# gmlc-dispatches/dispatches

Hardware: AMD Instinct MI355X
Metric: LP scenarios solved/sec, RTS-GMLC 24h multi-period dispatch, batch=4096 (higher is better)
Workload: dtype f64

## Files before the change

### dispatches_amd/csrc/dsp_capi.hip

```cpp
#include <hip/hip_runtime.h>

#include <cmath>
#include <cstdio>
#include <atomic>
#include <cstdlib>
#include <cstring>
#include <memory>
#include <new>
#include <vector>

#include "dsp_capi_internal.hpp"
#include "dsp_prepare.hpp"
#include "dsp_rtc.hpp"
#include "dsp_stream.hpp"

using namespace dsp;

struct Geometry { int wpb = 1, blocks_per_cu = 1; size_t lds = 0; };

struct dsp_handle {
  int device = 0;
  int n = 0, m = 0;
  int64_t nnz = 0;
  int cpl = 0, rpl = 0;
// ... 172 lines not shown
    Sc = build_slot_ell(AT, Lc, Lr, Ec.long_owner, pad_w);
    Sr = build_slot_ell(A, Lr, Lc, Er.long_owner, pad_w);
  }
  SlotELL Scu = build_slot_ell(ATu, Lc, Lr, Ec.long_owner, pad_w), Sru = build_slot_ell(Au, Lr, Lc, Er.long_owner, pad_w);
  const bool shared_slots = shared_slot_maps(cpl, rpl);
  SlotMap My = optimise_slots(Sc, P.m_pad, 4000, shared_slots), Mx = optimise_slots(Sr, P.n_pad, 4000, shared_slots);
  h->lds_conflicts[0] = My.cost_identity; h->lds_conflicts[1] = My.cost_final;
  h->lds_conflicts[2] = Mx.cost_identity; h->lds_conflicts[3] = Mx.cost_final;
  apply_slots(Sc, My.slot); apply_slots(Scu, My.slot);
  apply_slots(Sr, Mx.slot); apply_slots(Sru, Mx.slot);
  std::vector<int32_t> nat_x((size_t)P.n_pad, 0), nat_y((size_t)P.m_pad, 0);
  for (int j = 0; j < h->n; ++j) nat_x[j] = 8 * Mx.slot[Lc.pos[j]];
  for (int i = 0; i < h->m; ++i) nat_y[i] = 8 * My.slot[Lr.pos[i]];
  P.mr_wc_pack = Sc.pack; P.mr_wr_pack = Sr.pack; P.mr_tailc_entries = (int)Sc.tail_val.size(); P.mr_tailr_entries = (int)Sr.tail_val.size();
  if ((rc = fill_long(P.mr_long_c, Sc.long_owner_pos, Sc)) || (rc = fill_long(P.mr_long_r, Sr.long_owner_pos, Sr))) return rc;
  h->matreg = h->opt.no_matreg ? 0 : (rtc_ok ? 1 : matreg_available(cpl, rpl, Sc.pack, Sr.pack, has_long));
  h->matreg_qp = h->opt.no_matreg ? 0 : matreg_available(cpl, rpl, Sc.pack, Sr.pack, has_long, true);
  std::vector<Entry> pk;
  auto ent = [&](const std::vector<double> &val, const auto &idx, const Entry **field) {
    if (rc == DSP_OK) { pack_entries(val, idx, pk); rc = upload(h, pk, field); }
  };
  auto vec = [&](const auto &v, auto field) { if (rc == DSP_OK) rc = upload(h, v, field); };
  ent(Ec.val, Ec.idx, &P.ellc); ent(Er.val, Er.idx, &P.ellr); ent(Ec.tail_val, Ec.tail_idx, &P.tailc); ent(Er.tail_val, Er.tail_idx, &P.tailr);
  ent(Ecu.val, Ecu.idx, &P.ellc_unscaled); ent(Eru.val, Eru.idx, &P.ellr_unscaled);
  ent(Ecu.tail_val, Ecu.tail_idx, &P.tailc_unscaled); ent(Eru.tail_val, Eru.tail_idx, &P.tailr_unscaled);
  vec(h->dc, &P.col_scale); vec(h->dr, &P.row_scale);
  ent(Sc.val, Sc.off, &P.mr_ellc); ent(Sr.val, Sr.off, &P.mr_ellr); ent(Sc.tail_val, Sc.tail_off, &P.mr_tailc); ent(Sr.tail_val, Sr.tail_off, &P.mr_tailr);
  vec(Lc.at, &P.mr_colat); vec(Lr.at, &P.mr_rowat); vec(Mx.slot, &P.mr_slot_x); vec(My.slot, &P.mr_slot_y);
  ent(Scu.val, Scu.off, &P.mr_ellc_unscaled); ent(Sru.val, Sru.off, &P.mr_ellr_unscaled);
  ent(Scu.tail_val, Scu.tail_off, &P.mr_tailc_unscaled); ent(Sru.tail_val, Sru.tail_off, &P.mr_tailr_unscaled);
  vec(nat_x, &P.mr_nat_slot_x); vec(nat_y, &P.mr_nat_slot_y);
  return rc;
}

static int create_device_objects(dsp_handle *h, const HostCSR &A) {
  if (!h->opt.no_simplex && h->n + h->m <= 128 && h->m <= 64 && h->m >= 1) {
    h->sx_lds = simplex_lds_bytes(h->n, h->m, &h->sx_row_stride);
    if (h->sx_lds <= (size_t)h->lds_limit) {
      std::vector<double> dense((size_t)h->m * h->n, 0.0);
      for (int i = 0; i < A.m; ++i)
        for (int p = A.ptr[i]; p < A.ptr[i + 1]; ++p) dense[(size_t)i * h->n + A.idx[p]] = A.val[p];
      if (int rc = upload(h, dense, &h->A_dense)) return rc;
      h->simplex = 1;
    }
  }
  const size_t ring = sizeof(int) * kQueueRing * kQueueStride;
  if (hipMalloc((void **)&h->queue, ring) != hipSuccess || hipMemset(h->queue, 0, ring) != hipSuccess) return DSP_ERR_HIP;
  void *aw = nullptr;
  if (hipMalloc(&aw, sizeof(double) * (kAnchorWeights + 1)) != hipSuccess) return DSP_ERR_HIP;
  h->allocs.push_back(aw); h->anchor_w = (const double *)aw;
  hipLaunchKernelGGL(anchor_weight_kernel, dim3(1), dim3(256), 0, (hipStream_t)0, (double *)aw, kAnchorWeights + 1);
  if (hipGetLastError() != hipSuccess || hipStreamSynchronize((hipStream_t)0) != hipSuccess) return DSP_ERR_HIP;
  if (h->matreg && h->rtc_state[0] != 1) {
    SolveArgs first{}; first.P = h->P; first.matreg = 1; first.qp = 0;
    const size_t l = lds_bytes(h->P, 1, 0, h->cpl, h->rpl);
    if (l <= (size_t)h->lds_limit && light_followup_blocks(h->cpl, h->rpl, first, l) > 0) h->light_lds = l;
  }
  return DSP_OK;
}

static int resolve_options(const dsp_handle *h, const dsp_batch *batch, const dsp_options *opt, SolveArgs *a) {
  a->P = h->P; a->b = *batch; a->anchor_w = h->anchor_w;
  a->opt = opt ? *opt : h->opt;
  const dsp_options &o = a->opt;
  if (o.max_iter < 1 || o.check_every < 0 || o.kkt_every < 0 || !(o.kkt_gate >= 0) || o.stall_rescue < 0 || o.polish_patience < 0 || !(o.jump_rel >= 0) ||
      !(o.eps_rel > 0) || !(o.eps_obj >= 0) || !(o.eps_infeasible >= 0) || !(o.pid_kp >= 0) || !(o.restart_artificial >= 0) || !(o.step_scale > 0))
    return DSP_ERR_INVALID;
  a->eta = o.step_scale * h->eta_unit;
  a->qp = batch->row_compliance != nullptr;
  const bool fused64 = !h->streaming && o.precision == 0;
  if (o.restart_artificial == 0.0) a->opt.restart_artificial = fused64 ? (a->qp ? 0.3 : 0.2) : 0.36;
  if (o.pid_kp == 0.0) a->opt.pid_kp = fused64 ? 0.6 : 0.7;
  if (o.precision != 0 && o.precision != 1) return DSP_ERR_INVALID;
  const bool has_long = h->P.long_c.count > 0 || h->P.long_r.count > 0;
  if (o.precision && (h->streaming || has_long)) return DSP_ERR_INVALID;
  if (a->qp && !h->streaming && has_long) return DSP_ERR_INVALID;
  return DSP_OK;
}

static int finish_stats(dsp_handle *h, const dsp_batch *batch, dsp_stats *stats, bool timed, hipStream_t st) {
  if (!timed) return DSP_OK;
  const int B = batch->B;
  HIP_TRY(hipStreamSynchronize(st));
  HIP_TRY(hipEventElapsedTime(&stats->kernel_ms, h->ev0, h->ev1));
  std::vector<int32_t> hs(B), hi(B);
  HIP_TRY(hipMemcpy(hs.data(), batch->status, B * sizeof(int32_t), hipMemcpyDeviceToHost));
  if (batch->iters) HIP_TRY(hipMemcpy(hi.data(), batch->iters, B * sizeof(int32_t), hipMemcpyDeviceToHost));
  for (int i = 0; i < B; ++i) {
    stats->n_optimal += hs[i] == DSP_STATUS_OPTIMAL;
    if (batch->iters) { stats->total_iterations += hi[i]; stats->max_iterations = std::max(stats->max_iterations, hi[i]); }
  }
  return DSP_OK;
}

struct Followup { bool light = false; int wpb = 0; size_t lds = 0; };
static Followup followup_geometry(const dsp_handle *h, bool light) {
  Followup f{light};
  for (int wpb = 1; wpb <= 4 && !light; ++wpb) {
    const size_t l = lds_bytes(h->P, wpb, 0, h->cpl, h->rpl);
    if (l <= (size_t)h->lds_limit) { f.wpb = wpb; f.lds = l; }
  }
  if (light) { f.wpb = 1; f.lds = h->light_lds; }
  return f;
}
static hipError_t launch_followup(const dsp_handle *h, Followup f, const SolveArgs &first, const SolveArgs &c, int grid, hipStream_t st) {
  return f.light ? launch_solve_light(h->cpl, h->rpl, first, c, grid, f.lds, st)
                 : launch_solve(h->cpl, h->rpl, c, dim3(grid), dim3(64 * f.wpb), f.lds, st);
}

static int *claim_queue_slot(dsp_handle *h, hipStream_t st, int ints) {
  int *q = h->queue + (size_t)(h->queue_next.fetch_add(1u) % kQueueRing) * kQueueStride;
  hipLaunchKernelGGL(queue_reset_kernel, dim3(1), dim3(64), 0, st, q, ints);
  return q;
}

static int solve_streaming(dsp_handle *h, const dsp_batch *batch, const SolveArgs &a, dsp_stats *stats, bool timed, hipStream_t st) {
  if (timed) HIP_TRY(hipEventRecord(h->ev0, st));
  int periods = 0;
  HIP_TRY(stream_solve(&h->stream, *batch, a.opt, a.eta, st, &periods));
  if (timed) HIP_TRY(hipEventRecord(h->ev1, st));
  stats->streaming = 1; stats->quadratic = a.qp;
  stats->grid_blocks = (std::max(h->n, h->m) + 255) / 256; stats->block_threads = 256;
  stats->stream_bytes_per_iteration = (int64_t)stream_bytes_per_iteration(&h->stream);
  const StreamReport &rep = h->stream.report;
  stats->stream_form = rep.form;
  stats->stream_phases = rep.phases;
  stats->ipm_solved = rep.ipm_solved;
  return finish_stats(h, batch, stats, timed, st);
}

static int solve_f32(dsp_handle *h, const dsp_batch *batch, SolveArgs &a, dsp_stats *stats, bool timed, hipStream_t st) {
  a.queue = claim_queue_slot(h, st, 2);
  if (timed) HIP_TRY(hipEventRecord(h->ev0, st));
  int grid = 0, threads = 0; size_t lds = 0;
  HIP_TRY(launch_solve_f32(h->cpl, h->rpl, a, h->num_cus, (size_t)h->lds_limit, st, &grid, &threads, &lds));
  if (timed) HIP_TRY(hipEventRecord(h->ev1, st));
  stats->grid_blocks = grid; stats->block_threads = threads; stats->lds_bytes = (int)lds;
  stats->cols_per_lane = h->cpl; stats->rows_per_lane = h->rpl; stats->quadratic = a.qp; stats->precision = 1;
  return finish_stats(h, batch, stats, timed, st);
}

static int grow_simplex_warm(dsp_handle *h, int B) {
  const size_t N = (size_t)h->n + h->m;
  double *t = nullptr; int *bs = nullptr, *vl = nullptr; unsigned char *up = nullptr;
  HIP_TRY(hipMalloc((void **)&t, (size_t)B * h->m * N * sizeof(double))); h->sx_warm_allocs.push_back(t);
  HIP_TRY(hipMalloc((void **)&bs, (size_t)B * h->m * sizeof(int))); h->sx_warm_allocs.push_back(bs);
  HIP_TRY(hipMalloc((void **)&up, (size_t)B * N)); h->sx_warm_allocs.push_back(up);
  HIP_TRY(hipMalloc((void **)&vl, (size_t)B * sizeof(int))); h->sx_warm_allocs.push_back(vl);
  HIP_TRY(hipMemset(vl, 0, (size_t)B * sizeof(int)));
  h->sx_warm_T = t; h->sx_warm_basis = bs; h->sx_warm_upper = up; h->sx_warm_valid = vl; h->sx_warm_cap = B;
  return DSP_OK;
}

static int simplex_pass(dsp_handle *h, SolveArgs &a, hipStream_t st) {
  if (!h->simplex || a.qp) return DSP_OK;
  const int B = a.b.B;
  SimplexArgs sa{};
  sa.n = h->n; sa.m = h->m; sa.row_stride = h->sx_row_stride; sa.max_pivots = 20 * (h->n + h->m);
  sa.A_dense = h->A_dense; sa.col_scale = h->P.col_scale; sa.row_scale = h->P.row_scale; sa.b = a.b;
  sa.tol_p = 1e-10; sa.tol_d = 1e-12; sa.tol_piv = 1e-9; sa.unsolved = a.queue + 1;
  { static const char *tp = getenv("DSP_SX_TOLP"); if (tp) sa.tol_p = atof(tp); }
  if (a.opt.simplex_warm == 1 || a.opt.simplex_warm == 2) {
    if (B > h->sx_warm_cap)
      if (int rc = grow_simplex_warm(h, B)) return rc;
    sa.warm = a.opt.simplex_warm;
    sa.warm_T = h->sx_warm_T; sa.warm_basis = h->sx_warm_basis; sa.warm_upper = h->sx_warm_upper; sa.warm_valid = h->sx_warm_valid;
  }
  static const int sx_debug = getenv("DSP_SX_DEBUG") ? atoi(getenv("DSP_SX_DEBUG")) : 0;
  sa.debug_keep = sx_debug;
  const int per_cu = std::max<int>(1, std::min<int>(32, (int)((size_t)h->lds_limit / h->sx_lds)));
  HIP_TRY(launch_simplex(sa, std::min(B, h->num_cus * per_cu), h->sx_lds, st));
  a.skip_solved = 1;
  return DSP_OK;
}

static hipError_t first_pass(dsp_handle *h, SolveArgs &a, int grid, size_t lds, hipStream_t st) {
  if (!(h->rtc_state[a.qp] == 1 && a.matreg)) return launch_solve(h->cpl, h->rpl, a, dim3(grid), dim3(64 * a.waves_per_block), lds, st);
  size_t arg_size = sizeof(a);
  void *config[] = {HIP_LAUNCH_PARAM_BUFFER_POINTER, &a, HIP_LAUNCH_PARAM_BUFFER_SIZE, &arg_size, HIP_LAUNCH_PARAM_END};
  return hipModuleLaunchKernel(h->rtc[a.qp].fn, grid, 1, 1, 64 * a.waves_per_block, 1, 1, (unsigned)lds, st, nullptr, config);
}

static int certificate_pass(dsp_handle *h, const SolveArgs &a, Followup f, bool host_waits, hipStream_t st) {
  if (!a.matreg || !(a.opt.eps_infeasible > 0.0)) return DSP_OK;
  SolveArgs c = a;
  c.matreg = 0; c.skip_solved = 2; c.queue = a.queue + 3;
  c.b.x0 = a.b.x; c.b.y0 = a.b.y; c.waves_per_block = f.wpb;
  static const int cert_grid_env = getenv("DSP_CERT_GRID") ? atoi(getenv("DSP_CERT_GRID")) : 0;
  int nsus = -1;
  if (host_waits) {
    HIP_TRY(hipMemcpyAsync(&nsus, a.suspects, sizeof(int), hipMemcpyDeviceToHost, st));
    HIP_TRY(hipStreamSynchronize(st));
  }
  if (nsus == 0) return DSP_OK;
  const int want = nsus > 0 ? (nsus + f.wpb - 1) / f.wpb : (cert_grid_env > 0 ? cert_grid_env : 8);
  HIP_TRY(launch_followup(h, f, a, c, std::max(1, std::min(std::min((a.b.B + f.wpb - 1) / f.wpb, want), 2 * h->num_cus)), st));
  return DSP_OK;
}

static int recertify_passes(dsp_handle *h, const SolveArgs &a, Followup f, hipStream_t st) {
  if (!(a.opt.recertify_passes > 0 && a.b.flags)) return DSP_OK;
  static const struct { double pid_kp, restart_artificial; int check_every; } kRecertify[3] = {{0.45, 0.3, 0}, {0.8, 0.15, 0}, {0.3, 0.5, 12}};
  for (int v = 0; f.wpb && v < std::min(a.opt.recertify_passes, 3); ++v) {
    SolveArgs c = a;
    c.matreg = 0; c.skip_solved = 3; c.queue = a.queue + 5 + v;
    c.b.x0 = nullptr; c.b.y0 = nullptr; c.waves_per_block = f.wpb;
    c.opt.pid_kp = kRecertify[v].pid_kp; c.opt.restart_artificial = kRecertify[v].restart_artificial;
    if (kRecertify[v].check_every) c.opt.check_every = kRecertify[v].check_every;
    c.opt.polish_patience = std::max(c.opt.polish_patience, 1024);
    HIP_TRY(launch_followup(h, f, a, c, std::max(1, std::min((a.b.B + f.wpb - 1) / f.wpb, 64)), st));
  }
  return DSP_OK;
}

static int solve_fused(dsp_handle *h, const dsp_batch *batch, SolveArgs &a, dsp_stats *stats, bool timed, hipStream_t st) {
  const int B = batch->B, qp = a.qp;
  if (qp && h->rtc_state[1] == -1) {
    h->rtc_state[1] = rtc_get_kernel(h->device, h->cpl, h->rpl, false, h->P.mr_wc_pack, h->P.mr_wr_pack, true, &h->rtc[1], &h->rtc_why) ? 1 : 0;
    if (h->rtc_state[1] == 1) h->matreg_qp = 1;
  }
  Geometry geo;
  int rc = solve_geometry(h, a.opt.waves_per_block, B, &geo, qp);
  if (rc != DSP_OK) return rc;
  a.waves_per_block = geo.wpb; a.queue = claim_queue_slot(h, st, 8);
  a.queue_base = 0u; a.unsolved = a.queue + 1;
  a.suspects = a.queue + 2;
  a.matreg = qp ? h->matreg_qp : h->matreg;
#ifdef DSP_KKT_TRACE
  const char *trace_env = getenv("DSP_TRACE_SCENARIO");
  double *trace_dev = nullptr;
  if (trace_env) {
    HIP_TRY(hipMalloc((void **)&trace_dev, 4096 * 12 * sizeof(double)));
    HIP_TRY(hipMemsetAsync(trace_dev, 0, 4096 * 12 * sizeof(double), st));
    a.trace = trace_dev; a.trace_scenario = atoi(trace_env);
  }
#endif
  const int grid = std::min((B + geo.wpb - 1) / geo.wpb, h->num_cus * geo.blocks_per_cu);
  const Followup f = followup_geometry(h, a.matreg && !qp && h->rtc_state[0] != 1 && h->light_lds > 0);
  if (a.matreg && a.opt.eps_infeasible > 0.0 && !f.wpb) a.opt.eps_infeasible = 0.0;
  if (timed) HIP_TRY(hipEventRecord(h->ev0, st));
  if ((rc = simplex_pass(h, a, st)) != DSP_OK) return rc;
  HIP_TRY(first_pass(h, a, grid, geo.lds, st));
  if ((rc = certificate_pass(h, a, f, timed, st)) != DSP_OK || (rc = recertify_passes(h, a, f, st)) != DSP_OK) return rc;
  if (timed) HIP_TRY(hipEventRecord(h->ev1, st));
#ifdef DSP_KKT_TRACE
  if (trace_dev) {
    HIP_TRY(hipStreamSynchronize(st));
    std::vector<double> tr(4096 * 12);
    HIP_TRY(hipMemcpy(tr.data(), trace_dev, tr.size() * sizeof(double), hipMemcpyDeviceToHost));
    (void)hipFree(trace_dev);
    const char *path = getenv("DSP_TRACE_FILE");
    if (FILE *f = fopen(path ? path : "dsp_trace.bin", "wb")) { fwrite(tr.data(), sizeof(double), tr.size(), f); fclose(f); }
  }
#endif
  stats->grid_blocks = grid; stats->block_threads = 64 * a.waves_per_block; stats->lds_bytes = (int)geo.lds;
  stats->cols_per_lane = h->cpl; stats->rows_per_lane = h->rpl; stats->matreg = a.matreg; stats->simplex = h->simplex && !qp;
  stats->quadratic = qp; stats->rtc = (h->rtc_state[qp] == 1 && a.matreg) ? 1 : 0;
  stats->lds_conflicts_identity = h->lds_conflicts[0] + h->lds_conflicts[2];
  stats->lds_conflicts_chosen = a.matreg ? h->lds_conflicts[1] + h->lds_conflicts[3] : stats->lds_conflicts_identity;
  return finish_stats(h, batch, stats, timed, st);
}

extern "C" {

void dsp_default_options(dsp_options *o) {
  if (!o) return;
  std::memset(o, 0, sizeof(*o));
  o->eps_rel = 1e-9;
  o->eps_obj = 5e-7;
  o->max_iter = 200000;
  o->check_every = 0;
  o->kkt_every = 32;
  o->kkt_gate = 16.0;
  o->stall_rescue = 4000;
  o->no_simplex = 0;
  o->jump_rel = 3.0;
  o->restart_sufficient = 0.2;
  o->restart_necessary = 0.8;
  o->restart_artificial = 0.0;
  o->pid_kp = 0.0;
  o->max_dlog_weight = std::log(30.0);
  o->step_scale = 0.998;
  o->weight_guard = 4.0;
  o->jump_steady = 0.05;
  o->jump_tol = 3e-3;
  o->jump_min = 4.0;
  o->ray_jumps = 1;
  o->ruiz_iters = 10;
  o->waves_per_block = 0;
  o->precision = 0;
  o->polish_patience = 1024;
  o->no_rtc = 0;
  o->no_interior_point = 0;
  o->eps_infeasible = 1e-6;
  o->recertify_passes = 0;
  o->simplex_warm = 0;
  o->warm_patience = 0;
}

int dsp_version(void) { return DSP_VERSION; }
#ifndef DSP_SOURCE_HASH
#define DSP_SOURCE_HASH "unknown"
#endif
static const char kSourceHashTag[] = "dsp_source_hash=" DSP_SOURCE_HASH;
const char *dsp_source_hash(void) { return kSourceHashTag + 16; }
int dsp_last_hip_error(void) { return g_last_hip_error; }

const char *dsp_strerror(int code) {
  switch (code) {
    case DSP_OK: return "ok";
    case DSP_ERR_INVALID: return "invalid argument";
    case DSP_ERR_TOO_LARGE: return "LP too large (more than 4096 vectors longer than the ELL width, or dsp_spmv_step on a streaming handle)";
    case DSP_ERR_HIP: return "HIP runtime error (see dsp_last_hip_error)";
    case DSP_ERR_NO_DEVICE: return "no HIP device";
    case DSP_ERR_ALLOC: return "allocation failed";
    default: return "unknown error";
  }
}

int dsp_create(const dsp_lp_desc *d, int device, const dsp_options *opt, dsp_handle **out) {
  if (!out || !desc_ok(d)) return DSP_ERR_INVALID;
  static const int kCpl[] = {1, 2, 3, 4, 5, 7, 10};
  static const int kRpl[] = {1, 2, 3, 4, 6};
  int cpl = pick(kCpl, 7, (d->n + 63) / 64);
  int rpl = pick(kRpl, 5, std::max(1, (d->m + 63) / 64));
  const bool streaming = cpl < 0 || rpl < 0 || d->n > 65535 || d->m > 65535;
  if (streaming && d->m < 1) return DSP_ERR_INVALID;

  int ndev = 0;
  if (hipGetDeviceCount(&ndev) != hipSuccess || ndev <= 0) return DSP_ERR_NO_DEVICE;
  if (device < 0 || device >= ndev) return DSP_ERR_INVALID;
  HIP_TRY(hipSetDevice(device));

  struct Destroy { void operator()(dsp_handle *p) const { dsp_destroy(p); } };
  std::unique_ptr<dsp_handle, Destroy> owner(new (std::nothrow) dsp_handle());
  dsp_handle *h = owner.get();
  if (!h) return DSP_ERR_ALLOC;
  h->device = device; h->n = d->n; h->m = d->m; h->nnz = d->nnz; h->cpl = cpl; h->rpl = rpl;
  if (opt) h->opt = *opt; else dsp_default_options(&h->opt);
  hipDeviceProp_t prop;
  if (hipGetDeviceProperties(&prop, device) == hipSuccess) {
    h->num_cus = prop.multiProcessorCount;
    h->lds_limit = (int)prop.maxSharedMemoryPerMultiProcessor > 0 ? (int)prop.maxSharedMemoryPerMultiProcessor : 64 * 1024;
  }

  HostCSR A; A.m = d->m; A.n = d->n;
  A.ptr.assign(d->A_rowptr, d->A_rowptr + d->m + 1);
  A.idx.assign(d->A_colidx, d->A_colidx + d->nnz);
  A.val.assign(d->A_val, d->A_val + d->nnz);
  HostCSR Au = A;
  equilibrate(A, h->opt.ruiz_iters, h->dr, h->dc, std::max(0, h->opt.geo_iters), d->col_scale);
  HostCSR AT = transpose(A), ATu = transpose(Au);
  h->eta_unit = 1.0 / spectral_norm(A, AT, 500);
  int rc = streaming ? create_streaming(h, A, AT) : create_fused(h, A, AT, Au, ATu);
  if (rc == DSP_OK && !streaming) rc = create_device_objects(h, A);
  if (rc != DSP_OK) return rc;
  if (hipEventCreate(&h->ev0) != hipSuccess || hipEventCreate(&h->ev1) != hipSuccess) return DSP_ERR_HIP;
  *out = owner.release();
  return DSP_OK;
}

int dsp_solve(dsp_handle *h, const dsp_batch *batch, const dsp_options *opt, dsp_stats *stats, int sync_stats, void *hipStream) {
  if (!h || !batch || batch->B < 0) return DSP_ERR_INVALID;
  if (batch->B == 0) { if (stats) std::memset(stats, 0, sizeof(*stats)); return DSP_OK; }
  if (!batch->c || !batch->x || !batch->y || !batch->obj || !batch->status) return DSP_ERR_INVALID;
  hipStream_t st = (hipStream_t)hipStream;
  HIP_TRY(hipSetDevice(h->device));
  SolveArgs a{};
  if (int rc = resolve_options(h, batch, opt, &a)) return rc;
  dsp_stats lent;
  const bool timed = stats && sync_stats;
  stats = stats ? stats : &lent;
  std::memset(stats, 0, sizeof(*stats));
  if (h->streaming) return solve_streaming(h, batch, a, stats, timed, st);
  if (a.opt.precision == 1) return solve_f32(h, batch, a, stats, timed, st);
  return solve_fused(h, batch, a, stats, timed, st);
}

int dsp_spmv_step(dsp_handle *h, int32_t B, const double *X, const double *Y, double *AX, double *ATY, void *hipStream) {
  if (!h || B < 0 || !X || !Y || !AX || !ATY) return DSP_ERR_INVALID;
  if (B == 0) return DSP_OK;
  if (h->streaming) return DSP_ERR_TOO_LARGE;
  HIP_TRY(hipSetDevice(h->device));
  SpmvArgs a{};
  a.P = h->P; a.B = B; a.X = X; a.Y = Y; a.AX = AX; a.ATY = ATY;
  static const int wpb_env = getenv("DSP_SPMV_WPB") ? atoi(getenv("DSP_SPMV_WPB")) : 0;
  constexpr int kSpmvMaxWaves = 16;
  a.waves_per_block = wpb_env > 0 ? std::min(wpb_env, kSpmvMaxWaves) : kMaxWavesPerBlock;
  size_t lds = lds_bytes(h->P, a.waves_per_block);
  while (lds > (size_t)h->lds_limit && a.waves_per_block > 1) lds = lds_bytes(h->P, --a.waves_per_block);
  if (lds > (size_t)h->lds_limit) return DSP_ERR_TOO_LARGE;
  int blocks_per_cu = std::max<int>(1, std::min<int>((int)(h->lds_limit / lds), 32 / a.waves_per_block));
  int grid = std::min((B + a.waves_per_block - 1) / a.waves_per_block, h->num_cus * blocks_per_cu);
  const hipError_t se = launch_spmv(h->cpl, h->rpl, a, dim3(grid), dim3(64 * a.waves_per_block), lds, (hipStream_t)hipStream);
  if (se == hipErrorInvalidValue) return DSP_ERR_INVALID;
  HIP_TRY(se);
  return DSP_OK;
}

int dsp_rtc_compile_check(int cpl, int rpl, int has_long, unsigned wc_pack, unsigned wr_pack, int qp, char *msg, int msg_len) {
  std::vector<char> code;
  std::string name, why;
  const bool ok = rtc_build_code(cpl, rpl, has_long != 0, wc_pack, wr_pack, qp != 0, &code, &name, &why);
  if (msg && msg_len > 0) { std::snprintf(msg, (size_t)msg_len, "%s", ok ? name.c_str() : why.c_str()); }
  return ok ? (int)code.size() : 0;
}

const char *dsp_rtc_message(const dsp_handle *h) { return h ? h->rtc_why.c_str() : ""; }

int dsp_get_dims(const dsp_handle *h, int32_t *n, int32_t *m, int64_t *nnz) {
  if (!h) return DSP_ERR_INVALID;
  if (n) *n = h->n;
  if (m) *m = h->m;
// ... 27 lines not shown
```

### dispatches_amd/csrc/dsp_capi_internal.hpp

```cpp
#pragma once
#include "dsp_device.hpp"

namespace dsp { inline thread_local int g_last_hip_error = 0; }

#define HIP_TRY(expr)                                                                                            \
  do {                                                                                                           \
    if (hipError_t _e = (expr); _e != hipSuccess) { dsp::g_last_hip_error = (int)_e; return DSP_ERR_HIP; }       \
  } while (0)
```

### dispatches_amd/csrc/dsp_capi_loop.hip

```cpp
#include <cmath>
#include <vector>

#include "dsp_capi_internal.hpp"
#include "dsp_record_check.hpp"

using namespace dsp;

static bool market_col_ok(int32_t col, int32_t n) { return col >= 0 && col < n; }
static bool loop_cols_ok(const int32_t *cols, int count, int32_t n) {
  for (int i = 0; i < count; ++i)
    if (!market_col_ok(cols[i], n)) return false;
  return true;
}
static bool loop_terms_ok(const int32_t (*pt_cols)[2], int T, int32_t n) {
  for (int t = 0; t < T; ++t)
    for (int e = 0; e < 2; ++e)
      if (pt_cols[t][e] != -1 && !market_col_ok(pt_cols[t][e], n)) return false;
  return true;
}
static bool loop_wind_ok(const int32_t *wind_cols, int T, int32_t n, const void *cf_series) {
  return wind_cols[0] < 0 || (cf_series && loop_cols_ok(wind_cols, T, n));
}
static bool plant_sizes_ok(const double *wind_kw_plant, const double *c0_base_plant, int32_t wind_col0) {
  if (!wind_kw_plant != !c0_base_plant) return false;
  return !wind_kw_plant || wind_col0 >= 0;
}
static bool loop_tracker_cols_ok(const dsp_loop_model *tr, int T, const void *state, const void *cf_series) {
  if (tr->n_state < 0 || tr->n_state > 2 || (tr->n_state > 0 && !state)) return false;
  return loop_cols_ok(tr->state_init, tr->n_state, tr->n) && loop_cols_ok(tr->track_rows, T, tr->m) && loop_wind_ok(tr->wind_cols, T, tr->n, cf_series) &&
         plant_sizes_ok(tr->wind_kw_plant, tr->c0_base_plant, tr->wind_cols[0]);
}
static bool loop_tracker_ok(const dsp_loop_model *tr, int T, const void *state, const void *cf_series) {
  if (!tr || T < 1 || T > DSP_LOOP_MAX_T || tr->T != T || tr->n < 1 || tr->m < 1) return false;
  if (!tr->lb || !tr->ub || !tr->rlo || !tr->rhi || !tr->c0) return false;
  return loop_tracker_cols_ok(tr, T, state, cf_series);
}
static bool market_state_ok(const dsp_market_state *st) {
  if (!st || st->B < 0 || st->N < 1 || st->S < 1 || st->S > DSP_MARKET_MAX_S) return false;
  if (st->backcast ? (st->D < 1 || st->S > st->D || 24ll * st->D > st->N) : st->S != 1) return false;
  return st->start && st->hour && st->da_series && st->rt_series;
}
static bool loop_market_state_ok(const dsp_loop_market_state *st) {
  if (!st || st->B < 0 || st->N < 1 || st->S < 1 || st->S > DSP_MARKET_MAX_S || st->p_min_cents < 0 || st->p_min_cents > 2000000000ll) return false;
  if (st->backcast ? (st->D < 1 || st->S > st->D || 24ll * st->D > st->N) : st->S != 1) return false;
  if (st->rt_history_lag_days < 0 || (st->backcast && 24ll * ((long long)st->D + st->rt_history_lag_days) > st->N)) return false;
  if (st->self_schedule < 0 || st->self_schedule > 1) return false;
  if (st->curve_slots != 0 && (st->curve_slots < st->S + 1 || st->curve_slots > DSP_MARKET_MAX_S + 1)) return false;
  if (st->coupled < 0 || st->coupled > 1 || (st->coupled && st->self_schedule)) return false;
  return st->start && st->hour && st->da_series && st->rt_series;
}
static bool loop_market_model_ok(const dsp_loop_market_model *m) {
  return m && m->n >= 1 && m->T >= 1 && m->T <= DSP_MARKET_MAX_T && m->n_state >= 0 && m->n_state <= 2 &&
         (m->row_stride == 0 || m->row_stride >= m->n);
}
static bool loop_market_prepare_ok(const dsp_loop_market_state *st, const dsp_loop_market_model *m) {
  if (!m->c || !m->lb || !m->ub || !m->base_c || !m->c0) return false;
  if ((m->n_state > 0 && !st->state) || !loop_cols_ok(m->state_init, m->n_state, m->n)) return false;
  if (!loop_wind_ok(m->wind_cols, m->T, m->n, st->cf_series) || !plant_sizes_ok(m->wind_kw_plant, m->c0_base_plant, m->wind_cols[0])) return false;
  return loop_cols_ok(m->pda_cols, m->T, m->n) && loop_terms_ok(m->pt_cols, m->T, m->n);
}

static bool plant_p_min_ok(const dsp_loop_market_state *st, hipStream_t stream) {
  if (!st->p_min_cents_plant || st->B == 0) return true;
  hipStreamCaptureStatus capturing = hipStreamCaptureStatusNone;
  if (hipStreamIsCapturing(stream, &capturing) != hipSuccess) return false;
  if (capturing != hipStreamCaptureStatusNone) return true;
  std::vector<int64_t> host((size_t)st->B);
  if (hipMemcpyAsync(host.data(), st->p_min_cents_plant, host.size() * sizeof(int64_t), hipMemcpyDeviceToHost, stream) != hipSuccess) return false;
  if (hipStreamSynchronize(stream) != hipSuccess) return false;
  for (int64_t v : host)
    if (v < 0 || v > 2000000000ll) return false;
  return true;
}

extern "C" {

int dsp_wb_rolling_update(const dsp_wb_state *st, const dsp_wb_model *rt, const dsp_wb_model *tr, int32_t phase, int32_t k, void *hipStream) {
  if (!st || !rt || !tr || st->B < 0 || phase < 0 || phase > 2 || k < 0 || k > 23 || rt->T < 1 || rt->T > 8 || tr->T < 1 || tr->T > 8)
    return DSP_ERR_INVALID;
  if (st->B == 0) return DSP_OK;
  HIP_TRY(launch_wb_rolling(*st, *rt, *tr, (int)phase, (int)k, (hipStream_t)hipStream));
  return DSP_OK;
}

int dsp_loop_update(const dsp_loop_state *st, const dsp_loop_model *rt, const dsp_loop_model *tr, int32_t phase, int32_t k, void *hipStream) {
  if (!st || !rt || !tr || st->B < 0 || phase < 0 || phase > 2 || k < 0 || k > 23 || rt->T < 1 || rt->T > DSP_LOOP_MAX_T || tr->T < 1 ||
      tr->T > DSP_LOOP_MAX_T || rt->n_state < 0 || rt->n_state > 2 || tr->n_state != rt->n_state || !rt->c0 || !tr->c0)
    return DSP_ERR_INVALID;
  if (!plant_sizes_ok(rt->wind_kw_plant, rt->c0_base_plant, rt->wind_cols[0]) || !rt->wind_kw_plant != !tr->wind_kw_plant) return DSP_ERR_INVALID;
  if ((phase < 2 && tr->T > rt->T) || !loop_tracker_cols_ok(tr, tr->T, st->state, st->cf_series) || !loop_cols_ok(tr->state_real, tr->n_state, tr->n) ||
      !loop_terms_ok(tr->pt_cols, tr->T, tr->n))
    return DSP_ERR_INVALID;
  if (!loop_cols_ok(rt->pda_cols, rt->T, rt->n) || !loop_terms_ok(rt->pt_cols, rt->T, rt->n) || !loop_cols_ok(rt->state_init, rt->n_state, rt->n) ||
      !loop_wind_ok(rt->wind_cols, rt->T, rt->n, st->cf_series))
    return DSP_ERR_INVALID;
  if (st->B == 0) return DSP_OK;
  HIP_TRY(launch_loop_update(*st, *rt, *tr, (int)phase, (int)k, (hipStream_t)hipStream));
  return DSP_OK;
}

int dsp_loop_ledger(const dsp_loop_state *st, const dsp_loop_model *tr, const dsp_loop_ledger_desc *g, void *hipStream) {
  if (!st || !tr || !g || st->B < 0 || tr->n < 1 || !tr->x) return DSP_ERR_INVALID;
  if (g->n_forms < 1 || g->n_forms > DSP_LEDGER_MAX_FORMS || g->reserved != 0) return DSP_ERR_INVALID;
  if (!g->acc || !g->hour_value || !g->coef || !g->constant) return DSP_ERR_INVALID;
  if (g->coef_stride < 0 || (g->coef_stride != 0 && g->coef_stride < (int64_t)g->n_forms * DSP_LEDGER_MAX_TERMS)) return DSP_ERR_INVALID;
  if (g->const_stride < 0 || (g->const_stride != 0 && g->const_stride < g->n_forms)) return DSP_ERR_INVALID;
  for (int f = 0; f < g->n_forms; ++f) {
    if (g->n_terms[f] < 0 || g->n_terms[f] > DSP_LEDGER_MAX_TERMS || !loop_cols_ok(g->cols[f], g->n_terms[f], tr->n)) return DSP_ERR_INVALID;
    if (g->per_avail[f] == 0.0) continue;
    if (!std::isfinite(g->per_avail[f]) || tr->wind_cols[0] < 0 || !st->cf_series || !st->start || !st->hour || st->N < 1) return DSP_ERR_INVALID;
    if (!plant_sizes_ok(tr->wind_kw_plant, tr->c0_base_plant, tr->wind_cols[0])) return DSP_ERR_INVALID;
  }
  if (st->B == 0) return DSP_OK;
  HIP_TRY(launch_loop_ledger(*st, *tr, *g, (hipStream_t)hipStream));
  return DSP_OK;
}

int dsp_loop_record(const dsp_loop_record_desc *rec, int32_t B, void *hipStream) {
  if (!loop_record_ok(rec, B)) return DSP_ERR_INVALID;
  HIP_TRY(launch_loop_record(*rec, (hipStream_t)hipStream));
  return DSP_OK;
}

int dsp_bid_points(const dsp_bid_request *rq, void *hipStream) {
  if (!rq || rq->B < 0 || rq->T < 0 || rq->terms < 0 || rq->terms > 2 || rq->ldx < 1 || rq->ldp < rq->T) return DSP_ERR_INVALID;
  if (rq->B > DSP_BID_MAX_SCENARIOS || rq->T > DSP_BID_MAX_HOURS) return DSP_ERR_TOO_LARGE;
  if (rq->T == 0) return DSP_OK;
  if (!rq->out || (rq->B > 0 && (!rq->x || !rq->price))) return DSP_ERR_INVALID;
  for (int t = 0; t < rq->T; ++t)
    for (int e = 0; e < (rq->terms == 2 ? 2 : 1); ++e)
      if (rq->col[t][e] < 0 || rq->col[t][e] >= rq->ldx) return DSP_ERR_INVALID;
  HIP_TRY(launch_bid_points(*rq, (hipStream_t)hipStream));
  return DSP_OK;
}

int dsp_market_prepare(const dsp_market_state *st, const dsp_market_model *m, int32_t k, void *hipStream) {
  if (!market_state_ok(st) || !m || k < -1 || k > 23 || m->n < 1 || m->T < 1 || m->T > DSP_MARKET_MAX_T) return DSP_ERR_INVALID;
  if (!st->cf_series || !st->soc || !st->thr || !m->c || !m->lb || !m->ub || !m->base_c) return DSP_ERR_INVALID;
  if (k >= 0 && (!st->da_offer || !st->da_prices)) return DSP_ERR_INVALID;
  if (!market_col_ok(m->soc_init, m->n) || !market_col_ok(m->thr_init, m->n)) return DSP_ERR_INVALID;
  for (int t = 0; t < m->T; ++t)
    if (!market_col_ok(m->wind_cols[t], m->n) || !market_col_ok(m->pt_cols[t][0], m->n) || !market_col_ok(m->pt_cols[t][1], m->n) ||
        !market_col_ok(m->pda_cols[t], m->n))
      return DSP_ERR_INVALID;
  if (st->B == 0) return DSP_OK;
  HIP_TRY(launch_market_prepare(*st, *m, (int)k, (hipStream_t)hipStream));
  return DSP_OK;
}

int dsp_market_clear(const dsp_market_state *st, const dsp_market_model *m, const dsp_wb_model *tr, int32_t k, int32_t T,
                     double *dispatch, int32_t *curve, int32_t *count, void *hipStream) {
  if (!market_state_ok(st) || !m || k < -1 || k > 23 || m->n < 1 || m->T < 1 || m->T > DSP_MARKET_MAX_T || T < 1 || T > m->T) return DSP_ERR_INVALID;
  if (!m->x || !m->status || !dispatch || !curve || !count) return DSP_ERR_INVALID;
  if (k < 0 ? (T > 24 || !st->da_prices || tr) : T > 8) return DSP_ERR_INVALID;
  for (int t = 0; t < T; ++t)
    if (k < 0 ? !market_col_ok(m->pda_cols[t], m->n) : (!market_col_ok(m->pt_cols[t][0], m->n) || !market_col_ok(m->pt_cols[t][1], m->n)))
      return DSP_ERR_INVALID;
  if (tr) {
    if (tr->T != T || tr->n < 1 || tr->m < 1 || !tr->lb || !tr->ub || !tr->rlo || !tr->rhi || !st->cf_series || !st->soc || !st->thr) return DSP_ERR_INVALID;
    if (!market_col_ok(tr->soc_init, tr->n) || !market_col_ok(tr->thr_init, tr->n)) return DSP_ERR_INVALID;
    for (int t = 0; t < T; ++t)
      if (!market_col_ok(tr->wind_cols[t], tr->n) || !market_col_ok(tr->track_rows[t], tr->m)) return DSP_ERR_INVALID;
  }
  if (st->B == 0) return DSP_OK;
  HIP_TRY(launch_market_clear(*st, *m, tr, (int)k, (int)T, dispatch, curve, count, (hipStream_t)hipStream));
  return DSP_OK;
}

int dsp_loop_market_prepare(const dsp_loop_market_state *st, const dsp_loop_market_model *m, int32_t k, void *hipStream) {
  if (!loop_market_state_ok(st) || !loop_market_model_ok(m) || k < -1 || k > 23) return DSP_ERR_INVALID;
  if (m->row_stride != 0 && m->row_stride != m->n) return DSP_ERR_INVALID;
  if (k >= 0 && (!st->da_offer || !st->da_prices)) return DSP_ERR_INVALID;
  if (!loop_market_prepare_ok(st, m)) return DSP_ERR_INVALID;
  if (st->B == 0) return DSP_OK;
  HIP_TRY(launch_loop_market_prepare(*st, *m, (int)k, (hipStream_t)hipStream));
  return DSP_OK;
}

int dsp_loop_schedule_prepare(const dsp_loop_market_state *st, const dsp_loop_market_model *m, void *hipStream) {
  if (!loop_market_state_ok(st) || !loop_market_model_ok(m)) return DSP_ERR_INVALID;
  if ((long long)m->row_stride < (long long)st->S * m->n) return DSP_ERR_INVALID;
  if (!loop_market_prepare_ok(st, m) || m->wind_kw_plant || m->c0_base_plant) return DSP_ERR_INVALID;
  if (st->B == 0) return DSP_OK;
  HIP_TRY(launch_loop_schedule_prepare(*st, *m, (hipStream_t)hipStream));
  return DSP_OK;
}

int dsp_loop_monotone_prepare(const dsp_loop_market_state *st, const dsp_loop_market_model *m, double *rlo, double *rhi, int32_t m_rows,
                              int32_t first_coupling_row, void *hipStream) {
  if (!loop_market_state_ok(st) || !loop_market_model_ok(m) || !rlo || !rhi || st->S < 2 || first_coupling_row < 0) return DSP_ERR_INVALID;
  if ((long long)m->row_stride < (long long)st->S * m->n) return DSP_ERR_INVALID;
  if ((long long)first_coupling_row + (long long)(st->S * (st->S - 1) / 2) * m->T > (long long)m_rows) return DSP_ERR_INVALID;
  if (!loop_market_prepare_ok(st, m) || m->wind_kw_plant || m->c0_base_plant) return DSP_ERR_INVALID;
  if (st->B == 0) return DSP_OK;
  HIP_TRY(launch_loop_monotone_prepare(*st, *m, rlo, rhi, (int)m_rows, (int)first_coupling_row, (hipStream_t)hipStream));
  return DSP_OK;
}

int dsp_loop_market_clear(const dsp_loop_market_state *st, const dsp_loop_market_model *m, const dsp_loop_model *tr, int32_t k, int32_t T,
                          double *dispatch, int32_t *curve, int32_t *count, void *hipStream) {
  if (!loop_market_state_ok(st) || !loop_market_model_ok(m) || k < -1 || k > 23 || T < 1 || T > m->T) return DSP_ERR_INVALID;
  if (st->coupled && (long long)m->row_stride < (long long)st->S * m->n) return DSP_ERR_INVALID;
  if (!m->x || !m->status || !dispatch || !curve || !count) return DSP_ERR_INVALID;
  if (k < 0 ? (T > 24 || !st->da_prices || tr) : T > DSP_LOOP_MAX_T) return DSP_ERR_INVALID;
  if (!plant_sizes_ok(m->wind_kw_plant, m->c0_base_plant, m->wind_cols[0])) return DSP_ERR_INVALID;
  if (k < 0 ? !loop_cols_ok(m->pda_cols, T, m->n) : !loop_terms_ok(m->pt_cols, T, m->n)) return DSP_ERR_INVALID;
  if (tr && (!loop_tracker_ok(tr, T, st->state, st->cf_series) || tr->n_state != m->n_state || !tr->wind_kw_plant != !m->wind_kw_plant)) return DSP_ERR_INVALID;
  if (!plant_p_min_ok(st, (hipStream_t)hipStream)) return DSP_ERR_INVALID;
  if (st->B == 0) return DSP_OK;
  HIP_TRY(launch_loop_market_clear(*st, *m, tr, (int)k, (int)T, dispatch, curve, count, (hipStream_t)hipStream));
  return DSP_OK;
}

int dsp_loop_param_step(const dsp_loop_param_state *st, const dsp_loop_model *tr, int32_t phase, int32_t k, void *hipStream) {
  if (!st || !tr || st->B < 1 || st->N < 24 || tr->T < 1 || tr->T > DSP_LOOP_MAX_T) return DSP_ERR_INVALID;
  if (phase < 0 || phase > 2 || (phase == 0 ? k != -1 : (k < 0 || k > 23))) return DSP_ERR_INVALID;
  if (tr->wind_kw_plant || tr->c0_base_plant) return DSP_ERR_INVALID;
  if (!st->start || !st->hour || !st->da_series || !st->rt_series || !st->da_cf_series || !st->rt_cf_series || !st->bid_price ||
      !st->storage_mw)
    return DSP_ERR_INVALID;
  if (phase == 0) {
    if (!st->da_offer || !st->da_prices || !st->da_curve || !st->da_count) return DSP_ERR_INVALID;
  } else if (phase == 1) {
    if (!st->rt_dispatch || !st->rt_curve || !st->rt_count) return DSP_ERR_INVALID;
    if (!loop_tracker_ok(tr, tr->T, st->state, st->rt_cf_series)) return DSP_ERR_INVALID;
  } else {
    if (!st->h2_kg || !tr->x || tr->n < 1 || !market_col_ok(st->pem_col, tr->n)) return DSP_ERR_INVALID;
  }
  HIP_TRY(launch_loop_param_step(*st, *tr, (int)phase, (hipStream_t)hipStream));
  return DSP_OK;
}

int dsp_loop_project(const dsp_loop_project_state *st, const dsp_loop_model *pj, int32_t phase, int32_t j, void *hipStream) {
  if (!st || st->B < 1 || st->N < 1 || st->ruc_hour < 1 || st->ruc_hour > 23 || phase < 0 || phase > 2) return DSP_ERR_INVALID;
// ... 23 lines not shown
```

### dispatches_amd/csrc/dsp_device.hpp

```cpp
#pragma once
#ifdef __HIPCC_RTC__
#ifndef DSP_RTC_TYPES
#define DSP_RTC_TYPES
typedef signed char int8_t; typedef unsigned char uint8_t; typedef short int16_t; typedef unsigned short uint16_t;
typedef int int32_t; typedef unsigned int uint32_t; typedef long long int64_t; typedef unsigned long long uint64_t;
typedef unsigned long uintptr_t; typedef unsigned long size_t;
#ifndef INFINITY
#define INFINITY (__builtin_inff())
#endif
#ifndef NAN
#define NAN (__builtin_nanf(""))
#endif
#endif
#else
#include <hip/hip_runtime.h>

#include <cstdint>
#endif

#include "../../include/dsp_hip.h"
#include "dsp_shapes.hpp"

namespace dsp {

constexpr int kMaxLong = 32;

struct __attribute__((aligned(16))) Entry {
  double v;
  uint32_t off;
  uint32_t pad;
};

struct LongList {
  int count;
  int owner[kMaxLong];
  int start[kMaxLong];
  int len[kMaxLong];
};

struct DeviceProblem {
  int n, m;
  int n_pad, m_pad;
  int Wc, Wr;
  int ellc_entries, ellr_entries, tailc_entries, tailr_entries;
  const Entry *ellc, *ellr, *tailc, *tailr;
  const Entry *ellc_unscaled, *ellr_unscaled, *tailc_unscaled, *tailr_unscaled;
  const double *col_scale, *row_scale;
  LongList long_c, long_r;
  const Entry *mr_ellc, *mr_ellr, *mr_tailc, *mr_tailr;
  int mr_tailc_entries, mr_tailr_entries;
  const int *mr_colat, *mr_rowat;
  unsigned mr_wc_pack, mr_wr_pack;
  const int32_t *mr_slot_x, *mr_slot_y;
  LongList mr_long_c, mr_long_r;
  const Entry *mr_ellc_unscaled, *mr_ellr_unscaled, *mr_tailc_unscaled, *mr_tailr_unscaled;
  const int32_t *mr_nat_slot_x, *mr_nat_slot_y;
};

#define DSP_STATUS_UNSOLVED 99
#define DSP_STATUS_SUSPECT 98

struct SolveArgs {
  DeviceProblem P;
  dsp_batch b;
  int skip_solved;
  int waves_per_block;
  double eta;
  dsp_options opt;
  int *queue;
  unsigned queue_base;
  const int *unsolved;
  int matreg;
  int qp;
  double *trace;
  int trace_scenario;
  int *suspects;
  const double *anchor_w;
};

constexpr int kAnchorWeights = 4096;

#ifdef DSP_KKT_TRACE
#define DSP_SW_TRACE 1ull
#else
#define DSP_SW_TRACE 0ull
#endif
#ifdef DSP_PROF
#define DSP_SW_PROF 2ull
#else
#define DSP_SW_PROF 0ull
#endif
#ifdef DSP_CLOCKS
#define DSP_SW_CLOCKS 4ull
#else
#define DSP_SW_CLOCKS 0ull
#endif
#ifdef DSP_LEGACY_PULL
#define DSP_SW_PULL 8ull
#else
#define DSP_SW_PULL 0ull
#endif
#ifdef DSP_NO_JUMP
#define DSP_SW_NOJUMP 16ull
#else
#define DSP_SW_NOJUMP 0ull
#endif
constexpr unsigned long long kBuildSwitches = DSP_SW_TRACE | DSP_SW_PROF | DSP_SW_CLOCKS | DSP_SW_PULL | DSP_SW_NOJUMP;
constexpr unsigned long long kSolveArgsToken =
    ((unsigned long long)sizeof(SolveArgs) << 40) ^ ((unsigned long long)__builtin_offsetof(SolveArgs, opt) << 28) ^
    ((unsigned long long)__builtin_offsetof(SolveArgs, queue) << 16) ^ ((unsigned long long)sizeof(DeviceProblem) << 52) ^
    ((unsigned long long)DSP_VERSION << 8) ^ kBuildSwitches ^ ((unsigned long long)__builtin_offsetof(SolveArgs, anchor_w) << 4) ^
    ((unsigned long long)rare_lds_bytes(0) << 20);

struct SimplexArgs {
  int n, m;
  int row_stride;
  int max_pivots;
  const double *A_dense;
  const double *col_scale, *row_scale;
  dsp_batch b;
  double tol_p, tol_d, tol_piv;
  int *unsolved;
  int debug_keep;
  int warm;
  double *warm_T;
  int *warm_basis;
  unsigned char *warm_upper;
  int *warm_valid;
};

struct SpmvArgs {
  DeviceProblem P;
  int B;
  int waves_per_block;
  const double *X, *Y;
  double *AX, *ATY;
};

constexpr int kPadWidth = 4;
inline unsigned uniform_pack(int slots, int w) { unsigned p = 0; for (int q = 0; q < slots; ++q) p |= (unsigned)w << (4 * q); return p; }

#ifndef __HIPCC_RTC__
hipError_t launch_solve(int cpl, int rpl, const SolveArgs &a, dim3 grid, dim3 block, size_t lds, hipStream_t st);
int matreg_available(int cpl, int rpl, unsigned wc_pack, unsigned wr_pack, bool lng, bool qp = false);
hipError_t occupancy_solve(int cpl, int rpl, const SolveArgs &a, int block_threads, size_t lds, int *blocks_per_cu);
int light_followup_blocks(int cpl, int rpl, const SolveArgs &first, size_t lds);
hipError_t launch_solve_light(int cpl, int rpl, const SolveArgs &first, const SolveArgs &a, int grid, size_t lds, hipStream_t st);
size_t simplex_lds_bytes(int n, int m, int *row_stride);
hipError_t launch_simplex(const SimplexArgs &a, int grid, size_t lds, hipStream_t st);
hipError_t launch_solve_f32(int cpl, int rpl, const SolveArgs &a, int num_cus, size_t lds_limit, hipStream_t st, int *grid,
                            int *threads, size_t *lds);
hipError_t launch_wb_rolling(const dsp_wb_state &st, const dsp_wb_model &rt, const dsp_wb_model &tr, int phase, int k, hipStream_t stream);
hipError_t launch_loop_update(const dsp_loop_state &st, const dsp_loop_model &rt, const dsp_loop_model &tr, int phase, int k, hipStream_t stream);
hipError_t launch_loop_ledger(const dsp_loop_state &st, const dsp_loop_model &tr, const dsp_loop_ledger_desc &ledger, hipStream_t stream);
hipError_t launch_loop_record(const dsp_loop_record_desc &rec, hipStream_t stream);
hipError_t launch_bid_points(const dsp_bid_request &rq, hipStream_t st);
hipError_t launch_market_prepare(const dsp_market_state &st, const dsp_market_model &m, int k, hipStream_t stream);
hipError_t launch_market_clear(const dsp_market_state &st, const dsp_market_model &m, const dsp_wb_model *tr, int k, int T, double *dispatch,
                               int32_t *curve, int32_t *count, hipStream_t stream);
hipError_t launch_loop_market_prepare(const dsp_loop_market_state &st, const dsp_loop_market_model &m, int k, hipStream_t stream);
hipError_t launch_loop_schedule_prepare(const dsp_loop_market_state &st, const dsp_loop_market_model &m, hipStream_t stream);
hipError_t launch_loop_monotone_prepare(const dsp_loop_market_state &st, const dsp_loop_market_model &m, double *rlo, double *rhi, int m_rows,
                                        int first, hipStream_t stream);
hipError_t launch_loop_market_clear(const dsp_loop_market_state &st, const dsp_loop_market_model &m, const dsp_loop_model *tr, int k, int T,
                                    double *dispatch, int32_t *curve, int32_t *count, hipStream_t stream);
hipError_t launch_loop_param_step(const dsp_loop_param_state &st, const dsp_loop_model &tr, int phase, hipStream_t stream);
hipError_t launch_loop_project(const dsp_loop_project_state &st, const dsp_loop_model &pj, int phase, int j, hipStream_t stream);
hipError_t launch_spmv(int cpl, int rpl, const SpmvArgs &a, dim3 grid, dim3 block, size_t lds, hipStream_t st);

#endif

}
```

### dispatches_amd/csrc/dsp_loop.hip

```cpp
#include <hip/hip_runtime.h>

#include "dsp_device.hpp"
#include "dsp_loop_device.hpp"

using namespace dsp;

template <class M, class S>
__device__ __forceinline__ void loop_check(const S &s, const M &m, int b) {
  if (m.status && s.bad && m.status[b] != 0) *s.bad = 1;
  if (m.flags && s.uncertified && (m.flags[b] & DSP_FLAG_OBJ_WAIVED)) atomicAdd(reinterpret_cast<unsigned long long *>(s.uncertified), 1ull);
}

__global__ void __launch_bounds__(256) wb_rolling_kernel(dsp_wb_state s, dsp_wb_model rt, dsp_wb_model tr, int phase, int k) {
  const int b = blockIdx.x * blockDim.x + threadIdx.x;
  if (b >= s.B) return;
  const long long h = *s.hour, st0 = s.start[b];
  auto win = [&](const double *series, int t) { return series[(st0 + h + t) % s.N]; };
  if (phase == 0) {
    const dsp_wb_model &m = rt;
    const int known = min(m.T, 24 - k);
    double *c = m.c + (size_t)b * m.n, *lb = m.lb + (size_t)b * m.n, *ub = m.ub + (size_t)b * m.n;
    double avail_sum = 0.0;
    for (int t = 0; t < m.T; ++t) {
      const double rtp = win(s.rt_series, t);
      const double dap = t < known ? s.da_prices[(size_t)b * 24 + k + t] : win(s.da_series, t);
      const double r3 = loop_opaque(__dmul_rn(1e-3, rtp));
      c[m.pt_cols[t][0]] = __dsub_rn(m.base_c[m.pt_cols[t][0]], r3);
      c[m.pt_cols[t][1]] = __dsub_rn(m.base_c[m.pt_cols[t][1]], r3);
      c[m.pda_cols[t]] = __dsub_rn(m.base_c[m.pda_cols[t]], loop_opaque(__dsub_rn(dap, rtp)));
      const double avail = __dmul_rn(m.wind_kw, win(s.cf_series, t));
      ub[m.wind_cols[t]] = avail;
      avail_sum = t ? __dadd_rn(avail_sum, avail) : avail;
      const double fix = t < known ? s.da_offer[(size_t)b * 24 + k + t] : 0.0;
      lb[m.pda_cols[t]] = fix;
      ub[m.pda_cols[t]] = t < known ? fix : INFINITY;
    }
    if (m.c0) m.c0[b] = __dadd_rn(m.c0_base, loop_opaque(__dmul_rn(m.waste_per_kw, avail_sum)));
    lb[m.soc_init] = s.soc[b]; ub[m.soc_init] = s.soc[b];
    lb[m.thr_init] = s.thr[b]; ub[m.thr_init] = s.thr[b];
  } else if (phase == 1) {
    loop_check(s, rt, b);
    const double *xr = rt.x + (size_t)b * rt.n;
    double *lb = tr.lb + (size_t)b * tr.n, *ub = tr.ub + (size_t)b * tr.n;
    double *rlo = tr.rlo + (size_t)b * tr.m, *rhi = tr.rhi + (size_t)b * tr.m;
    double avail_sum = 0.0;
    for (int t = 0; t < tr.T; ++t) {
      const double offer = __dmul_rn(1e-3, loop_opaque(__dadd_rn(xr[rt.pt_cols[t][0]], xr[rt.pt_cols[t][1]])));
      rlo[tr.track_rows[t]] = offer;
      rhi[tr.track_rows[t]] = offer;
      const double avail = __dmul_rn(tr.wind_kw, win(s.cf_series, t));
      ub[tr.wind_cols[t]] = avail;
      avail_sum = t ? __dadd_rn(avail_sum, avail) : avail;
    }
    if (tr.c0) tr.c0[b] = __dadd_rn(tr.c0_base, loop_opaque(__dmul_rn(tr.waste_per_kw, avail_sum)));
    lb[tr.soc_init] = s.soc[b]; ub[tr.soc_init] = s.soc[b];
    lb[tr.thr_init] = s.thr[b]; ub[tr.thr_init] = s.thr[b];
  } else {
    loop_check(s, tr, b);
    const double *x = tr.x + (size_t)b * tr.n;
    const double delivered = loop_opaque(__dmul_rn(1e-3, loop_opaque(__dadd_rn(x[tr.pt_cols[0][0]], x[tr.pt_cols[0][1]]))));
    const double rt0 = win(s.rt_series, 0);
    s.delivered[b] = delivered;
    s.soc[b] = __ddiv_rn(rint(loop_opaque(__dmul_rn(x[tr.soc0], 100.0))), 100.0);
    s.thr[b] = __ddiv_rn(rint(loop_opaque(__dmul_rn(x[tr.thr0], 100.0))), 100.0);
    const double dao = s.da_offer[(size_t)b * 24 + k], dap = s.da_prices[(size_t)b * 24 + k];
    const double t1 = loop_opaque(__dmul_rn(delivered, rt0)), t2 = loop_opaque(__dmul_rn(dao, loop_opaque(__dsub_rn(dap, rt0))));
    s.revenue[b] = __dadd_rn(s.revenue[b], loop_opaque(__dadd_rn(t1, t2)));
    s.energy_mwh[b] = __dadd_rn(s.energy_mwh[b], delivered);
  }
}

__global__ void wb_clock_kernel(long long *hour) { *hour += 1; }

__device__ __forceinline__ double loop_power(const dsp_loop_model &m, const double *x, int t) {
  double p = m.pt_const[t];
  if (m.pt_cols[t][0] >= 0) p = fma(m.pt_coef[t][0], x[m.pt_cols[t][0]], p);
  if (m.pt_cols[t][1] >= 0) p = fma(m.pt_coef[t][1], x[m.pt_cols[t][1]], p);
  return p;
}
__device__ __forceinline__ void loop_state_and_wind(const dsp_loop_state &s, const dsp_loop_model &m, int b, long long h, long long st0, double c0) {
  double *lb = m.lb + (size_t)b * m.n, *ub = m.ub + (size_t)b * m.n;
  for (int j = 0; j < m.n_state; ++j) {
    const double v = s.state[(size_t)b * m.n_state + j];
    lb[m.state_init[j]] = v; ub[m.state_init[j]] = v;
  }
  if (m.wind_cols[0] >= 0) {
    const double kw = m.wind_kw_plant ? m.wind_kw_plant[b] : m.wind_kw;
    double sum = 0.0;
    for (int t = 0; t < m.T; ++t) {
      const double avail = kw * s.cf_series[(st0 + h + t) % s.N];
      ub[m.wind_cols[t]] = avail;
      sum += avail;
    }
    c0 = fma(m.waste_per_kw, sum, c0);
  }
  m.c0[b] = c0;
}
__global__ void __launch_bounds__(256) loop_update_kernel(dsp_loop_state s, dsp_loop_model rt, dsp_loop_model tr, int phase, int k) {
  const int b = blockIdx.x * blockDim.x + threadIdx.x;
  if (b >= s.B) return;
  const long long h = *s.hour, st0 = s.start[b];
  auto win = [&](const double *series, int t) { return series[(st0 + h + t) % s.N]; };
  if (phase == 0) {
    const dsp_loop_model &m = rt;
    const int known = min(m.T, 24 - k);
    double *c = m.c + (size_t)b * m.n, *lb = m.lb + (size_t)b * m.n, *ub = m.ub + (size_t)b * m.n;
    double c0 = m.c0_base_plant ? m.c0_base_plant[b] : m.c0_base;
    for (int t = 0; t < m.T; ++t) {
      const double rtp = win(s.rt_series, t);
      const double dap = t < known ? s.da_prices[(size_t)b * 24 + k + t] : win(s.da_series, t);
      for (int e = 0; e < 2; ++e)
        if (m.pt_cols[t][e] >= 0) c[m.pt_cols[t][e]] = fma(-rtp, m.pt_coef[t][e], m.base_c[m.pt_cols[t][e]]);
      c[m.pda_cols[t]] = m.base_c[m.pda_cols[t]] - (dap - rtp);
      c0 = fma(-rtp, m.pt_const[t], c0);
      const double fix = t < known ? s.da_offer[(size_t)b * 24 + k + t] : 0.0;
      lb[m.pda_cols[t]] = fix;
      ub[m.pda_cols[t]] = t < known ? fix : INFINITY;
    }
    loop_state_and_wind(s, m, b, h, st0, c0);
  } else if (phase == 1) {
    loop_check(s, rt, b);
    const double *xr = rt.x + (size_t)b * rt.n;
    double *rlo = tr.rlo + (size_t)b * tr.m, *rhi = tr.rhi + (size_t)b * tr.m;
    for (int t = 0; t < tr.T; ++t) {
      const double rhs = loop_power(rt, xr, t) - tr.pt_const[t];
      rlo[tr.track_rows[t]] = rhs;
      rhi[tr.track_rows[t]] = rhs;
    }
    loop_state_and_wind(s, tr, b, h, st0, tr.c0_base_plant ? tr.c0_base_plant[b] : tr.c0_base);
  } else {
    loop_check(s, tr, b);
    const double *x = tr.x + (size_t)b * tr.n;
    const double delivered = loop_power(tr, x, 0);
    const double rt0 = win(s.rt_series, 0);
    s.delivered[b] = delivered;
    for (int j = 0; j < tr.n_state; ++j)
      s.state[(size_t)b * tr.n_state + j] = rint(x[tr.state_real[j]] * s.state_scale[j]) / s.state_scale[j];
    const double dao = s.da_offer[(size_t)b * 24 + k], dap = s.da_prices[(size_t)b * 24 + k];
    s.revenue[b] += delivered * rt0 + dao * (dap - rt0);
    s.energy_mwh[b] += delivered;
  }
}

__global__ void __launch_bounds__(256) loop_ledger_kernel(dsp_loop_state s, const double *x, int n, double wind_kw, const double *wind_kw_plant,
                                                          dsp_loop_ledger_desc g) {
  const int b = blockIdx.x * blockDim.x + threadIdx.x, f = blockIdx.y;
  if (b >= s.B) return;
  const double per_avail = g.per_avail[f];
  double avail0 = 0.0;
  if (per_avail != 0.0) {
    const double kw = wind_kw_plant ? wind_kw_plant[b] : wind_kw;
    avail0 = loop_opaque(__dmul_rn(kw, s.cf_series[(s.start[b] + *s.hour) % s.N]));
  }
  const double *coef = g.coef + (size_t)b * g.coef_stride + f * DSP_LEDGER_MAX_TERMS;
  const double v = loop_ledger_form(x + (size_t)b * n, g.cols[f], coef, g.n_terms[f], g.constant[(size_t)b * g.const_stride + f], per_avail, avail0);
  const size_t at = (size_t)f * s.B + b;
  g.hour_value[at] = v;
  g.acc[at] = __dadd_rn(g.acc[at], loop_opaque(v));
}

__global__ void __launch_bounds__(256) loop_record_kernel(dsp_loop_record_desc d) {
  const dsp_loop_record_segment &g = d.segments[blockIdx.y];
  const int e = blockIdx.x * blockDim.x + threadIdx.x;
  if (e >= d.n_plants * g.width) return;
  const int q = e / g.width, j = e - q * g.width;
  const long long t = *d.clock + d.offset;
  const long long r = (t < 0 || t / d.divisor >= d.rows) ? d.rows : t / d.divisor;
  const size_t from = (size_t)d.plants[q] * (size_t)g.plant_stride + (size_t)j * (size_t)g.elem_stride;
  const size_t to = ((size_t)r * d.n_plants + q) * g.width + j;
  if (g.elem_bytes == 8)
    ((unsigned long long *)g.dst)[to] = ((const unsigned long long *)g.src)[from];
  else
    ((unsigned int *)g.dst)[to] = ((const unsigned int *)g.src)[from];
}

namespace dsp {

hipError_t launch_loop_record(const dsp_loop_record_desc &rec, hipStream_t stream) {
  int widest = 0;
  for (int g = 0; g < rec.n_segments; ++g) widest = rec.segments[g].width > widest ? rec.segments[g].width : widest;
  const long long lanes = (long long)rec.n_plants * widest;
  hipLaunchKernelGGL(loop_record_kernel, dim3((unsigned)((lanes + 255) / 256), rec.n_segments), dim3(256), 0, stream, rec);
  return hipGetLastError();
}

hipError_t launch_loop_ledger(const dsp_loop_state &st, const dsp_loop_model &tr, const dsp_loop_ledger_desc &ledger, hipStream_t stream) {
  hipLaunchKernelGGL(loop_ledger_kernel, dim3((st.B + 255) / 256, ledger.n_forms), dim3(256), 0, stream, st, tr.x, (int)tr.n, tr.wind_kw,
                     tr.wind_kw_plant, ledger);
  return hipGetLastError();
}

template <class K, class S, class M>
static hipError_t launch_hand_off(K kernel, const S &st, const M &rt, const M &tr, int phase, int k, hipStream_t stream) {
  hipLaunchKernelGGL(kernel, dim3((st.B + 255) / 256), dim3(256), 0, stream, st, rt, tr, phase, k);
  if (phase == 2) hipLaunchKernelGGL(wb_clock_kernel, dim3(1), dim3(1), 0, stream, (long long *)st.hour);
  return hipGetLastError();
}
hipError_t launch_wb_rolling(const dsp_wb_state &st, const dsp_wb_model &rt, const dsp_wb_model &tr, int phase, int k, hipStream_t stream) {
  return launch_hand_off(wb_rolling_kernel, st, rt, tr, phase, k, stream);
}
hipError_t launch_loop_update(const dsp_loop_state &st, const dsp_loop_model &rt, const dsp_loop_model &tr, int phase, int k, hipStream_t stream) {
  return launch_hand_off(loop_update_kernel, st, rt, tr, phase, k, stream);
}

}
```

### dispatches_amd/csrc/dsp_loop_device.hpp

```cpp
#pragma once
#include <hip/hip_runtime.h>

#include <cstdint>

#include "../../include/dsp_hip.h"
#include "dsp_bid_cents.hpp"

namespace dsp {

__device__ __forceinline__ double loop_opaque(double v) { asm volatile("" : "+v"(v)); return v; }

template <class State>
__device__ __forceinline__ long long loop_scenario_index(const State &s, long long st0, long long h, int i, int hod, int t) {
  if (!s.backcast) return (st0 + h + t) % s.N;
  const long long D = s.D, d = h / 24;
  const long long pos = (24 * (D - 1 - i) + hod + t) % (24 * D);
  long long v = (st0 + 24 * (d - D) + pos) % s.N;
  return v < 0 ? v + s.N : v;
}

__device__ __forceinline__ double loop_wind_window(double *ub, const int32_t *wind_cols, int T, double kw, const double *cf_series,
                                                   long long first, long long N) {
  double avail_sum = 0.0;
  for (int q = 0; q < T; ++q) {
    const double avail = loop_opaque(__dmul_rn(kw, cf_series[(first + q) % N]));
    ub[wind_cols[q]] = avail;
    avail_sum = q ? __dadd_rn(avail_sum, avail) : avail;
  }
  return avail_sum;
}

__device__ __forceinline__ double loop_c0(double base, double per_kw, double avail_sum) {
  return __dadd_rn(base, loop_opaque(__dmul_rn(per_kw, avail_sum)));
}

__device__ __forceinline__ void loop_tracker_plant(const dsp_loop_model &tr, int b, const double *cf_series, long long first, long long N,
                                                   const double *state) {
  double *lb = tr.lb + (size_t)b * tr.n, *ub = tr.ub + (size_t)b * tr.n;
  for (int j = 0; j < tr.n_state; ++j) {
    const double v = state[j];
    lb[tr.state_init[j]] = v; ub[tr.state_init[j]] = v;
  }
  double c0 = tr.c0_base_plant ? tr.c0_base_plant[b] : tr.c0_base;
  if (tr.wind_cols[0] >= 0) {
    const double kw = tr.wind_kw_plant ? tr.wind_kw_plant[b] : tr.wind_kw;
    c0 = loop_c0(c0, tr.waste_per_kw, loop_wind_window(ub, tr.wind_cols, tr.T, kw, cf_series, first, N));
  }
  tr.c0[b] = c0;
}

__device__ __forceinline__ double loop_ledger_form(const double *x, const int32_t *cols, const double *coef, int E, double constant,
                                                   double per_avail, double avail0) {
  double v = constant;
  for (int e = 0; e < E; ++e) v = fma(coef[e], x[cols[e]], v);
  if (per_avail != 0.0) v = fma(per_avail, avail0, v);
  return v;
}

__device__ __forceinline__ void loop_emit_point(int32_t *out, int &pos, long long &run, long long &cleared, long long U, long long M,
                                                bool price_taker, double lmp) {
  run = pos == 0 ? M : max(run, M);
  out[2 * pos] = (int32_t)U;
  out[2 * pos + 1] = (int32_t)run;
  if (pos == 0 || !price_taker || __ddiv_rn((double)run, 100.0) <= lmp) cleared = U;
  ++pos;
}

__device__ __forceinline__ double loop_curve_close(int32_t *out, int pos, int slots, long long cleared) {
  for (int q = pos; q < slots; ++q) { out[2 * q] = 0; out[2 * q + 1] = 0; }
  return __ddiv_rn((double)cleared, 100.0);
}

template <int SP>
__device__ __forceinline__ double loop_curve_and_clear(const long long (&keys)[SP], int S, long long pmin, bool price_taker, double lmp,
                                                       int32_t *out, int32_t *count) {
  const bool has_min = keys[0] != kBidDrop && bid_key_power(keys[0]) == pmin;
  long long lowest = 0x7fffffffffffffffll;
  int n = 0;
#pragma unroll
  for (int i = 0; i < SP; ++i) {
    const bool first = keys[i] != kBidDrop && (i == 0 || bid_key_power(keys[i]) != bid_key_power(keys[i ? i - 1 : 0]));
    if (first) { lowest = min(lowest, bid_key_price(keys[i])); ++n; }
  }
  int pos = 0;
  long long run = 0, cleared = 0;
  if (!has_min) loop_emit_point(out, pos, run, cleared, pmin, n == 0 ? 0 : lowest, price_taker, lmp);
#pragma unroll
  for (int i = 0; i < SP; ++i) {
    const bool first = keys[i] != kBidDrop && (i == 0 || bid_key_power(keys[i]) != bid_key_power(keys[i ? i - 1 : 0]));
    if (first) loop_emit_point(out, pos, run, cleared, bid_key_power(keys[i]), bid_key_price(keys[i]), price_taker, lmp);
  }
  *count = pos;
  return loop_curve_close(out, pos, S + 1, cleared);
}

}
```

### dispatches_amd/csrc/dsp_simplex.hip

```cpp
#include <hip/hip_runtime.h>

#include <cmath>
#include <cstdint>
#include <cstdlib>

#include "dsp_device.hpp"
#include "dsp_wave.hpp"

namespace dsp {

namespace {

constexpr double kBig = 1e300;

__device__ __forceinline__ double lds_d(const double *base, int idx) { return base[idx]; }

__device__ __forceinline__ int first_lane(unsigned long long mask) { return __ffsll((long long)mask) - 1; }

template <int CQ>
__global__ void __launch_bounds__(64, CQ == 1 ? 4 : 3) simplex_kernel(SimplexArgs a) {
  extern __shared__ __attribute__((aligned(16))) char smem[];
  const dsp_batch &b = a.b;
  const int lane = threadIdx.x;
  const int n = a.n, m = a.m, N = n + m;
  const int RS = a.row_stride;
  double *T = reinterpret_cast<double *>(smem);
  const int mp = (m + 1) & ~1, Np = (N + 1) & ~1;
  double *alpha_s = T + (size_t)m * RS;
  double *cB_s = alpha_s + mp;
  double *xval = cB_s + mp;
  double *scal = xval + Np;
  int *iscal = reinterpret_cast<int *>(scal + 8);

  for (int s = blockIdx.x; s < b.B; s += gridDim.x) {
    bool use_warm = a.warm == 1 && a.warm_valid[s] != 0;
    int pivots_before = 0;
  restart:
    double lo[CQ], hi[CQ], cost[CQ], val[CQ];
    bool basic[CQ], upper[CQ], fixedv[CQ], live[CQ];
    double cabs = 0.0;
    bool bad = false;
#pragma unroll
    for (int q = 0; q < CQ; ++q) {
      const int j = lane + 64 * q;
      live[q] = j < N;
      lo[q] = 0.0; hi[q] = 0.0; cost[q] = 0.0;
      if (j < n) {
        const double d = a.col_scale[j];
        const double cu = b.c[(size_t)s * b.c_stride + j];
        const double lu = b.var_lb ? b.var_lb[(size_t)s * b.var_lb_stride + j] : -INFINITY;
        const double uu = b.var_ub ? b.var_ub[(size_t)s * b.var_ub_stride + j] : INFINITY;
        cost[q] = cu * d; lo[q] = lu / d; hi[q] = uu / d;
        if (!(lu <= uu) || !(cu == cu)) bad = true;
      } else if (j < N) {
        const int i = j - n;
        const double d = a.row_scale[i];
        const double l = b.row_lb ? b.row_lb[(size_t)s * b.row_lb_stride + i] : -INFINITY;
        const double u = b.row_ub ? b.row_ub[(size_t)s * b.row_ub_stride + i] : INFINITY;
        lo[q] = l * d; hi[q] = u * d;
        if (!(l <= u)) bad = true;
      }
      cabs = fmax(cabs, fabs(cost[q]));
      fixedv[q] = lo[q] == hi[q];
      basic[q] = live[q] && j >= n;
      const bool lo_f = is_finite(lo[q]), hi_f = is_finite(hi[q]);
      double v = 0.0;
      if (lo_f && (!hi_f || fabs(lo[q]) <= fabs(hi[q]))) v = lo[q];
      else if (hi_f) v = hi[q];
      val[q] = v;
      upper[q] = hi_f && v == hi[q] && !(v == lo[q]);
    }
    if (__ballot(bad) != 0ull) {
#pragma unroll
      for (int q = 0; q < CQ; ++q) { const int j = lane + 64 * q; if (j < n) b.x[(size_t)s * n + j] = NAN; }
      if (lane < m) b.y[(size_t)s * m + lane] = NAN;
      bool nanc = false;
#pragma unroll
      for (int q = 0; q < CQ; ++q) nanc |= !(cost[q] == cost[q]);
      const bool any_nan = __ballot(nanc) != 0ull;
      if (lane == 0) {
        b.obj[s] = NAN;
        b.status[s] = any_nan ? DSP_STATUS_NUMERICAL : DSP_STATUS_PRIMAL_INFEASIBLE;
        if (b.iters) b.iters[s] = 0;
        if (b.jumps) b.jumps[s] = 0;
        if (b.flags) b.flags[s] = 0;
      }
      continue;
    }
    const double ctol = a.tol_d * (1.0 + wave_max(cabs));
    int bvar = (lane < m) ? n + lane : -1;
    double beta = 0.0, blo = -INFINITY, bhi = INFINITY;
    if (use_warm) {
      const double *Ts = a.warm_T + (size_t)s * m * N;
      if (lane < m) bvar = a.warm_basis[(size_t)s * m + lane];
      for (int i0 = 0; i0 < m; i0 += 4) {
        double tv[4][CQ];
#pragma unroll
        for (int u = 0; u < 4; ++u) {
          const int i = min(i0 + u, m - 1);
#pragma unroll
          for (int q = 0; q < CQ; ++q) { const int j = lane + 64 * q; tv[u][q] = (j < N) ? Ts[(size_t)i * N + j] : 0.0; }
        }
#pragma unroll
        for (int u = 0; u < 4; ++u) {
          if (i0 + u < m) {
#pragma unroll
            for (int q = 0; q < CQ; ++q) { const int j = lane + 64 * q; if (j < N) T[(i0 + u) * RS + j] = tv[u][q]; }
          }
        }
      }
#pragma unroll
      for (int q = 0; q < CQ; ++q) { const int j = lane + 64 * q; if (j < N) xval[j] = lo[q]; }
      wave_lds_fence();
      if (lane < m) blo = xval[bvar];
      wave_lds_fence();
#pragma unroll
      for (int q = 0; q < CQ; ++q) { const int j = lane + 64 * q; if (j < N) xval[j] = hi[q]; }
      wave_lds_fence();
      if (lane < m) bhi = xval[bvar];
      wave_lds_fence();
#pragma unroll
      for (int q = 0; q < CQ; ++q) { const int j = lane + 64 * q; if (j < N) xval[j] = 0.0; }
      wave_lds_fence();
      if (lane < m) xval[bvar] = 1.0;
      wave_lds_fence();
#pragma unroll
      for (int q = 0; q < CQ; ++q) {
        const int j = lane + 64 * q;
        basic[q] = live[q] && xval[j] != 0.0;
        const bool lo_f = is_finite(lo[q]), hi_f = is_finite(hi[q]);
        bool up = live[q] && a.warm_upper[(size_t)s * N + j] != 0 && hi_f && !fixedv[q];
        if (!lo_f && hi_f) up = true;
        val[q] = up ? hi[q] : (lo_f ? lo[q] : 0.0);
        upper[q] = up;
      }
      wave_lds_fence();
#pragma unroll
      for (int q = 0; q < CQ; ++q) { const int j = lane + 64 * q; if (j < N) xval[j] = basic[q] ? 0.0 : val[q]; }
      wave_lds_fence();
      if (lane < m) {
#pragma unroll 8
        for (int j = 0; j < N; ++j) beta = fma(-T[lane * RS + j], xval[j], beta);
      }
    } else {
      for (int i0 = 0; i0 < m; i0 += 4) {
        double tv[4][CQ];
#pragma unroll
        for (int u = 0; u < 4; ++u) {
          const int i = min(i0 + u, m - 1);
#pragma unroll
          for (int q = 0; q < CQ; ++q) { const int j = lane + 64 * q; tv[u][q] = (j < n) ? -a.A_dense[(size_t)i * n + j] : ((j - n == i) ? 1.0 : 0.0); }
        }
#pragma unroll
        for (int u = 0; u < 4; ++u) {
          if (i0 + u < m) {
#pragma unroll
            for (int q = 0; q < CQ; ++q) { const int j = lane + 64 * q; if (j < N) T[(i0 + u) * RS + j] = tv[u][q]; }
          }
        }
      }
#pragma unroll
      for (int q = 0; q < CQ; ++q) { const int j = lane + 64 * q; if (j < N) xval[j] = val[q]; }
      wave_lds_fence();
      if (lane < m) {
#pragma unroll 8
        for (int j = 0; j < n; ++j) beta = fma(-T[lane * RS + j], xval[j], beta);
        const double d = a.row_scale[lane];
        const double l = b.row_lb ? b.row_lb[(size_t)s * b.row_lb_stride + lane] : -INFINITY;
        const double u = b.row_ub ? b.row_ub[(size_t)s * b.row_ub_stride + lane] : INFINITY;
        blo = l * d; bhi = u * d;
      }
    }
    const int it_limit = use_warm ? min(a.max_pivots, 6 * N) : a.max_pivots;
    int status = -1, pivots = pivots_before;
    bool p1_priced_out = false;
    bool phase1 = false;

    int refines = 0;
    double res_c = 0.0, mag_c = 0.0;
    bool res_valid = false;
    bool tight = false;
  pivot:
    for (int it = 0;; ++it) {
      const double ptol = (tight ? 1e-3 : 1.0) * a.tol_p * (1.0 + fmax(fabs(finite_or_zero(blo)), fabs(finite_or_zero(bhi))));
      const bool below = lane < m && beta < blo - ptol;
      const bool above = lane < m && beta > bhi + ptol;
      phase1 = __ballot(below || above) != 0ull;
// ... 549 lines not shown
      wave_lds_fence();
      if (lane < m) xval[n + lane] = res;
      wave_lds_fence();
      double rj[CQ];
#pragma unroll
      for (int q = 0; q < CQ; ++q) { const int j = lane + 64 * q; rj[q] = (j >= n && j < N) ? xval[j] : 0.0; }
#pragma unroll
      for (int i0 = 0; i0 < MR; i0 += 4) {
        double part[4];
#pragma unroll
        for (int u = 0; u < 4; ++u) {
          double t = 0.0;
#pragma unroll
          for (int q = 0; q < CQ; ++q) t = fma(T[i0 + u][q], rj[q], t);
          part[u] = t;
        }
        wave_sums<4>(part);
#pragma unroll
        for (int u = 0; u < 4; ++u) if (lane == i0 + u && lane < m) beta += part[u];
      }
      wave_lds_fence();
      bool out = false;
      if (lane < m) {
        const double tt = 1e-3 * a.tol_p * (1.0 + fmax(fabs(finite_or_zero(blo)), fabs(finite_or_zero(bhi))));
        out = beta < blo - tt || beta > bhi + tt;
      }
      if (__ballot(out) != 0ull) { tight = true; status = -1; goto pivot; }
    }

#pragma unroll
    for (int q = 0; q < CQ; ++q) { const int j = lane + 64 * q; if (j < N) xval[j] = val[q]; }
    wave_lds_fence();
    if (lane < m) xval[bvar] = beta;
    wave_lds_fence();
    double xs[CQ];
    double po = 0.0;
    bool okv = true, okb = true, okr = true;
    double viol = 0.0;
#pragma unroll
    for (int q = 0; q < CQ; ++q) {
      const int j = lane + 64 * q;
      xs[q] = (j < N) ? xval[j] : 0.0;
      if (j < N) {
        const double scl = 1.0 + fmax(fabs(xs[q]), fmax(fabs(finite_or_zero(lo[q])), fabs(finite_or_zero(hi[q]))));
        const double tol = 1e-9 * scl;
        if (xs[q] < lo[q] - tol || xs[q] > hi[q] + tol || !(xs[q] == xs[q])) { okv = false; okb = false; }
        viol = fmax(viol, fmax(lo[q] - xs[q], xs[q] - hi[q]) / scl);
      }
      if (j < n) po = fma(cost[q], xs[q], po);
    }
    po = wave_sum(po);
    {
      double res = 0.0, mag = 0.0;
      for (int i0 = 0; i0 < m; i0 += 2) {
        double part[4] = {0.0, 0.0, 0.0, 0.0};
#pragma unroll
        for (int u = 0; u < 2; ++u) {
          const int i = i0 + u;
          if (i < m) {
#pragma unroll
            for (int q = 0; q < CQ; ++q) {
              const int j = lane + 64 * q;
              if (j < n) { const double t = a.A_dense[(size_t)i * n + j] * xs[q]; part[2 * u] += t; part[2 * u + 1] += fabs(t); }
            }
          }
        }
        wave_sums<4>(part);
#pragma unroll
        for (int u = 0; u < 2; ++u)
          if (lane == i0 + u) { res = part[2 * u] - xval[n + lane]; mag = part[2 * u + 1] + fabs(xval[n + lane]); }
      }
      const double gmag = wave_max(mag);
      if (lane < m && !(fabs(res) <= 1e-9 * (1.0 + gmag))) { okv = false; okr = false; }
    }
    const bool certified = __ballot(!okv) == 0ull;
    const unsigned long long bad_bounds = __ballot(!okb), bad_any = __ballot(!okv);
    int reason = status == -1 ? 1 : 0;
    if (status == DSP_STATUS_OPTIMAL && !certified) { status = -1; reason = 2; }
    const bool clearly_infeasible = status == DSP_STATUS_PRIMAL_INFEASIBLE && p1_priced_out && __ballot(!okr) == 0ull && wave_max(viol) > 1e-6;
    if (clearly_infeasible) {
#pragma unroll
      for (int q = 0; q < CQ; ++q) { const int j = lane + 64 * q; if (j < n) b.x[(size_t)s * n + j] = NAN; }
      if (lane < m) b.y[(size_t)s * m + lane] = NAN;
      if (lane == 0) {
        b.obj[s] = NAN;
        b.status[s] = DSP_STATUS_PRIMAL_INFEASIBLE;
        if (b.iters) b.iters[s] = pivots;
        if (b.jumps) b.jumps[s] = 0;
        if (b.flags) b.flags[s] = 0;
      }
      wave_lds_fence();
      continue;
    }
    if (status == DSP_STATUS_PRIMAL_INFEASIBLE || status == DSP_STATUS_DUAL_INFEASIBLE) { status = -1; reason = 3; }
    if (status == -1) {
      if (lane == 0) {
        if (a.debug_keep) {
          b.status[s] = 50 + reason;
          if (b.iters) b.iters[s] = pivots;
          if (b.jumps) b.jumps[s] = bad_bounds ? 1000 + first_lane(bad_bounds) : (bad_any ? 2000 + first_lane(bad_any) : 0);
          b.obj[s] = po;
          if (b.flags) b.flags[s] = 0;
        } else {
          b.status[s] = DSP_STATUS_UNSOLVED;
          atomicAdd(a.unsolved, 1);
        }
      }
      wave_lds_fence();
      continue;
    }
    double dsl[CQ];
#pragma unroll
    for (int q = 0; q < CQ; ++q) dsl[q] = cost[q];
    const double cb2 = (lane < m) ? cbas : 0.0;
#pragma unroll
    for (int i = 0; i < MR; ++i) {
      const double cb = readlane_f64(cb2, i);
#pragma unroll
      for (int q = 0; q < CQ; ++q) dsl[q] = fma(-cb, T[i][q], dsl[q]);
    }
#pragma unroll
    for (int q = 0; q < CQ; ++q) {
      const int j = lane + 64 * q;
      if (j < n) b.x[(size_t)s * n + j] = xs[q] * a.col_scale[j];
      else if (j < N) b.y[(size_t)s * m + (j - n)] = dsl[q] * a.row_scale[j - n];
    }
    if (lane == 0) {
      b.obj[s] = po;
      b.status[s] = status;
      if (b.iters) b.iters[s] = pivots;
      if (b.jumps) b.jumps[s] = 0;
      if (b.flags) b.flags[s] = 0;
    }
    wave_lds_fence();
  }
}

}

size_t simplex_lds_bytes(int n, int m, int *row_stride) {
  const int N = n + m;
  int rs = N | 1;
  if (row_stride) *row_stride = rs;
  const int mp = (m + 1) & ~1, Np = (N + 1) & ~1;
  return ((size_t)m * rs + mp + mp + Np + 8 + 8) * sizeof(double);
}

hipError_t launch_simplex(const SimplexArgs &a, int grid, size_t lds, hipStream_t st) {
  const int cq = (a.n + a.m + 63) / 64;
  if (cq > 2) return hipErrorInvalidValue;
  SimplexArgs args = a;
  void *params[] = {&args};
  static const int force_lds = getenv("DSP_SX_LDS") ? atoi(getenv("DSP_SX_LDS")) : 0;
  if (!force_lds && !a.warm && a.m <= 24 && cq <= 1 && a.b.B <= 2048) {
    const void *fr = reinterpret_cast<const void *>(&simplex_reg_kernel<1, 24>);
    return hipLaunchKernel(fr, dim3(a.b.B < grid ? a.b.B : grid), dim3(64), params, 0, st);
  }
  const void *fn = cq <= 1 ? reinterpret_cast<const void *>(&simplex_kernel<1>)
                           : reinterpret_cast<const void *>(&simplex_kernel<2>);
  hipError_t e = hipFuncSetAttribute(fn, hipFuncAttributeMaxDynamicSharedMemorySize, (int)lds);
  if (e != hipSuccess) return e;
  return hipLaunchKernel(fn, dim3(grid), dim3(64), params, lds, st);
}

}
```

### dispatches_amd/hip_solver.py

```python
from __future__ import annotations

import ctypes as C
import os
from typing import Optional

import numpy as np

_HERE = os.path.dirname(os.path.abspath(__file__))
_LIB_PATH = os.path.join(_HERE, os.environ.get("DSP_LIB", "libdsp_hip.so"))
_lib = None


class DspOptions(C.Structure):
    _fields_ = [("eps_rel", C.c_double), ("eps_obj", C.c_double), ("max_iter", C.c_int32), ("check_every", C.c_int32),
                ("restart_sufficient", C.c_double), ("restart_necessary", C.c_double),
                ("restart_artificial", C.c_double), ("pid_kp", C.c_double), ("max_dlog_weight", C.c_double),
                ("step_scale", C.c_double), ("weight_guard", C.c_double), ("jump_steady", C.c_double), ("jump_tol", C.c_double),
                ("jump_min", C.c_double), ("ray_jumps", C.c_int32), ("ruiz_iters", C.c_int32),
                ("waves_per_block", C.c_int32), ("kkt_every", C.c_int32), ("no_matreg", C.c_int32), ("geo_iters", C.c_int32),
                ("kkt_gate", C.c_double), ("stall_rescue", C.c_int32), ("no_simplex", C.c_int32),
                ("jump_rel", C.c_double), ("precision", C.c_int32), ("polish_patience", C.c_int32), ("no_rtc", C.c_int32), ("no_interior_point", C.c_int32),
                ("eps_infeasible", C.c_double), ("recertify_passes", C.c_int32), ("simplex_warm", C.c_int32), ("warm_patience", C.c_int32)]


class DspBatch(C.Structure):
    _fields_ = [("B", C.c_int32), ("reserved", C.c_int32),
                ("c", C.c_void_p), ("c_stride", C.c_int64),
                ("var_lb", C.c_void_p), ("var_lb_stride", C.c_int64),
                ("var_ub", C.c_void_p), ("var_ub_stride", C.c_int64),
                ("row_lb", C.c_void_p), ("row_lb_stride", C.c_int64),
                ("row_ub", C.c_void_p), ("row_ub_stride", C.c_int64),
                ("obj_offset", C.c_void_p), ("obj_offset_stride", C.c_int64),
                ("row_compliance", C.c_void_p), ("row_compliance_stride", C.c_int64),
                ("x0", C.c_void_p), ("y0", C.c_void_p), ("primal_weight", C.c_void_p),
                ("x", C.c_void_p), ("y", C.c_void_p), ("obj", C.c_void_p),
                ("status", C.c_void_p), ("iters", C.c_void_p), ("jumps", C.c_void_p), ("flags", C.c_void_p)]


class DspStats(C.Structure):
    _fields_ = [("total_iterations", C.c_int64), ("max_iterations", C.c_int32), ("n_optimal", C.c_int32),
                ("grid_blocks", C.c_int32), ("block_threads", C.c_int32), ("lds_bytes", C.c_int32),
                ("cols_per_lane", C.c_int32), ("rows_per_lane", C.c_int32), ("kernel_ms", C.c_float),
                ("matreg", C.c_int32), ("lds_conflicts_identity", C.c_int32), ("lds_conflicts_chosen", C.c_int32),
                ("simplex", C.c_int32), ("streaming", C.c_int32), ("stream_bytes_per_iteration", C.c_int64),
                ("quadratic", C.c_int32), ("precision", C.c_int32), ("rtc", C.c_int32), ("stream_form", C.c_int32), ("stream_phases", C.c_int32),
                ("ipm_solved", C.c_int32), ("reserved1", C.c_int32)]


class DspLpDesc(C.Structure):
    _fields_ = [("n", C.c_int32), ("m", C.c_int32), ("nnz", C.c_int64),
                ("A_rowptr", C.POINTER(C.c_int32)), ("A_colidx", C.POINTER(C.c_int32)),
                ("A_val", C.POINTER(C.c_double)), ("col_scale", C.POINTER(C.c_double))]


class DspWbModel(C.Structure):
    _fields_ = [("c", C.c_void_p), ("lb", C.c_void_p), ("ub", C.c_void_p), ("rlo", C.c_void_p), ("rhi", C.c_void_p),
                ("base_c", C.c_void_p), ("x", C.c_void_p),
                ("n", C.c_int32), ("m", C.c_int32), ("T", C.c_int32),
                ("soc_init", C.c_int32), ("thr_init", C.c_int32), ("soc0", C.c_int32), ("thr0", C.c_int32),
                ("wind_cols", C.c_int32 * 8), ("pt_cols", (C.c_int32 * 2) * 8), ("pda_cols", C.c_int32 * 8),
                ("track_rows", C.c_int32 * 8), ("wind_kw", C.c_double),
                ("c0", C.c_void_p), ("c0_base", C.c_double), ("waste_per_kw", C.c_double),
                ("status", C.c_void_p), ("flags", C.c_void_p)]


class DspWbState(C.Structure):
    _fields_ = [("B", C.c_int32), ("N", C.c_int32), ("start", C.c_void_p), ("hour", C.c_void_p),
                ("da_series", C.c_void_p), ("rt_series", C.c_void_p), ("cf_series", C.c_void_p),
                ("soc", C.c_void_p), ("thr", C.c_void_p), ("da_offer", C.c_void_p), ("da_prices", C.c_void_p),
                ("delivered", C.c_void_p), ("revenue", C.c_void_p), ("energy_mwh", C.c_void_p),
                ("bad", C.c_void_p), ("uncertified", C.c_void_p)]


class DspLoopModel(C.Structure):
    _fields_ = [("c", C.c_void_p), ("lb", C.c_void_p), ("ub", C.c_void_p), ("rlo", C.c_void_p), ("rhi", C.c_void_p),
                ("base_c", C.c_void_p), ("x", C.c_void_p), ("c0", C.c_void_p),
                ("n", C.c_int32), ("m", C.c_int32), ("T", C.c_int32), ("n_state", C.c_int32),
                ("pt_cols", (C.c_int32 * 2) * 16), ("pt_coef", (C.c_double * 2) * 16), ("pt_const", C.c_double * 16),
                ("pda_cols", C.c_int32 * 16), ("track_rows", C.c_int32 * 16), ("wind_cols", C.c_int32 * 16),
                ("state_init", C.c_int32 * 2), ("state_real", C.c_int32 * 2),
                ("wind_kw", C.c_double), ("c0_base", C.c_double), ("waste_per_kw", C.c_double),
                ("status", C.c_void_p), ("flags", C.c_void_p), ("wind_kw_plant", C.c_void_p), ("c0_base_plant", C.c_void_p)]


class DspLoopState(C.Structure):
    _fields_ = [("B", C.c_int32), ("N", C.c_int32), ("start", C.c_void_p), ("hour", C.c_void_p),
                ("da_series", C.c_void_p), ("rt_series", C.c_void_p), ("cf_series", C.c_void_p),
                ("state", C.c_void_p), ("state_scale", C.c_double * 2), ("da_offer", C.c_void_p), ("da_prices", C.c_void_p),
                ("delivered", C.c_void_p), ("revenue", C.c_void_p), ("energy_mwh", C.c_void_p),
                ("bad", C.c_void_p), ("uncertified", C.c_void_p)]


EXPORTED_SYMBOLS = ("dsp_default_options", "dsp_create", "dsp_solve", "dsp_spmv_step", "dsp_get_dims",
                    "dsp_get_scaling", "dsp_destroy", "dsp_strerror", "dsp_last_hip_error", "dsp_version",
                    "dsp_rtc_compile_check", "dsp_rtc_message", "dsp_wb_rolling_update", "dsp_loop_update", "dsp_bid_points", "dsp_source_hash",
                    "dsp_market_prepare", "dsp_market_clear", "dsp_loop_market_prepare", "dsp_loop_market_clear", "dsp_loop_param_step", "dsp_loop_project",
                    "dsp_loop_schedule_prepare", "dsp_loop_monotone_prepare", "dsp_loop_ledger", "dsp_loop_record")


ABI_VERSION = 21


BID_MAX_HOURS, BID_MAX_SCENARIOS = 64, 16384


class DspBidRequest(C.Structure):
    _fields_ = [("B", C.c_int32), ("T", C.c_int32), ("ldx", C.c_int32), ("ldp", C.c_int32), ("terms", C.c_int32), ("reserved", C.c_int32),
                ("x", C.c_void_p), ("price", C.c_void_p), ("ok", C.c_void_p), ("out", C.c_void_p), ("p_min", C.c_double),
                ("col", (C.c_int32 * 2) * BID_MAX_HOURS), ("val", (C.c_double * 2) * BID_MAX_HOURS), ("constant", C.c_double * BID_MAX_HOURS)]


MARKET_MAX_T, MARKET_MAX_S = 48, 16


class DspMarketModel(C.Structure):
    _fields_ = [("c", C.c_void_p), ("lb", C.c_void_p), ("ub", C.c_void_p), ("base_c", C.c_void_p), ("x", C.c_void_p), ("c0", C.c_void_p),
                ("status", C.c_void_p), ("flags", C.c_void_p),
                ("n", C.c_int32), ("T", C.c_int32), ("soc_init", C.c_int32), ("thr_init", C.c_int32),
                ("wind_cols", C.c_int32 * MARKET_MAX_T), ("pt_cols", (C.c_int32 * 2) * MARKET_MAX_T), ("pda_cols", C.c_int32 * MARKET_MAX_T),
                ("wind_kw", C.c_double), ("c0_base", C.c_double), ("waste_per_kw", C.c_double)]


class DspMarketState(C.Structure):
    _fields_ = [("B", C.c_int32), ("S", C.c_int32), ("D", C.c_int32), ("N", C.c_int32), ("backcast", C.c_int32), ("price_taker", C.c_int32),
                ("start", C.c_void_p), ("hour", C.c_void_p),
                ("da_series", C.c_void_p), ("rt_series", C.c_void_p), ("cf_series", C.c_void_p),
                ("soc", C.c_void_p), ("thr", C.c_void_p), ("da_offer", C.c_void_p), ("da_prices", C.c_void_p),
                ("bad", C.c_void_p), ("uncertified", C.c_void_p)]


class DspLoopMarketModel(C.Structure):
    _fields_ = [("c", C.c_void_p), ("lb", C.c_void_p), ("ub", C.c_void_p), ("base_c", C.c_void_p), ("x", C.c_void_p), ("c0", C.c_void_p),
                ("status", C.c_void_p), ("flags", C.c_void_p),
                ("n", C.c_int32), ("T", C.c_int32), ("n_state", C.c_int32), ("row_stride", C.c_int32),
                ("pt_cols", (C.c_int32 * 2) * MARKET_MAX_T), ("pt_coef", (C.c_double * 2) * MARKET_MAX_T), ("pt_const", C.c_double * MARKET_MAX_T),
                ("pda_cols", C.c_int32 * MARKET_MAX_T), ("wind_cols", C.c_int32 * MARKET_MAX_T), ("state_init", C.c_int32 * 2),
                ("wind_kw", C.c_double), ("c0_base", C.c_double), ("waste_per_kw", C.c_double),
                ("wind_kw_plant", C.c_void_p), ("c0_base_plant", C.c_void_p)]


class DspLoopMarketState(C.Structure):
    _fields_ = [("B", C.c_int32), ("S", C.c_int32), ("D", C.c_int32), ("N", C.c_int32), ("backcast", C.c_int32), ("price_taker", C.c_int32),
                ("start", C.c_void_p), ("hour", C.c_void_p),
                ("da_series", C.c_void_p), ("rt_series", C.c_void_p), ("cf_series", C.c_void_p),
                ("state", C.c_void_p), ("da_offer", C.c_void_p), ("da_prices", C.c_void_p),
                ("bad", C.c_void_p), ("uncertified", C.c_void_p), ("p_min_cents", C.c_int64),
                ("rt_history_lag_days", C.c_int32), ("self_schedule", C.c_int32), ("curve_slots", C.c_int32), ("coupled", C.c_int32),
                ("p_min_cents_plant", C.c_void_p)]


class DspLoopParamState(C.Structure):
    _fields_ = [("B", C.c_int32), ("N", C.c_int32), ("price_taker", C.c_int32), ("battery", C.c_int32),
                ("start", C.c_void_p), ("hour", C.c_void_p),
                ("da_series", C.c_void_p), ("rt_series", C.c_void_p), ("da_cf_series", C.c_void_p), ("rt_cf_series", C.c_void_p),
                ("state", C.c_void_p), ("bid_price", C.c_void_p), ("storage_mw", C.c_void_p), ("wind_mw", C.c_double),
                ("da_offer", C.c_void_p), ("da_prices", C.c_void_p), ("da_curve", C.c_void_p), ("da_count", C.c_void_p),
                ("rt_dispatch", C.c_void_p), ("rt_curve", C.c_void_p), ("rt_count", C.c_void_p),
                ("h2_kg", C.c_void_p), ("h2_mul", C.c_double), ("h2_div", C.c_double), ("pem_col", C.c_int32), ("reserved", C.c_int32)]


class DspLoopProjectState(C.Structure):
    _fields_ = [("B", C.c_int32), ("N", C.c_int32), ("ruc_hour", C.c_int32), ("slots", C.c_int32),
                ("start", C.c_void_p), ("hour", C.c_void_p), ("cf_series", C.c_void_p), ("state", C.c_void_p),
                ("state_scale", C.c_double * 2), ("obj", C.c_void_p),
                ("proj_state", C.c_void_p), ("proj_real", C.c_void_p), ("proj_obj", C.c_void_p),
                ("bad", C.c_void_p), ("uncertified", C.c_void_p),
                ("da_offer", C.c_void_p), ("da_prices", C.c_void_p), ("pend_offer", C.c_void_p), ("pend_prices", C.c_void_p),
                ("da_curve", C.c_void_p), ("da_count", C.c_void_p), ("pend_curve", C.c_void_p), ("pend_count", C.c_void_p)]


LEDGER_MAX_FORMS, LEDGER_MAX_TERMS = 8, 8


class DspLoopLedgerDesc(C.Structure):
    _fields_ = [("n_forms", C.c_int32), ("reserved", C.c_int32), ("n_terms", C.c_int32 * LEDGER_MAX_FORMS),
                ("cols", (C.c_int32 * LEDGER_MAX_TERMS) * LEDGER_MAX_FORMS), ("per_avail", C.c_double * LEDGER_MAX_FORMS),
                ("coef", C.c_void_p), ("constant", C.c_void_p), ("coef_stride", C.c_int64), ("const_stride", C.c_int64),
                ("acc", C.c_void_p), ("hour_value", C.c_void_p)]


RECORD_MAX_PLANTS, RECORD_MAX_SEGMENTS, RECORD_MAX_WIDTH = 64, 16, 1 << 20


class DspLoopRecordSegment(C.Structure):
    _fields_ = [("src", C.c_void_p), ("dst", C.c_void_p), ("plant_stride", C.c_int64), ("elem_stride", C.c_int64),
                ("width", C.c_int32), ("elem_bytes", C.c_int32)]


class DspLoopRecordDesc(C.Structure):
    _fields_ = [("n_plants", C.c_int32), ("n_segments", C.c_int32), ("plants", C.c_int32 * RECORD_MAX_PLANTS), ("clock", C.c_void_p),
                ("divisor", C.c_int32), ("offset", C.c_int32), ("rows", C.c_int32), ("reserved", C.c_int32),
                ("segments", DspLoopRecordSegment * RECORD_MAX_SEGMENTS)]


def source_hash(root: Optional[str] = None) -> Optional[str]:
    import glob
    import hashlib
    root = root or os.path.dirname(_HERE)
    csrc = os.path.join(root, "dispatches_amd", "csrc")
    files = sorted(glob.glob(os.path.join(csrc, "*.hip")) + glob.glob(os.path.join(csrc, "*.hpp")), key=os.path.basename)
    hdr = os.path.join(root, "include", "dsp_hip.h")
    if not files or not os.path.exists(hdr):
        return None
    h = hashlib.sha256()
    for f in files + [hdr]:
        h.update(os.path.basename(f).encode())
        with open(f, "rb") as fh:
            h.update(fh.read())
    return h.hexdigest()[:16]


def load_library(path: Optional[str] = None):
    global _lib
    if _lib is not None and path is None:
        return _lib
    path = path or _LIB_PATH
    if not os.path.exists(path):
        raise RuntimeError(f"{path} not found: build the HIP extension first (python -c 'import __graft_entry__ as g; g.build()')")
    try:
        import torch
    except Exception:
        pass
    lib = C.CDLL(path)
    lib.dsp_version.restype = C.c_int
    if not hasattr(lib, "dsp_source_hash"):
        raise RuntimeError(f"{path} predates ABI 9 (no dsp_source_hash): rebuild (python -c 'import __graft_entry__ as g; g.build(force=True)')")
    lib.dsp_source_hash.restype = C.c_char_p
    if lib.dsp_version() != ABI_VERSION:
        raise RuntimeError(f"{path} has ABI version {lib.dsp_version()}, this binding mirrors include/dsp_hip.h version "
                           f"{ABI_VERSION}: rebuild (python -c 'import __graft_entry__ as g; g.build(force=True)')")
    want, have = source_hash(), lib.dsp_source_hash().decode()
    if want is not None and have != want and "DSP_LIB" not in os.environ and os.environ.get("DSP_ALLOW_STALE_LIB") != "1":
        raise RuntimeError(f"{path} was built from other sources (library {have}, tree {want}): rebuild "
                           f"(python -c 'import __graft_entry__ as g; g.build()')")
    missing = [name for name in EXPORTED_SYMBOLS if not hasattr(lib, name)]
    if missing:
        raise RuntimeError(f"{path} lacks {missing}: rebuild (python -c 'import __graft_entry__ as g; g.build(force=True)')")
    vp, i32, i64, dp = C.c_void_p, C.c_int32, C.c_int64, C.c_void_p
    lib.dsp_default_options.argtypes = [C.POINTER(DspOptions)]
    lib.dsp_default_options.restype = None
    lib.dsp_create.argtypes = [C.POINTER(DspLpDesc), C.c_int, C.POINTER(DspOptions), C.POINTER(vp)]
    lib.dsp_create.restype = C.c_int
    lib.dsp_solve.argtypes = [vp, C.POINTER(DspBatch), C.POINTER(DspOptions), C.POINTER(DspStats), C.c_int, vp]
    lib.dsp_solve.restype = C.c_int
    lib.dsp_spmv_step.argtypes = [vp, i32, dp, dp, dp, dp, vp]
    lib.dsp_spmv_step.restype = C.c_int
    lib.dsp_get_dims.argtypes = [vp, C.POINTER(i32), C.POINTER(i32), C.POINTER(i64)]
    lib.dsp_get_dims.restype = C.c_int
    lib.dsp_get_scaling.argtypes = [vp, dp, dp, C.POINTER(C.c_double)]
    lib.dsp_get_scaling.restype = C.c_int
    lib.dsp_destroy.argtypes = [vp]
    lib.dsp_destroy.restype = C.c_int
    lib.dsp_strerror.argtypes = [C.c_int]
    lib.dsp_strerror.restype = C.c_char_p
    lib.dsp_rtc_compile_check.argtypes = [C.c_int, C.c_int, C.c_int, C.c_uint, C.c_uint, C.c_int, C.c_char_p, C.c_int]
    lib.dsp_rtc_compile_check.restype = C.c_int
    lib.dsp_rtc_message.argtypes = [vp]
    lib.dsp_rtc_message.restype = C.c_char_p
    lib.dsp_wb_rolling_update.argtypes = [C.POINTER(DspWbState), C.POINTER(DspWbModel), C.POINTER(DspWbModel), i32, i32, vp]
    lib.dsp_wb_rolling_update.restype = C.c_int
    lib.dsp_loop_update.argtypes = [C.POINTER(DspLoopState), C.POINTER(DspLoopModel), C.POINTER(DspLoopModel), i32, i32, vp]
    lib.dsp_loop_update.restype = C.c_int
    lib.dsp_bid_points.argtypes = [C.POINTER(DspBidRequest), vp]
    lib.dsp_bid_points.restype = C.c_int
    lib.dsp_market_prepare.argtypes = [C.POINTER(DspMarketState), C.POINTER(DspMarketModel), i32, vp]
    lib.dsp_market_prepare.restype = C.c_int
    lib.dsp_market_clear.argtypes = [C.POINTER(DspMarketState), C.POINTER(DspMarketModel), C.POINTER(DspWbModel), i32, i32, vp, vp, vp, vp]
    lib.dsp_market_clear.restype = C.c_int
    lib.dsp_loop_market_prepare.argtypes = [C.POINTER(DspLoopMarketState), C.POINTER(DspLoopMarketModel), i32, vp]
    lib.dsp_loop_market_prepare.restype = C.c_int
    lib.dsp_loop_market_clear.argtypes = [C.POINTER(DspLoopMarketState), C.POINTER(DspLoopMarketModel), C.POINTER(DspLoopModel), i32, i32, vp, vp, vp, vp]
    lib.dsp_loop_market_clear.restype = C.c_int
    lib.dsp_loop_schedule_prepare.argtypes = [C.POINTER(DspLoopMarketState), C.POINTER(DspLoopMarketModel), vp]
    lib.dsp_loop_schedule_prepare.restype = C.c_int
    lib.dsp_loop_monotone_prepare.argtypes = [C.POINTER(DspLoopMarketState), C.POINTER(DspLoopMarketModel), vp, vp, i32, i32, vp]
    lib.dsp_loop_monotone_prepare.restype = C.c_int
    lib.dsp_loop_param_step.argtypes = [C.POINTER(DspLoopParamState), C.POINTER(DspLoopModel), i32, i32, vp]
    lib.dsp_loop_param_step.restype = C.c_int
    lib.dsp_loop_project.argtypes = [C.POINTER(DspLoopProjectState), C.POINTER(DspLoopModel), i32, i32, vp]
    lib.dsp_loop_project.restype = C.c_int
    lib.dsp_loop_ledger.argtypes = [C.POINTER(DspLoopState), C.POINTER(DspLoopModel), C.POINTER(DspLoopLedgerDesc), vp]
    lib.dsp_loop_ledger.restype = C.c_int
    lib.dsp_loop_record.argtypes = [C.POINTER(DspLoopRecordDesc), i32, vp]
    lib.dsp_loop_record.restype = C.c_int
    lib.dsp_last_hip_error.restype = C.c_int
    if path == _LIB_PATH:
        _lib = lib
    return lib


class DspError(RuntimeError):
    pass


def _check(lib, rc, what):
    if rc != 0:
        raise DspError(f"{what} failed: {lib.dsp_strerror(rc).decode()} (code {rc}, hip error {lib.dsp_last_hip_error()})")


def default_options(**overrides) -> DspOptions:
    lib = load_library()
    o = DspOptions()
    lib.dsp_default_options(C.byref(o))
    env = {}
    for item in filter(None, os.environ.get("DSP_OPTIONS", "").split(",")):
        k, _, v = item.partition("=")
        env[k.strip()] = type(getattr(o, k.strip(), 0.0))(float(v))
    for k, v in {**env, **overrides}.items():
        if not hasattr(o, k):
            raise TypeError(f"unknown solver option {k!r}")
        setattr(o, k, v)
    return o


class DeviceLP:

    def __init__(self, lp, device: int = 0, options: Optional[DspOptions] = None):
        import torch

        if not torch.cuda.is_available():
            raise DspError("no MI355X visible: the dispatch solver has no CPU path")
        self.lib = load_library()
        self.lp = lp
        self.device = device
        self._rowptr = np.ascontiguousarray(lp.indptr, np.int32)
        self._colidx = np.ascontiguousarray(lp.indices, np.int32)
        self._val = np.ascontiguousarray(lp.data, np.float64)
        cs = getattr(lp, "col_scale", None)
        self._col_scale = None if cs is None else np.ascontiguousarray(cs, np.float64)
        desc = DspLpDesc(lp.n, lp.m, int(self._rowptr[-1]),
                         self._rowptr.ctypes.data_as(C.POINTER(C.c_int32)),
                         self._colidx.ctypes.data_as(C.POINTER(C.c_int32)),
                         self._val.ctypes.data_as(C.POINTER(C.c_double)),
                         None if self._col_scale is None else self._col_scale.ctypes.data_as(C.POINTER(C.c_double)))
        h = C.c_void_p()
        torch.cuda.set_device(device)
        _check(self.lib, self.lib.dsp_create(C.byref(desc), device, C.byref(options) if options else None, C.byref(h)),
               "dsp_create")
        self.handle = h
        self.options = options
        self.last_stats: Optional[DspStats] = None

    def close(self):
        if getattr(self, "handle", None):
            self.lib.dsp_destroy(self.handle)
            self.handle = None

    def __del__(self):
        try:
            self.close()
        except Exception:
            pass

    def scaling(self):
        dr = np.zeros(self.lp.m)
        dc = np.zeros(self.lp.n)
        eta = C.c_double()
        _check(self.lib, self.lib.dsp_get_scaling(self.handle, dr.ctypes.data, dc.ctypes.data, C.byref(eta)), "dsp_get_scaling")
        return dr, dc, eta.value

    @staticmethod
    def _ptr_stride(t, width):
        if t is None:
            return None, 0
        assert t.is_cuda and t.dtype.is_floating_point and t.element_size() == 8 and t.is_contiguous()
        if t.dim() == 1:
            assert t.shape[0] == width
            return t.data_ptr(), 0
        assert t.shape[1] == width
        return t.data_ptr(), width

    def solve(self, B, c, lb=None, ub=None, rlo=None, rhi=None, x0=None, y0=None, options=None, out=None,
              sync_stats=True, obj_offset=None, primal_weight=None, row_compliance=None):
        import torch

        n, m = self.lp.n, self.lp.m
        dev = torch.device("cuda", self.device)
        if out is None:
            out = dict(x=torch.empty((B, n), dtype=torch.float64, device=dev),
                       y=torch.empty((B, max(m, 1)), dtype=torch.float64, device=dev),
                       obj=torch.empty(B, dtype=torch.float64, device=dev),
                       status=torch.empty(B, dtype=torch.int32, device=dev),
                       iters=torch.empty(B, dtype=torch.int32, device=dev),
                       jumps=torch.empty(B, dtype=torch.int32, device=dev),
                       flags=torch.zeros(B, dtype=torch.int32, device=dev))
        bt = DspBatch()
        bt.B = B
        bt.c, bt.c_stride = self._ptr_stride(c, n)
        bt.var_lb, bt.var_lb_stride = self._ptr_stride(lb, n)
        bt.var_ub, bt.var_ub_stride = self._ptr_stride(ub, n)
        bt.row_lb, bt.row_lb_stride = self._ptr_stride(rlo, m)
        bt.row_ub, bt.row_ub_stride = self._ptr_stride(rhi, m)
        if obj_offset is not None:
            assert obj_offset.is_cuda and obj_offset.element_size() == 8 and obj_offset.numel() in (1, B)
            bt.obj_offset, bt.obj_offset_stride = obj_offset.data_ptr(), (1 if obj_offset.numel() == B and B > 1 else 0)
        if row_compliance is not None:
            bt.row_compliance, bt.row_compliance_stride = self._ptr_stride(row_compliance, m)
        bt.x0 = x0.data_ptr() if x0 is not None else None
        bt.y0 = y0.data_ptr() if y0 is not None else None
        if primal_weight is not None:
            assert primal_weight.is_cuda and primal_weight.element_size() == 8 and primal_weight.numel() == B
            bt.primal_weight = primal_weight.data_ptr()
        bt.x, bt.y, bt.obj = out["x"].data_ptr(), out["y"].data_ptr(), out["obj"].data_ptr()
        bt.status, bt.iters = out["status"].data_ptr(), out["iters"].data_ptr()
        bt.jumps = out["jumps"].data_ptr() if "jumps" in out else None
        bt.flags = out["flags"].data_ptr() if "flags" in out else None
        stats = DspStats()
        stream = torch.cuda.current_stream(dev).cuda_stream
        rc = self.lib.dsp_solve(self.handle, C.byref(bt), C.byref(options) if options is not None else None,
                                C.byref(stats), 1 if sync_stats else 0, C.c_void_p(stream))
        _check(self.lib, rc, "dsp_solve")
        self.last_stats = stats
        out["stats"] = stats
        return out

    def spmv_step(self, X, Y, AX=None, ATY=None):
        import torch

        B = X.shape[0]
        AX = torch.empty((B, self.lp.m), dtype=torch.float64, device=X.device) if AX is None else AX
        ATY = torch.empty((B, self.lp.n), dtype=torch.float64, device=X.device) if ATY is None else ATY
        stream = torch.cuda.current_stream(X.device).cuda_stream
        _check(self.lib, self.lib.dsp_spmv_step(self.handle, B, X.data_ptr(), Y.data_ptr(), AX.data_ptr(),
                                                ATY.data_ptr(), C.c_void_p(stream)), "dsp_spmv_step")
        return AX, ATY


def period_shift_maps(lp, shift: int):
    import re

    cache = lp.__dict__.setdefault("_shift_maps", {})
    if shift not in cache:
        def build(names):
            pat = re.compile(r"^(.*)\[(\d+)\]$")
            where = {}
            parsed = []
            for k, nm in enumerate(names):
                mt = pat.match(nm)
                parsed.append((mt.group(1), int(mt.group(2))) if mt else None)
                if mt:
                    where[(mt.group(1), int(mt.group(2)))] = k
            return np.array([where.get((p[0], p[1] + shift), k) if p else k for k, p in enumerate(parsed)], np.int64)
        cache[shift] = (build(lp.col_names), build(lp.row_names))
    return cache[shift]


FLAG_OBJ_WAIVED = 1
STATUS_PRIMAL_INFEASIBLE, STATUS_DUAL_INFEASIBLE = 2, 3
STATUS_UNCERTIFIED = 5


def uncertified(status, flags):
    status = np.asarray(status)
    if flags is None:
        return np.zeros(status.shape, bool)
    return (status == 0) & ((np.asarray(flags) & FLAG_OBJ_WAIVED) != 0)


class DeviceSolution:

    def __init__(self, out, m, device, price_windows=()):
        self.x, self.y, self.m, self.device = out["x"], out["y"], m, device
        self.price_windows = price_windows

    def fetch(self):
        import torch
        hx = torch.empty(self.x.shape, dtype=self.x.dtype, pin_memory=True)
        hy = torch.empty(self.y.shape, dtype=self.y.dtype, pin_memory=True)
        hx.copy_(self.x, non_blocking=True)
        hy.copy_(self.y, non_blocking=True)
        torch.cuda.current_stream(self.device).synchronize()
        return hx.numpy(), hy.numpy()[:, :self.m]

    def columns(self, cols):
        import torch
        idx = torch.as_tensor(np.ascontiguousarray(cols, np.int64), device=self.x.device)
        return self.x.index_select(1, idx).cpu().numpy()

    def rows(self, lo, hi):
        return self.x[lo:hi].cpu().numpy()

    def device_prices(self, prices):
        import torch
        for host, dev in self.price_windows:
            if host is prices:
                return dev
        return torch.as_tensor(np.ascontiguousarray(prices, np.float64), device=self.x.device)

    def bid_points(self, cols, vals, const, terms, prices, p_min, ok=None):
        import torch
        B, T = self.x.shape[0], len(const)
        if B > BID_MAX_SCENARIOS or T > BID_MAX_HOURS or B < 1 or T < 1:
            return None
        lib = load_library()
        dev = self.x.device
        pd = prices if isinstance(prices, torch.Tensor) else self.device_prices(prices)
        okd = None if ok is None else torch.as_tensor(np.ascontiguousarray(ok, np.uint8), device=dev)
        out = torch.empty((T, B + 1), dtype=torch.int64, device=dev)
        rq = DspBidRequest()
        rq.B, rq.T, rq.ldx, rq.ldp, rq.terms = B, T, self.x.stride(0), pd.stride(0), int(terms)
        rq.x, rq.price, rq.ok, rq.out, rq.p_min = self.x.data_ptr(), pd.data_ptr(), (okd.data_ptr() if okd is not None else None), out.data_ptr(), float(p_min)
        C.memmove(rq.col, np.ascontiguousarray(cols, np.int32).ctypes.data, 8 * T)
        C.memmove(rq.val, np.ascontiguousarray(vals, np.float64).ctypes.data, 16 * T)
        C.memmove(rq.constant, np.ascontiguousarray(const, np.float64).ctypes.data, 8 * T)
        stream = torch.cuda.current_stream(dev)
        _check(lib, lib.dsp_bid_points(C.byref(rq), C.c_void_p(stream.cuda_stream)), "dsp_bid_points")
        host = torch.empty((T, B + 1), dtype=torch.int64, pin_memory=True)
        host.copy_(out, non_blocking=True)
        stream.synchronize()
        keys = host.numpy()
        halves = keys[:, 1:].view(np.int32)
        return keys[:, 0].astype(np.int64), halves[:, 1::2], halves[:, 0::2]


class HipPdlpSolver:

    supports_warm_start = True

    RECERTIFY_VARIANTS = (dict(pid_kp=0.45, restart_artificial=0.3), dict(pid_kp=0.8, restart_artificial=0.15),
                          dict(pid_kp=0.3, restart_artificial=0.5, check_every=12))

    def __init__(self, device: int = 0, recertify: int = 3, lazy_solution: bool = True, **options):
        self.device = device
        self.lazy_solution = bool(lazy_solution)
        self.recertify = max(0, min(int(recertify), len(self.RECERTIFY_VARIANTS)))
        self._option_overrides = options
        self.options = None
        self.last_stats = None
        self.last_recertified = 0

    def available(self, exception_flag=False):
        try:
            import torch
            load_library()
            ok = torch.cuda.is_available()
        except Exception:
            ok = False
        if not ok and exception_flag:
            raise DspError("HIP dispatch solver unavailable (library not built or no GPU)")
        return ok

    def _device_lp(self, model) -> DeviceLP:
        if self.options is None:
            self.options = default_options(**self._option_overrides)
        h = model.solve_handle
        if h is None or h.lp is not model.lp:
            hints = dict(getattr(model, "solver_hints", None) or {})
            hints.update(self._option_overrides)
            h = DeviceLP(model.lp, self.device, default_options(**hints))
            model.solve_handle = h
        return h

    def _recertify(self, dlp, inputs, out, host, idx):
        import torch

        dev = torch.device("cuda", self.device)
        certified = 0
        todo = np.asarray(idx)
        for variant in self.RECERTIFY_VARIANTS[:self.recertify]:
            if not len(todo):
                break
            opts = DspOptions.from_buffer_copy(dlp.options)
            for k, v in variant.items():
                setattr(opts, k, v)
# ... 106 lines not shown
```

### dispatches_amd/rolling.py

```python
from __future__ import annotations

import numpy as np

from . import scenarios
from ._device_loop import _DeviceLoop, _NoSolver, attach_solver


class _DeviceModel:

    def __init__(self, model, B, dev, device_index, hints=None, lp_backend=None, waste_cost_per_kw=None, cf_template_sum=0.0):
        import torch
        self.lp = model.lp
        self.c0 = None
        if waste_cost_per_kw is not None:
            self.c0 = torch.zeros(B, dtype=torch.float64, device=dev)
            base = float(model.base_c0) if hasattr(model, "base_c0") else float(np.asarray(model.c0).ravel()[0])
            self._c0_base = base - float(waste_cost_per_kw) * float(model.block.windBattery["wind_kw"]) * float(cf_template_sum)
            self._waste_per_kw = float(waste_cost_per_kw)
        self.T = len(model.HOUR)
        t = lambda a, dt=torch.float64: torch.as_tensor(np.ascontiguousarray(a), dtype=dt, device=dev)
        lb, ub, rlo, rhi = model.block.current_bounds()
        self.c = t(model.base_c if hasattr(model, "base_c") else model.c[0]).repeat(B, 1)
        self.base_c = self.c[0].clone()
        self.lb, self.ub = t(lb).repeat(B, 1), t(ub).repeat(B, 1)
        self.rlo, self.rhi = t(rlo).repeat(B, 1), t(rhi).repeat(B, 1)
        fam = model.block.windBattery
        per = fam["periods"]
        idx = lambda cols: torch.as_tensor(np.asarray(cols, np.int64), device=dev)
        self.wind_cols = idx([p["wind"].index for p in per])
        self.soc_init, self.thr_init = fam["soc_init"].index, fam["thr_init"].index
        self.soc0, self.thr0 = per[0]["state_of_charge"].index, getattr(per[0]["energy_throughput"], "index", None)
        self.wind_kw = float(fam["wind_kw"])
        self.pt_cols = idx([[p["grid_elec"].index, p["elec_out"].index] for p in per])
        attach_solver(self, B, dev, device_index, hints, lp_backend)

    def wb_struct(self, needs_state=True):
        from .hip_solver import DspWbModel
        w = DspWbModel()
        w.c, w.lb, w.ub, w.rlo, w.rhi = (t.data_ptr() for t in (self.c, self.lb, self.ub, self.rlo, self.rhi))
        w.base_c, w.x = self.base_c.data_ptr(), self.out["x"].data_ptr()
        w.n, w.m, w.T = self.lp.n, self.lp.m, self.T
        if self.thr0 is None and needs_state:
            raise ValueError("this model holds period 0's throughput as an expression (two-level accumulator): it cannot hand the "
                             "realised state to the fused rolling-update kernel")
        w.soc_init, w.thr_init, w.soc0, w.thr0 = self.soc_init, self.thr_init, self.soc0, (self.thr_init if self.thr0 is None else self.thr0)
        wc, pt = self.wind_cols.cpu().tolist(), self.pt_cols.cpu().tolist()
        pda = self.pda_cols.cpu().tolist() if hasattr(self, "pda_cols") else []
        trk = self.track_rows.cpu().tolist() if hasattr(self, "track_rows") else []
        for t in range(8):
            w.wind_cols[t] = wc[t] if t < len(wc) else -1
            w.pt_cols[t][0], w.pt_cols[t][1] = (pt[t] if t < len(pt) else (-1, -1))
            w.pda_cols[t] = pda[t] if t < len(pda) else -1
            w.track_rows[t] = trk[t] if t < len(trk) else -1
        w.wind_kw = self.wind_kw
        if self.c0 is not None:
            w.c0, w.c0_base, w.waste_per_kw = self.c0.data_ptr(), self._c0_base, self._waste_per_kw
        w.status, w.flags = self.out["status"].data_ptr(), self.out["flags"].data_ptr()
        return w

    def market_struct(self):
        from .hip_solver import DspMarketModel
        w = DspMarketModel()
        w.c, w.lb, w.ub, w.base_c, w.x = (t.data_ptr() for t in (self.c, self.lb, self.ub, self.base_c, self.out["x"]))
        w.c0 = self.c0.data_ptr()
        w.status, w.flags = self.out["status"].data_ptr(), self.out["flags"].data_ptr()
        w.n, w.T, w.soc_init, w.thr_init = self.lp.n, self.T, self.soc_init, self.thr_init
        wc, pt, pda = self.wind_cols.cpu().tolist(), self.pt_cols.cpu().tolist(), self.pda_cols.cpu().tolist()
        for t in range(self.T):
            w.wind_cols[t], w.pda_cols[t] = wc[t], pda[t]
            w.pt_cols[t][0], w.pt_cols[t][1] = pt[t]
        w.wind_kw, w.c0_base, w.waste_per_kw = self.wind_kw, self._c0_base, self._waste_per_kw
        return w

    def power_output(self, x):
        return 1e-3 * x[:, self.pt_cols].sum(dim=2)

    def solve(self, B, x0=None, y0=None, primal_weight=None, hour=None):
        opts = self.opts if (hour is None or self.opts is None) else (self.opts_first if hour == 0 else self.opts_warm)
        self.out = self.dlp.solve(B, self.c, self.lb, self.ub, self.rlo if self.lp.m else None,
                                  self.rhi if self.lp.m else None, x0=x0, y0=y0, primal_weight=primal_weight,
                                  options=opts, out=self.out, sync_stats=False, obj_offset=self.c0)
        return self.out


class BatchedWindBatteryDoubleLoop(_DeviceLoop):
    def __init__(self, n_scenarios, device=0, first_scenario=0, series="rts_gmlc_309.npz", stride=17,
                 day_ahead_horizon=48, real_time_horizon=4, tracking_horizon=4, wind_mw=200.0, batt_mw=25.0,
                 price_cap=500.0, warm_start=True, lp_backend=None, use_graphs=True, use_fused=True, record=None, simplex_warm=True, warm_patience=10000,
                 n_price_scenarios=1, forecaster="perfect", max_historical_days=10, market="stub"):
        import torch
        from .workflow import Tracker
        self.B = B = int(n_scenarios)
        self.S = S = int(n_price_scenarios)
        self.D = D = int(max_historical_days)
        self._check_market_arguments(forecaster, market, S, D)
        self.forecaster, self.market = forecaster, market
        self.stochastic = forecaster != "perfect" or market != "stub"
        rows = B * S
        self.dev = dev = torch.device("cuda", device) if lp_backend is None else torch.device("cpu")
        s = scenarios.load_series(series)
        self.N = N = len(s["rt_lmp"])
        if self.stochastic and (24 * D > N or tracking_horizon > real_time_horizon):
            raise ValueError("the stochastic mode needs max_historical_days whole days inside the series and tracking_horizon <= real_time_horizon")
        t = lambda a: torch.as_tensor(np.ascontiguousarray(a, np.float64), device=dev)
        self.da_series = t(np.clip(s["da_lmp"], 0.0, price_cap))
        self.rt_series = t(np.clip(s["rt_lmp"], 0.0, price_cap))
        self.cf_series = t(s["rt_cf"])
        ids = first_scenario + np.arange(B)
        self.start = torch.as_tensor((stride * ids) % N, dtype=torch.int64, device=dev)
        self.T_da, self.T_rt, self.T_tr = day_ahead_horizon, real_time_horizon, tracking_horizon
        bidder, da_model = scenarios.wind_battery_batch(1, day_ahead_horizon, _NoSolver(), series=series, stride=stride,
                                                        wind_mw=wind_mw, batt_mw=batt_mw, price_cap=price_cap)
        rt_model = bidder.real_time_model
        if real_time_horizon != 4:
            raise NotImplementedError("real_time_horizon is 4 in every reference driver")
        tracker = Tracker(tracking_model_object=bidder.bidding_model_object.__class__(
            model_data=bidder.bidding_model_object.model_data, wind_capacity_factors=list(s["rt_cf"][:tracking_horizon]),
            wind_pmax_mw=wind_mw, battery_pmax_mw=batt_mw, battery_energy_capacity_mwh=4 * batt_mw),
            tracking_horizon=tracking_horizon, n_tracking_hour=1, solver=_NoSolver())
        tracker._pass_market_dispatch([0.0] * tracking_horizon)
        tr_model = tracker.model
        self.penalty = float(bidder.real_time_underbid_penalty)
        self.da = _DeviceModel(da_model, rows, dev, device, hints=getattr(da_model, "solver_hints", None), lp_backend=lp_backend,
                               waste_cost_per_kw=bidder.bidding_model_object.wind_waste_penalty * 1e-3,
                               cf_template_sum=float(np.sum(s["rt_cf"][:day_ahead_horizon])))
        waste = bidder.bidding_model_object.wind_waste_penalty * 1e-3
        self.rt = _DeviceModel(rt_model, rows, dev, device, hints=getattr(rt_model, "solver_hints", None), lp_backend=lp_backend,
                               waste_cost_per_kw=waste, cf_template_sum=float(np.sum(s["rt_cf"][:real_time_horizon])))
        self.tr = _DeviceModel(tr_model, B, dev, device, hints=getattr(tr_model, "solver_hints", None), lp_backend=lp_backend,
                               waste_cost_per_kw=waste, cf_template_sum=float(np.sum(s["rt_cf"][:tracking_horizon])))
        if self.tr.thr0 is None:
            raise ValueError("the tracking model must carry period 0's throughput as a column: the loop reads the realised state from it")
        idx = lambda cols: torch.as_tensor(np.asarray(cols, np.int64), device=dev)
        self.da.pda_cols, self.rt.pda_cols = idx(da_model.pda_cols), idx(rt_model.pda_cols)
        self.da.u_cols, self.rt.u_cols = (idx([v.index for v in mm.real_time_underbid_power]) for mm in (da_model, rt_model))
        self.rt_periods, self.tr_periods = rt_model.block.windBattery["periods"], tr_model.block.windBattery["periods"]
        self.da_periods = da_model.block.windBattery["periods"]
        from .hip_solver import period_shift_maps
        self.weight_only = warm_start == "weight"
        self.warm_start = bool(warm_start) and not self.weight_only and day_ahead_horizon > 24
        cmap, rmap = period_shift_maps(da_model.lp, 24)
        self.da_cmap, self.da_rmap = idx(cmap), idx(rmap)
        if self.warm_start:
            if lp_backend is None and self.da.opts is not None:
                import os
                self.da.opts.warm_patience = int(os.environ.get("DSP_WARM_PATIENCE", warm_patience))
            self.da_x0 = torch.zeros((rows, da_model.lp.n), dtype=torch.float64, device=dev)
            self.da_y0 = torch.zeros((rows, max(da_model.lp.m, 1)), dtype=torch.float64, device=dev)
        self.tr.track_rows = idx([tr_model.block.kept_row_index(r) for r in tr_model.tracking_rows])
        self.tr.c[:] = t(tr_model.c[0])
        z = lambda: torch.zeros(B, dtype=torch.float64, device=dev)
        self.soc, self.thr = z(), z()
        self.revenue, self.energy_mwh, self.da_energy_mwh = z(), z(), z()
        self.bad = torch.zeros((), dtype=torch.bool, device=dev)
        self.uncertified = torch.zeros((), dtype=torch.int64, device=dev)
        self.hour = 0
        self.hour_t = torch.zeros((), dtype=torch.int64, device=dev)
        self._clk = self.hour_t
        self.da_offer = torch.zeros((B, 24), dtype=torch.float64, device=dev)
        self.da_prices = torch.zeros((B, 24), dtype=torch.float64, device=dev)
        self.da_pw = torch.zeros(rows, dtype=torch.float64, device=dev)
        self.delivered = z()
        self._hundred = torch.full((), 100.0, dtype=torch.float64, device=dev)
        self.solves = 0
        self.use_graphs = bool(use_graphs) and lp_backend is None
        self.simplex_warm = bool(simplex_warm) and lp_backend is None
        self.use_fused = bool(use_fused) and lp_backend is None and real_time_horizon <= 8 and tracking_horizon <= 8
        if self.stochastic:
            from .hip_solver import MARKET_MAX_T
            self.use_fused = self.use_fused and day_ahead_horizon <= MARKET_MAX_T
            i32 = lambda *shape: torch.zeros(shape, dtype=torch.int32, device=dev)
            self.da_curve, self.da_count = i32(B, 24, S + 1, 2), i32(B, 24)
            self.rt_curve, self.rt_count = i32(B, tracking_horizon, S + 1, 2), i32(B, tracking_horizon)
            self.rt_dispatch = torch.zeros((B, tracking_horizon), dtype=torch.float64, device=dev)
            self.offered_mwh = z()
        if self.use_fused:
            from .hip_solver import DspWbState, load_library
            self._lib = load_library()
            st = DspWbState()
            st.B, st.N = B, N
            st.start, st.hour = self.start.data_ptr(), self.hour_t.data_ptr()
            st.da_series, st.rt_series, st.cf_series = self.da_series.data_ptr(), self.rt_series.data_ptr(), self.cf_series.data_ptr()
            st.soc, st.thr = self.soc.data_ptr(), self.thr.data_ptr()
            st.da_offer, st.da_prices = self.da_offer.data_ptr(), self.da_prices.data_ptr()
            st.delivered, st.revenue, st.energy_mwh = self.delivered.data_ptr(), self.revenue.data_ptr(), self.energy_mwh.data_ptr()
            st.bad, st.uncertified = self.bad.data_ptr(), self.uncertified.data_ptr()
            self._wb_state, self._wb_rt, self._wb_tr = st, self.rt.wb_struct(needs_state=False), self.tr.wb_struct()
            if self.stochastic:
                from .hip_solver import DspMarketState
                mk = DspMarketState()
                mk.B, mk.S, mk.D, mk.N = B, S, D, N
                mk.backcast, mk.price_taker = int(forecaster == "backcast"), int(market == "price_taker")
                for name in ("start", "hour", "da_series", "rt_series", "cf_series", "soc", "thr", "da_offer", "da_prices", "bad", "uncertified"):
                    setattr(mk, name, getattr(st, name))
                self._mk_state, self._mk_da, self._mk_rt = mk, self.da.market_struct(), self.rt.market_struct()
        self._graphs = {}
        self._rec = None
        if record is not None:
            plants, days = record
            R, H = len(plants), 24 * int(days)
            buf = lambda *shape: torch.zeros(shape, dtype=torch.float64, device=dev)
            sc = (S,) if self.stochastic else ()
            self._rec = dict(plants=idx(plants), days=int(days),
                             state=buf(H + 1, R, 2), rt_x=buf(H + 1, R, *sc, self.rt.lp.n), tr_x=buf(H + 1, R, self.tr.lp.n),
                             rt_obj=buf(H + 1, R, *sc), tr_obj=buf(H + 1, R),
                             da_state=buf(int(days) + 1, R, 2), da_x=buf(int(days) + 1, R, *sc, self.da.lp.n), da_obj=buf(int(days) + 1, R, *sc))
            if self.stochastic:
                ibuf = lambda *shape: torch.zeros(shape, dtype=torch.int32, device=dev)
                Dn, Ttr = int(days) + 1, tracking_horizon
                self._rec.update(da_curve=ibuf(Dn, R, 24, S + 1, 2), da_count=ibuf(Dn, R, 24), da_dispatch=buf(Dn, R, 24),
                                 rt_curve=ibuf(H + 1, R, Ttr, S + 1, 2), rt_count=ibuf(H + 1, R, Ttr), rt_dispatch=buf(H + 1, R, Ttr))
            self._day_t = torch.zeros((), dtype=torch.int64, device=dev)
            self._limit_h = torch.full((), H, dtype=torch.int64, device=dev)
            self._limit_d = torch.full((), int(days), dtype=torch.int64, device=dev)

    def _record(self, what, value, daily=False):
        import torch
        r = self._rec
        at = torch.minimum(torch.div(self.hour_t, 24, rounding_mode="floor"), self._limit_d) if daily else torch.minimum(self.hour_t, self._limit_h)
        r[what].index_copy_(0, at.view(1), value.index_select(0, r["plants"]).unsqueeze(0))

    def recorded(self):
        r = self._rec
        H, D = min(self.hour, 24 * r["days"]), min(self.hour // 24, r["days"])
        out = {k: r[k][:H].cpu().numpy() for k in ("state", "rt_x", "tr_x", "rt_obj", "tr_obj")}
        out.update({k: r[k][:D].cpu().numpy() for k in ("da_state", "da_x", "da_obj")})
        if self.stochastic:
            out.update({k: r[k][:H].cpu().numpy() for k in ("rt_curve", "rt_count", "rt_dispatch")})
            out.update({k: r[k][:D].cpu().numpy() for k in ("da_curve", "da_count", "da_dispatch")})
        out["plants"] = r["plants"].cpu().numpy()
        return out

    def reset(self):
        for t in (self.soc, self.thr, self.revenue, self.energy_mwh, self.da_energy_mwh, self.da_pw, self.delivered, self.hour_t, self.uncertified,
                  self.da_offer, self.da_prices):
            t.zero_()
        self.bad.zero_()
        if self.stochastic:
            self.offered_mwh.zero_()
        if self.warm_start:
            self.da_x0.zero_(), self.da_y0.zero_()
        self.hour = self.solves = 0

    def _set_prices(self, m, da, rt):
        m.c[:] = m.base_c
        m.c[:, m.pt_cols[:, 0]] -= 1e-3 * rt
        m.c[:, m.pt_cols[:, 1]] -= 1e-3 * rt
        m.c[:, m.pda_cols] -= da - rt

    def _set_state(self, m):
        m.lb[:, m.soc_init] = self.soc
        m.ub[:, m.soc_init] = self.soc
        m.lb[:, m.thr_init] = self.thr
        m.ub[:, m.thr_init] = self.thr
        avail = m.wind_kw * self._window(self.cf_series, m.T)
        m.ub[:, m.wind_cols] = avail
        if m.c0 is not None:
            total = avail[:, 0]
            for t in range(1, m.T):
                total = total + avail[:, t]
            m.c0.copy_(m._c0_base + m._waste_per_kw * total)

    def _day_ahead_step(self):
        import torch
        m = self.da
        da, rt = self._window(self.da_series, m.T), self._window(self.rt_series, m.T)
        self._set_prices(m, da, rt)
        self._set_state(m)
        self._free_day_ahead_power(m)
        if self.warm_start:
            out = m.solve(self.B, x0=self.da_x0, y0=self.da_y0, primal_weight=self.da_pw)
            torch.index_select(out["x"], 1, self.da_cmap, out=self.da_x0)
            torch.index_select(out["y"], 1, self.da_rmap, out=self.da_y0)
        else:
            if not self.weight_only:
                self.da_pw.zero_()
            out = m.solve(self.B, primal_weight=self.da_pw)
        self._check(out)
        if self._rec is not None:
            self._record("da_state", torch.stack([self.soc, self.thr], 1), daily=True)
            self._record("da_x", out["x"], daily=True)
            self._record("da_obj", out["obj"], daily=True)
        self.da_offer.copy_(out["x"][:, m.pda_cols][:, :24])
        self.da_prices.copy_(da[:, :24])
        self.da_energy_mwh += self.da_offer.sum(1)

    def _set_state_rows(self, m):
        soc, thr = self._rows(self.soc), self._rows(self.thr)
        m.lb[:, m.soc_init] = soc
        m.ub[:, m.soc_init] = soc
        m.lb[:, m.thr_init] = thr
        m.ub[:, m.thr_init] = thr
        avail = m.wind_kw * self._window(self.cf_series, m.T)
        m.ub[:, m.wind_cols] = self._rows(avail)
        total = avail[:, 0]
        for t in range(1, m.T):
            total = total + avail[:, t]
        m.c0.copy_(self._rows(m._c0_base + m._waste_per_kw * total))

    def _market(self, fn, *args):
        import ctypes as C
        self._call(fn, C.byref(self._mk_state), *args)

    def _day_ahead_step_stochastic(self):
        import ctypes as C
        import torch
        m, B, S = self.da, self.B, self.S
        if self.use_fused:
            self._market(self._lib.dsp_market_prepare, C.byref(self._mk_da), -1)
        else:
            da, rt = self._forecast(self.da_series, m.T, 0).expand(B, S, m.T), self._forecast(self.rt_series, m.T, 0).expand(B, S, m.T)
            self._set_prices(m, da.reshape(B * S, m.T), rt.reshape(B * S, m.T))
            self._set_state_rows(m)
            self._free_day_ahead_power(m)
        if self.warm_start:
            out = m.solve(B * S, x0=self.da_x0, y0=self.da_y0, primal_weight=self.da_pw)
            torch.index_select(out["x"], 1, self.da_cmap, out=self.da_x0)
            torch.index_select(out["y"], 1, self.da_rmap, out=self.da_y0)
        else:
            if not self.weight_only:
                self.da_pw.zero_()
            out = m.solve(B * S, primal_weight=self.da_pw)
        if self.use_fused:
            self._market(self._lib.dsp_market_clear, C.byref(self._mk_da), None, -1, 24, C.c_void_p(self.da_offer.data_ptr()),
                         C.c_void_p(self.da_curve.data_ptr()), C.c_void_p(self.da_count.data_ptr()))
        else:
            self._check(out)
            power = out["x"][:, m.pda_cols[:24]].reshape(B, S, 24)
            U, M, count = self._curves(power, self._forecast(self.da_series, 24, 0), out["status"])
            realised = self._window(self.da_series, 24)
            self.da_offer.copy_(self._clear(U, M, count, realised))
            self.da_prices.copy_(realised)
            self._store_curves(self.da_curve, self.da_count, U, M, count)
        if self._rec is not None:
            self._record("da_state", torch.stack([self.soc, self.thr], 1), daily=True)
            self._record("da_x", out["x"].reshape(B, S, -1), daily=True)
            self._record("da_obj", out["obj"].reshape(B, S), daily=True)
            for key, v in (("da_curve", self.da_curve), ("da_count", self.da_count), ("da_dispatch", self.da_offer)):
                self._record(key, v, daily=True)
        self._account_day_ahead()

    def _hour_step_stochastic(self, k):
        import ctypes as C
        import torch
        m, tr, B, S = self.rt, self.tr, self.B, self.S
        hour = k if self.simplex_warm else None
        if self._rec is not None:
            self._record("state", torch.stack([self.soc, self.thr], 1))
        if self.use_fused:
            self._market(self._lib.dsp_market_prepare, C.byref(self._mk_rt), k)
            m.solve(B * S, hour=hour)
            self._market(self._lib.dsp_market_clear, C.byref(self._mk_rt), C.byref(self._wb_tr), k, tr.T, C.c_void_p(self.rt_dispatch.data_ptr()),
                         C.c_void_p(self.rt_curve.data_ptr()), C.c_void_p(self.rt_count.data_ptr()))
            tr.solve(B, hour=hour)
        else:
            rt_f = self._forecast(self.rt_series, m.T, k).expand(B, S, m.T)
            da_f = self._forecast(self.da_series, m.T, k).expand(B, S, m.T).clone()
            known = min(m.T, 24 - k)
            da_f[:, :, :known] = self.da_prices[:, None, k:k + known]
            self._set_prices(m, da_f.reshape(B * S, m.T), rt_f.reshape(B * S, m.T))
            self._set_state_rows(m)
            self._free_day_ahead_power(m, k, S)
            out = m.solve(B * S, hour=hour)
            self._check(out)
            power = m.power_output(out["x"])[:, :tr.T].reshape(B, S, tr.T)
            U, M, count = self._curves(power, rt_f[:, :, :tr.T], out["status"])
            lmp = torch.cat([self._window(self.rt_series, 1), rt_f[:, 0, 1:tr.T]], dim=1)
            self.rt_dispatch.copy_(self._clear(U, M, count, lmp))
            self._store_curves(self.rt_curve, self.rt_count, U, M, count)
            self._set_state(tr)
            tr.rlo[:, tr.track_rows] = self.rt_dispatch
            tr.rhi[:, tr.track_rows] = self.rt_dispatch
            out = tr.solve(B, hour=hour)
            self._check(out)
        if self._rec is not None:
            self._record("rt_x", m.out["x"].reshape(B, S, -1))
            self._record("rt_obj", m.out["obj"].reshape(B, S))
            self._record("tr_x", tr.out["x"])
            self._record("tr_obj", tr.out["obj"])
            for key, v in (("rt_curve", self.rt_curve), ("rt_count", self.rt_count), ("rt_dispatch", self.rt_dispatch)):
                self._record(key, v)
        if self.use_fused:
            self._fused(2, k)
            return
        x = tr.out["x"]
        rt0 = self._window(self.rt_series, 1)[:, 0]
        self.delivered.copy_(tr.power_output(x)[:, 0])
        self.soc.copy_(torch.round(x[:, tr.soc0] * 100.0) / self._hundred)
        self.thr.copy_(torch.round(x[:, tr.thr0] * 100.0) / self._hundred)
        self.revenue += self.delivered * rt0 + self.da_offer[:, k] * (self.da_prices[:, k] - rt0)
        self.energy_mwh += self.delivered
        self.hour_t += 1

    def _fused(self, phase, k):
        import ctypes as C
        self._call(self._lib.dsp_wb_rolling_update, C.byref(self._wb_state), C.byref(self._wb_rt), C.byref(self._wb_tr), phase, k)

    def _hour_step(self, k):
        import torch
        if self.use_fused:
            if self._rec is not None:
                self._record("state", torch.stack([self.soc, self.thr], 1))
            self._fused(0, k)
            self.rt.solve(self.B, hour=k if self.simplex_warm else None)
            self._fused(1, k)
            self.tr.solve(self.B, hour=k if self.simplex_warm else None)
            if self._rec is not None:
                for key, m in (("rt", self.rt), ("tr", self.tr)):
                    self._record(key + "_x", m.out["x"])
                    self._record(key + "_obj", m.out["obj"])
            self._fused(2, k)
            return
        m = self.rt
        if self._rec is not None:
            self._record("state", torch.stack([self.soc, self.thr], 1))
        rt = self._window(self.rt_series, m.T)
        da = self._window(self.da_series, m.T).clone()
        known = min(m.T, 24 - k)
        da[:, :known] = self.da_prices[:, k:k + known]
        self._set_prices(m, da, rt)
        self._set_state(m)
        self._free_day_ahead_power(m, k)
        hour = k if self.simplex_warm else None
        out = m.solve(self.B, hour=hour)
        self._check(out)
        offer = m.power_output(out["x"])
        tr = self.tr
        self._set_state(tr)
        tr.rlo[:, tr.track_rows] = offer[:, :tr.T]
        tr.rhi[:, tr.track_rows] = offer[:, :tr.T]
        out = tr.solve(self.B, hour=hour)
        self._check(out)
        if self._rec is not None:
            for key, mm in (("rt", self.rt), ("tr", self.tr)):
                self._record(key + "_x", mm.out["x"])
                self._record(key + "_obj", mm.out["obj"])
        x = out["x"]
        self.delivered.copy_(tr.power_output(x)[:, 0])
        self.soc.copy_(torch.round(x[:, tr.soc0] * 100.0) / self._hundred)
        self.thr.copy_(torch.round(x[:, tr.thr0] * 100.0) / self._hundred)
        self.revenue += self.delivered * rt[:, 0] + self.da_offer[:, k] * (self.da_prices[:, k] - rt[:, 0])
        self.energy_mwh += self.delivered
        self.hour_t += 1

    def day_ahead(self):
        self.day_start = self.hour
        self._run("da", self._day_ahead_step_stochastic if self.stochastic else self._day_ahead_step)
        self.solves += self.B * self.S
        return self.da_offer.clone()

    def hour_step(self):
        k = self.hour - self.day_start
        self._run(k, (lambda: self._hour_step_stochastic(k)) if self.stochastic else (lambda: self._hour_step(k)))
        self.solves += self.B * self.S + self.B
        self.hour += 1
        return self.delivered.clone()

    def results(self):
        res = dict(obj=self.revenue, energy_mwh=self.energy_mwh, soc=self.soc, throughput=self.thr)
        if self.stochastic:
            res.update(da_energy_mwh=self.da_energy_mwh, offered_mwh=self.offered_mwh)
        return res, not bool(self.bad.item())


class PipelinedDoubleLoops:

    def __init__(self, n_scenarios, device=0, first_scenario=0, groups=0, record=None, **kw):
        import torch
        from .distributed import shard_bounds
        n = int(n_scenarios)
        G = int(groups) if groups and groups > 0 else (2 if n >= 1024 else 1)
        self.groups = G = max(1, min(G, max(n, 1)))
        self.dev = torch.device("cuda", device)
        cuts = [shard_bounds(n, G, g) for g in range(G)]
        rec = lambda b0, b1: None if record is None else ([p - b0 for p in record[0] if b0 <= p < b1], record[1])
        self.record_order = None if record is None else [p for b0, b1 in cuts for p in record[0] if b0 <= p < b1]
        self.loops = [BatchedWindBatteryDoubleLoop(b1 - b0, device=device, first_scenario=first_scenario + b0, record=rec(b0, b1), **kw) for b0, b1 in cuts]
        self.streams = [torch.cuda.Stream(device=self.dev) for _ in range(G)] if G > 1 else [None]

    def run_day(self):
        import torch
        if self.groups == 1:
            return self.loops[0].run_day()
        cur = torch.cuda.current_stream(self.dev)
        for loop, s in zip(self.loops, self.streams):
            s.wait_stream(cur)
            with torch.cuda.stream(s):
                loop.run_day()
        for s in self.streams:
            cur.wait_stream(s)

    def run_days(self, n, per_day=None):
        import torch
        if self.groups == 1:
            for _ in range(n):
                self.loops[0].run_day()
                if per_day is not None:
                    per_day(0, self.loops[0])
            return
        cur = torch.cuda.current_stream(self.dev)
        for s in self.streams:
            s.wait_stream(cur)
        for _ in range(n):
            for g, (loop, s) in enumerate(zip(self.loops, self.streams)):
                with torch.cuda.stream(s):
                    loop.run_day()
                    if per_day is not None:
                        per_day(g, loop)
        for s in self.streams:
            cur.wait_stream(s)

    def reset(self):
        for l in self.loops:
            l.reset()

    def recorded(self):
        parts = [l.recorded() for l in self.loops if l._rec is not None and len(l._rec["plants"])]
        out = {k: np.concatenate([p[k] for p in parts], axis=1) for k in parts[0] if k != "plants"}
        out["plants"] = np.asarray(self.record_order)
        return out

    @property
    def hour(self):
        return self.loops[0].hour

    @property
    def revenue(self):
        import torch
        return self.loops[0].revenue if self.groups == 1 else torch.cat([l.revenue for l in self.loops])

    @property
    def uncertified(self):
        return sum(l.uncertified for l in self.loops)

    @property
    def warm_start(self):
        return self.loops[0].warm_start

    def day_ahead_iterations(self):
        import torch
        return torch.cat([l.da.out["iters"] for l in self.loops])

    def results(self):
        import torch
        parts = [l.results() for l in self.loops]
        keys = parts[0][0].keys()
        return {k: torch.cat([p[0][k] for p in parts]) for k in keys}, all(p[1] for p in parts)
```

### include/dsp_hip.h

```cpp
#ifndef DSP_HIP_H
#define DSP_HIP_H

#ifndef __HIPCC_RTC__
#include <stdint.h>
#endif

#ifdef __cplusplus
extern "C" {
#endif

#define DSP_VERSION 21

#define DSP_OK                 0
#define DSP_ERR_INVALID       -1
#define DSP_ERR_TOO_LARGE     -2
#define DSP_ERR_HIP           -3
#define DSP_ERR_NO_DEVICE     -4
#define DSP_ERR_ALLOC         -5

#define DSP_STATUS_OPTIMAL            0
#define DSP_STATUS_ITERATION_LIMIT    1
#define DSP_STATUS_PRIMAL_INFEASIBLE  2
#define DSP_STATUS_DUAL_INFEASIBLE    3
#define DSP_STATUS_NUMERICAL          4

#define DSP_FLAG_OBJ_WAIVED   1
#define DSP_FLAG_STALL_RESCUE 2
#define DSP_FLAG_POLISH       4

typedef struct dsp_handle dsp_handle;

typedef struct dsp_lp_desc {
  int32_t n;
  int32_t m;
  int64_t nnz;
  const int32_t *A_rowptr;
  const int32_t *A_colidx;
  const double  *A_val;
  const double  *col_scale;
} dsp_lp_desc;

typedef struct dsp_options {
  double  eps_rel;
  double  eps_obj;
  int32_t max_iter;
  int32_t check_every;
  double  restart_sufficient;
  double  restart_necessary;
  double  restart_artificial;
  double  pid_kp;
  double  max_dlog_weight;
  double  step_scale;
  double  weight_guard;
  double  jump_steady;
  double  jump_tol;
  double  jump_min;
  int32_t ray_jumps;
  int32_t ruiz_iters;
  int32_t waves_per_block;
  int32_t kkt_every;
  int32_t no_matreg;
  int32_t geo_iters;
  double  kkt_gate;
  int32_t stall_rescue;
  int32_t no_simplex;
  double  jump_rel;
  int32_t precision;
  int32_t polish_patience;
  int32_t no_rtc;
  int32_t no_interior_point;
  double  eps_infeasible;
  int32_t recertify_passes;
  int32_t simplex_warm;
  int32_t warm_patience;
} dsp_options;

typedef struct dsp_batch {
  int32_t B;
  int32_t reserved;
  const double *c;          int64_t c_stride;
  const double *var_lb;     int64_t var_lb_stride;
  const double *var_ub;     int64_t var_ub_stride;
  const double *row_lb;     int64_t row_lb_stride;
  const double *row_ub;     int64_t row_ub_stride;
  const double *obj_offset; int64_t obj_offset_stride;
  const double *row_compliance; int64_t row_compliance_stride;
  const double *x0;
  const double *y0;
  double  *primal_weight;
  double  *x;
  double  *y;
  double  *obj;
  int32_t *status;
  int32_t *iters;
  int32_t *jumps;
  int32_t *flags;
} dsp_batch;

typedef struct dsp_stats {
  int64_t total_iterations;
  int32_t max_iterations;
  int32_t n_optimal;
  int32_t grid_blocks;
  int32_t block_threads;
  int32_t lds_bytes;
  int32_t cols_per_lane;
  int32_t rows_per_lane;
  float   kernel_ms;
  int32_t matreg;
  int32_t lds_conflicts_identity;
  int32_t lds_conflicts_chosen;
  int32_t simplex;
  int32_t streaming;
  int64_t stream_bytes_per_iteration;
  int32_t quadratic;
  int32_t precision;
  int32_t rtc;
  int32_t stream_form;
  int32_t stream_phases;
  int32_t ipm_solved;
  int32_t reserved1;
} dsp_stats;

#define DSP_STREAM_FORM_NONE       0
#define DSP_STREAM_FORM_TWO_LAUNCH 1
#define DSP_STREAM_FORM_TILE       2
#define DSP_STREAM_FORM_LANE       3
#define DSP_STREAM_FORM_BLOCK      4
#define DSP_STREAM_FORM_IPM        5

void dsp_default_options(dsp_options *opt);

int dsp_create(const dsp_lp_desc *desc, int device, const dsp_options *opt, dsp_handle **out);

int dsp_solve(dsp_handle *h, const dsp_batch *batch, const dsp_options *opt, dsp_stats *stats, int sync_stats,
              void *hipStream);

int dsp_spmv_step(dsp_handle *h, int32_t B, const double *X, const double *Y, double *AX, double *ATY,
                  void *hipStream);

typedef struct dsp_wb_model {
  double *c, *lb, *ub, *rlo, *rhi;
  const double *base_c;
  const double *x;
  int32_t n, m, T;
  int32_t soc_init, thr_init;
  int32_t soc0, thr0;
  int32_t wind_cols[8];
  int32_t pt_cols[8][2];
  int32_t pda_cols[8];
  int32_t track_rows[8];
  double wind_kw;
  double *c0;
  double c0_base, waste_per_kw;
  const int32_t *status, *flags;
} dsp_wb_model;

typedef struct dsp_wb_state {
  int32_t B, N;
  const int64_t *start;
  int64_t *hour;
  const double *da_series, *rt_series, *cf_series;
  double *soc, *thr;
  const double *da_offer, *da_prices;
  double *delivered, *revenue, *energy_mwh;
  uint8_t *bad;
  int64_t *uncertified;
} dsp_wb_state;

int dsp_wb_rolling_update(const dsp_wb_state *st, const dsp_wb_model *rt, const dsp_wb_model *tr, int32_t phase, int32_t k,
                          void *hipStream);

#define DSP_LOOP_MAX_T 16
typedef struct dsp_loop_model {
  double *c, *lb, *ub, *rlo, *rhi;
  const double *base_c;
  const double *x;
  double *c0;
  int32_t n, m, T, n_state;
  int32_t pt_cols[16][2];
  double  pt_coef[16][2];
  double  pt_const[16];
  int32_t pda_cols[16];
  int32_t track_rows[16];
  int32_t wind_cols[16];
  int32_t state_init[2], state_real[2];
  double  wind_kw, c0_base, waste_per_kw;
  const int32_t *status, *flags;
  const double *wind_kw_plant, *c0_base_plant;
} dsp_loop_model;

typedef struct dsp_loop_state {
  int32_t B, N;
  const int64_t *start;
  int64_t *hour;
  const double *da_series, *rt_series, *cf_series;
  double *state;
  double state_scale[2];
  const double *da_offer, *da_prices;
  double *delivered, *revenue, *energy_mwh;
  uint8_t *bad;
  int64_t *uncertified;
} dsp_loop_state;

int dsp_loop_update(const dsp_loop_state *st, const dsp_loop_model *rt, const dsp_loop_model *tr, int32_t phase, int32_t k, void *hipStream);

#define DSP_LEDGER_MAX_FORMS 8
#define DSP_LEDGER_MAX_TERMS 8
typedef struct dsp_loop_ledger_desc {
  int32_t n_forms, reserved;
  int32_t n_terms[8];
  int32_t cols[8][8];
  double  per_avail[8];
  const double *coef;
  const double *constant;
  int64_t coef_stride, const_stride;
  double *acc;
  double *hour_value;
} dsp_loop_ledger_desc;

int dsp_loop_ledger(const dsp_loop_state *st, const dsp_loop_model *tr, const dsp_loop_ledger_desc *ledger, void *hipStream);

#define DSP_RECORD_MAX_PLANTS 64
#define DSP_RECORD_MAX_SEGMENTS 16
#define DSP_RECORD_MAX_WIDTH 1048576
typedef struct dsp_loop_record_segment {
  const void *src;
  void *dst;
  int64_t plant_stride, elem_stride;
  int32_t width, elem_bytes;
} dsp_loop_record_segment;
typedef struct dsp_loop_record_desc {
  int32_t n_plants, n_segments;
  int32_t plants[64];
  const int64_t *clock;
  int32_t divisor, offset;
  int32_t rows, reserved;
  dsp_loop_record_segment segments[16];
} dsp_loop_record_desc;

int dsp_loop_record(const dsp_loop_record_desc *rec, int32_t B, void *hipStream);

#define DSP_BID_MAX_HOURS 64
#define DSP_BID_MAX_SCENARIOS 16384
typedef struct dsp_bid_request {
  int32_t B, T;
  int32_t ldx, ldp;
  int32_t terms;
  int32_t reserved;
  const double *x;
  const double *price;
  const uint8_t *ok;
  int64_t *out;
  double p_min;
  int32_t col[DSP_BID_MAX_HOURS][2];
  double val[DSP_BID_MAX_HOURS][2];
  double constant[DSP_BID_MAX_HOURS];
} dsp_bid_request;
int dsp_bid_points(const dsp_bid_request *rq, void *hipStream);

#define DSP_MARKET_MAX_T 48
#define DSP_MARKET_MAX_S 16
typedef struct dsp_market_model {
  double *c, *lb, *ub;
  const double *base_c;
  const double *x;
  double *c0;
  const int32_t *status, *flags;
  int32_t n, T;
  int32_t soc_init, thr_init;
  int32_t wind_cols[DSP_MARKET_MAX_T];
  int32_t pt_cols[DSP_MARKET_MAX_T][2];
  int32_t pda_cols[DSP_MARKET_MAX_T];
  double wind_kw, c0_base, waste_per_kw;
} dsp_market_model;

typedef struct dsp_market_state {
  int32_t B, S, D, N;
  int32_t backcast, price_taker;
  const int64_t *start;
  const int64_t *hour;
  const double *da_series, *rt_series, *cf_series;
  const double *soc, *thr;
  const double *da_offer;
  double *da_prices;
  uint8_t *bad;
  int64_t *uncertified;
} dsp_market_state;

int dsp_market_prepare(const dsp_market_state *st, const dsp_market_model *m, int32_t k, void *hipStream);

int dsp_market_clear(const dsp_market_state *st, const dsp_market_model *m, const dsp_wb_model *tr, int32_t k, int32_t T,
                     double *dispatch, int32_t *curve, int32_t *count, void *hipStream);

typedef struct dsp_loop_market_model {
  double *c, *lb, *ub;
  const double *base_c;
  const double *x;
  double *c0;
  const int32_t *status, *flags;
  int32_t n, T, n_state;
  int32_t row_stride;
  int32_t pt_cols[DSP_MARKET_MAX_T][2];
  double  pt_coef[DSP_MARKET_MAX_T][2];
  double  pt_const[DSP_MARKET_MAX_T];
  int32_t pda_cols[DSP_MARKET_MAX_T];
  int32_t wind_cols[DSP_MARKET_MAX_T];
  int32_t state_init[2];
  double wind_kw, c0_base, waste_per_kw;
  const double *wind_kw_plant, *c0_base_plant;
} dsp_loop_market_model;

typedef struct dsp_loop_market_state {
  int32_t B, S, D, N;
  int32_t backcast, price_taker;
  const int64_t *start;
  const int64_t *hour;
  const double *da_series, *rt_series, *cf_series;
  const double *state;
  const double *da_offer;
  double *da_prices;
  uint8_t *bad;
  int64_t *uncertified;
  int64_t p_min_cents;
  int32_t rt_history_lag_days;
// ... 75 lines not shown
```

Before: 4.670 million.

## Fold wind-battery rolling hand-off phases into simplex solve kernels

Moves the per-hour rolling update (phase0 price/bound writes, phase1 tracking-row setup, and the previous hour's settlement) out of separate kernel launches and into the warm simplex kernel through a WbHandOff argument. Settlement of an hour can be deferred and folded into the next hour's real-time solve, with the clock advanced in bulk by a lag counter. The aim is to remove small launches and serialization points between solves in the multi-period loop. In exchange it adds a second code path with deferred state, extra validation, and a larger simplex argument struct.

```diff
diff --git a/dispatches_amd/csrc/dsp_capi.hip b/dispatches_amd/csrc/dsp_capi.hip
--- a/dispatches_amd/csrc/dsp_capi.hip
+++ b/dispatches_amd/csrc/dsp_capi.hip
@@ -348,8 +348,8 @@
   return DSP_OK;
 }
 
-static int simplex_pass(dsp_handle *h, SolveArgs &a, hipStream_t st) {
-  if (!h->simplex || a.qp) return DSP_OK;
+static int simplex_pass(dsp_handle *h, SolveArgs &a, hipStream_t st, const WbHandOff *wb) {
+  if (!h->simplex || a.qp) return wb ? DSP_ERR_INVALID : DSP_OK;
   const int B = a.b.B;
   SimplexArgs sa{};
   sa.n = h->n; sa.m = h->m; sa.row_stride = h->sx_row_stride; sa.max_pivots = 20 * (h->n + h->m);
@@ -362,6 +362,7 @@
     sa.warm = a.opt.simplex_warm;
     sa.warm_T = h->sx_warm_T; sa.warm_basis = h->sx_warm_basis; sa.warm_upper = h->sx_warm_upper; sa.warm_valid = h->sx_warm_valid;
   }
+  if (wb) sa.wb = *wb;
   static const int sx_debug = getenv("DSP_SX_DEBUG") ? atoi(getenv("DSP_SX_DEBUG")) : 0;
   sa.debug_keep = sx_debug;
   const int per_cu = std::max<int>(1, std::min<int>(32, (int)((size_t)h->lds_limit / h->sx_lds)));
@@ -409,7 +410,7 @@
   return DSP_OK;
 }
 
-static int solve_fused(dsp_handle *h, const dsp_batch *batch, SolveArgs &a, dsp_stats *stats, bool timed, hipStream_t st) {
+static int solve_fused(dsp_handle *h, const dsp_batch *batch, SolveArgs &a, dsp_stats *stats, bool timed, hipStream_t st, const WbHandOff *wb = nullptr) {
   const int B = batch->B, qp = a.qp;
   if (qp && h->rtc_state[1] == -1) {
     h->rtc_state[1] = rtc_get_kernel(h->device, h->cpl, h->rpl, false, h->P.mr_wc_pack, h->P.mr_wr_pack, true, &h->rtc[1], &h->rtc_why) ? 1 : 0;
@@ -435,7 +436,7 @@
   const Followup f = followup_geometry(h, a.matreg && !qp && h->rtc_state[0] != 1 && h->light_lds > 0);
   if (a.matreg && a.opt.eps_infeasible > 0.0 && !f.wpb) a.opt.eps_infeasible = 0.0;
   if (timed) HIP_TRY(hipEventRecord(h->ev0, st));
-  if ((rc = simplex_pass(h, a, st)) != DSP_OK) return rc;
+  if ((rc = simplex_pass(h, a, st, wb)) != DSP_OK) return rc;
   HIP_TRY(first_pass(h, a, grid, geo.lds, st));
   if ((rc = certificate_pass(h, a, f, timed, st)) != DSP_OK || (rc = recertify_passes(h, a, f, st)) != DSP_OK) return rc;
   if (timed) HIP_TRY(hipEventRecord(h->ev1, st));
@@ -455,6 +456,20 @@
   stats->lds_conflicts_identity = h->lds_conflicts[0] + h->lds_conflicts[2];
   stats->lds_conflicts_chosen = a.matreg ? h->lds_conflicts[1] + h->lds_conflicts[3] : stats->lds_conflicts_identity;
   return finish_stats(h, batch, stats, timed, st);
+}
+
+int dsp::solve_with_hand_off(dsp_handle *h, const dsp_batch *batch, const dsp_options *opt, const WbHandOff &wb, hipStream_t st) {
+  if (!h || h->streaming || !h->simplex) return DSP_ERR_INVALID;
+  const dsp_wb_model &own = (wb.phases & DSP_WB_HAND_PHASE1) ? wb.tr : wb.rt;
+  if (own.n != h->n || own.m != h->m) return DSP_ERR_INVALID;
+  HIP_TRY(hipSetDevice(h->device));
+  SolveArgs a{};
+  if (int rc = resolve_options(h, batch, opt, &a)) return rc;
+  const int warm = (a.opt.simplex_warm == 1 || a.opt.simplex_warm == 2) ? a.opt.simplex_warm : 0;
+  if (a.qp || a.opt.precision != 0 || simplex_in_registers(warm, h->n, h->m, batch->B)) return DSP_ERR_INVALID;
+  dsp_stats stats;
+  std::memset(&stats, 0, sizeof(stats));
+  return solve_fused(h, batch, a, &stats, false, st, &wb);
 }
 
 extern "C" {
diff --git a/dispatches_amd/csrc/dsp_capi_internal.hpp b/dispatches_amd/csrc/dsp_capi_internal.hpp
--- a/dispatches_amd/csrc/dsp_capi_internal.hpp
+++ b/dispatches_amd/csrc/dsp_capi_internal.hpp
@@ -1,7 +1,10 @@
 #pragma once
 #include "dsp_device.hpp"
 
-namespace dsp { inline thread_local int g_last_hip_error = 0; }
+namespace dsp {
+inline thread_local int g_last_hip_error = 0;
+int solve_with_hand_off(dsp_handle *h, const dsp_batch *batch, const dsp_options *opt, const WbHandOff &wb, hipStream_t st);
+}
 
 #define HIP_TRY(expr)                                                                                            \
   do {                                                                                                           \
diff --git a/dispatches_amd/csrc/dsp_capi_loop.hip b/dispatches_amd/csrc/dsp_capi_loop.hip
--- a/dispatches_amd/csrc/dsp_capi_loop.hip
+++ b/dispatches_amd/csrc/dsp_capi_loop.hip
@@ -79,7 +79,57 @@
   if (!st || !rt || !tr || st->B < 0 || phase < 0 || phase > 2 || k < 0 || k > 23 || rt->T < 1 || rt->T > 8 || tr->T < 1 || tr->T > 8)
     return DSP_ERR_INVALID;
   if (st->B == 0) return DSP_OK;
-  HIP_TRY(launch_wb_rolling(*st, *rt, *tr, (int)phase, (int)k, (hipStream_t)hipStream));
+  HIP_TRY(launch_wb_rolling(*st, *rt, *tr, (int)phase, (int)k, 0, phase == 2 ? 1 : 0, (hipStream_t)hipStream));
+  return DSP_OK;
+}
+
+static bool wb_state_ok(const dsp_wb_state *st, bool phase2) {
+  if (!st || st->B < 0 || st->N < 1 || !st->start || !st->hour || !st->da_series || !st->rt_series || !st->cf_series) return false;
+  if (!st->soc || !st->thr || !st->da_offer || !st->da_prices) return false;
+  return !phase2 || (st->delivered && st->revenue && st->energy_mwh);
+}
+static bool wb_model_written_ok(const dsp_wb_model *m, bool rows) {
+  if (!m || m->n < 1 || m->m < 0 || m->T < 1 || m->T > 8 || !m->c || !m->lb || !m->ub || (rows && (!m->rlo || !m->rhi))) return false;
+  return loop_cols_ok(m->wind_cols, m->T, m->n) && market_col_ok(m->soc_init, m->n) && market_col_ok(m->thr_init, m->n);
+}
+static bool wb_power_cols_ok(const dsp_wb_model *m, int T) {
+  for (int t = 0; t < T; ++t)
+    if (!market_col_ok(m->pt_cols[t][0], m->n) || !market_col_ok(m->pt_cols[t][1], m->n)) return false;
+  return true;
+}
+static bool wb_settle_ok(const dsp_wb_state *st, const dsp_wb_model *tr, int k, int off) {
+  if (!wb_state_ok(st, true) || !tr || tr->n < 1 || !tr->x || tr->T < 1 || k < 0 || k > 23 || off < 0) return false;
+  return wb_power_cols_ok(tr, 1) && market_col_ok(tr->soc0, tr->n) && market_col_ok(tr->thr0, tr->n);
+}
+static bool wb_batch_is_model(const dsp_batch *b, const dsp_wb_model *m, bool rows) {
+  if (b->c != m->c || b->var_lb != m->lb || b->var_ub != m->ub || b->c_stride != m->n || b->var_lb_stride != m->n || b->var_ub_stride != m->n) return false;
+  return !rows || (b->row_lb == m->rlo && b->row_ub == m->rhi && b->row_lb_stride == m->m && b->row_ub_stride == m->m);
+}
+
+int dsp_wb_hour_solve(dsp_handle *h, const dsp_batch *batch, const dsp_options *opt, const dsp_wb_state *st, const dsp_wb_model *rt,
+                      const dsp_wb_model *tr, int32_t phases, int32_t k, int32_t off, void *hipStream) {
+  const bool p0 = phases == DSP_WB_HAND_PHASE0 || phases == (DSP_WB_HAND_PHASE0 | DSP_WB_HAND_PHASE2_PREV);
+  const bool p1 = phases == DSP_WB_HAND_PHASE1, p2 = p0 && (phases & DSP_WB_HAND_PHASE2_PREV);
+  if (!h || !batch || !st || !rt || !tr || !(p0 || p1) || k < 0 || k > 23 || off < 0) return DSP_ERR_INVALID;
+  if (batch->B != st->B || !batch->c || !batch->x || !batch->y || !batch->obj || !batch->status || !wb_state_ok(st, p2)) return DSP_ERR_INVALID;
+  if (p0) {
+    if (!wb_model_written_ok(rt, false) || !rt->base_c || !loop_cols_ok(rt->pda_cols, rt->T, rt->n) || !wb_power_cols_ok(rt, rt->T)) return DSP_ERR_INVALID;
+    if (!wb_batch_is_model(batch, rt, false)) return DSP_ERR_INVALID;
+    if (p2 && (k < 1 || off < 1 || !wb_settle_ok(st, tr, k - 1, off - 1))) return DSP_ERR_INVALID;
+  } else {
+    if (!wb_model_written_ok(tr, true) || tr->m < 1 || !loop_cols_ok(tr->track_rows, tr->T, tr->m) || !wb_batch_is_model(batch, tr, true)) return DSP_ERR_INVALID;
+    if (rt->n < 1 || !rt->x || rt->T < tr->T || rt->T > 8 || !wb_power_cols_ok(rt, tr->T)) return DSP_ERR_INVALID;
+  }
+  if (st->B == 0) return DSP_OK;
+  WbHandOff wb{*st, *rt, *tr, (int)k, (int)off, (int)phases};
+  return solve_with_hand_off(h, batch, opt, wb, (hipStream_t)hipStream);
+}
+
+int dsp_wb_hour_settle(const dsp_wb_state *st, const dsp_wb_model *rt, const dsp_wb_model *tr, int32_t k, int32_t off, int32_t advance,
+                       void *hipStream) {
+  if (!rt || advance < 0 || !wb_settle_ok(st, tr, k, off)) return DSP_ERR_INVALID;
+  if (st->B == 0) return DSP_OK;
+  HIP_TRY(launch_wb_rolling(*st, *rt, *tr, 2, (int)k, (int)off, (int)advance, (hipStream_t)hipStream));
   return DSP_OK;
 }
 
diff --git a/dispatches_amd/csrc/dsp_device.hpp b/dispatches_amd/csrc/dsp_device.hpp
--- a/dispatches_amd/csrc/dsp_device.hpp
+++ b/dispatches_amd/csrc/dsp_device.hpp
@@ -112,6 +112,14 @@
     ((unsigned long long)DSP_VERSION << 8) ^ kBuildSwitches ^ ((unsigned long long)__builtin_offsetof(SolveArgs, anchor_w) << 4) ^
     ((unsigned long long)rare_lds_bytes(0) << 20);
 
+struct WbHandOff {
+  dsp_wb_state s;
+  dsp_wb_model rt, tr;
+  int k;
+  int off;
+  int phases;
+};
+
 struct SimplexArgs {
   int n, m;
   int row_stride;
@@ -127,7 +135,10 @@
   int *warm_basis;
   unsigned char *warm_upper;
   int *warm_valid;
+  WbHandOff wb;
 };
+
+inline bool simplex_in_registers(int warm, int n, int m, int B) { return !warm && m <= 24 && n + m <= 64 && B <= 2048; }
 
 struct SpmvArgs {
   DeviceProblem P;
@@ -150,7 +161,8 @@
 hipError_t launch_simplex(const SimplexArgs &a, int grid, size_t lds, hipStream_t st);
 hipError_t launch_solve_f32(int cpl, int rpl, const SolveArgs &a, int num_cus, size_t lds_limit, hipStream_t st, int *grid,
                             int *threads, size_t *lds);
-hipError_t launch_wb_rolling(const dsp_wb_state &st, const dsp_wb_model &rt, const dsp_wb_model &tr, int phase, int k, hipStream_t stream);
+hipError_t launch_wb_rolling(const dsp_wb_state &st, const dsp_wb_model &rt, const dsp_wb_model &tr, int phase, int k, int off, int advance,
+                             hipStream_t stream);
 hipError_t launch_loop_update(const dsp_loop_state &st, const dsp_loop_model &rt, const dsp_loop_model &tr, int phase, int k, hipStream_t stream);
 hipError_t launch_loop_ledger(const dsp_loop_state &st, const dsp_loop_model &tr, const dsp_loop_ledger_desc &ledger, hipStream_t stream);
 hipError_t launch_loop_record(const dsp_loop_record_desc &rec, hipStream_t stream);
diff --git a/dispatches_amd/csrc/dsp_loop.hip b/dispatches_amd/csrc/dsp_loop.hip
--- a/dispatches_amd/csrc/dsp_loop.hip
+++ b/dispatches_amd/csrc/dsp_loop.hip
@@ -5,72 +5,16 @@
 
 using namespace dsp;
 
-template <class M, class S>
-__device__ __forceinline__ void loop_check(const S &s, const M &m, int b) {
-  if (m.status && s.bad && m.status[b] != 0) *s.bad = 1;
-  if (m.flags && s.uncertified && (m.flags[b] & DSP_FLAG_OBJ_WAIVED)) atomicAdd(reinterpret_cast<unsigned long long *>(s.uncertified), 1ull);
+__global__ void __launch_bounds__(256) wb_rolling_kernel(dsp_wb_state s, dsp_wb_model rt, dsp_wb_model tr, int phase, int k, int off) {
+  const int b = blockIdx.x * blockDim.x + threadIdx.x;
+  if (b >= s.B) return;
+  const long long h = *s.hour + off;
+  if (phase == 0) wb_phase0<1>(s, rt, k, h, b, 0);
+  else if (phase == 1) wb_phase1<1>(s, rt, tr, h, b, 0);
+  else wb_phase2(s, tr, k, h, b);
 }
 
-__global__ void __launch_bounds__(256) wb_rolling_kernel(dsp_wb_state s, dsp_wb_model rt, dsp_wb_model tr, int phase, int k) {
-  const int b = blockIdx.x * blockDim.x + threadIdx.x;
-  if (b >= s.B) return;
-  const long long h = *s.hour, st0 = s.start[b];
-  auto win = [&](const double *series, int t) { return series[(st0 + h + t) % s.N]; };
-  if (phase == 0) {
-    const dsp_wb_model &m = rt;
-    const int known = min(m.T, 24 - k);
-    double *c = m.c + (size_t)b * m.n, *lb = m.lb + (size_t)b * m.n, *ub = m.ub + (size_t)b * m.n;
-    double avail_sum = 0.0;
-    for (int t = 0; t < m.T; ++t) {
-      const double rtp = win(s.rt_series, t);
-      const double dap = t < known ? s.da_prices[(size_t)b * 24 + k + t] : win(s.da_series, t);
-      const double r3 = loop_opaque(__dmul_rn(1e-3, rtp));
-      c[m.pt_cols[t][0]] = __dsub_rn(m.base_c[m.pt_cols[t][0]], r3);
-      c[m.pt_cols[t][1]] = __dsub_rn(m.base_c[m.pt_cols[t][1]], r3);
-      c[m.pda_cols[t]] = __dsub_rn(m.base_c[m.pda_cols[t]], loop_opaque(__dsub_rn(dap, rtp)));
-      const double avail = __dmul_rn(m.wind_kw, win(s.cf_series, t));
-      ub[m.wind_cols[t]] = avail;
-      avail_sum = t ? __dadd_rn(avail_sum, avail) : avail;
-      const double fix = t < known ? s.da_offer[(size_t)b * 24 + k + t] : 0.0;
-      lb[m.pda_cols[t]] = fix;
-      ub[m.pda_cols[t]] = t < known ? fix : INFINITY;
-    }
-    if (m.c0) m.c0[b] = __dadd_rn(m.c0_base, loop_opaque(__dmul_rn(m.waste_per_kw, avail_sum)));
-    lb[m.soc_init] = s.soc[b]; ub[m.soc_init] = s.soc[b];
-    lb[m.thr_init] = s.thr[b]; ub[m.thr_init] = s.thr[b];
-  } else if (phase == 1) {
-    loop_check(s, rt, b);
-    const double *xr = rt.x + (size_t)b * rt.n;
-    double *lb = tr.lb + (size_t)b * tr.n, *ub = tr.ub + (size_t)b * tr.n;
-    double *rlo = tr.rlo + (size_t)b * tr.m, *rhi = tr.rhi + (size_t)b * tr.m;
-    double avail_sum = 0.0;
-    for (int t = 0; t < tr.T; ++t) {
-      const double offer = __dmul_rn(1e-3, loop_opaque(__dadd_rn(xr[rt.pt_cols[t][0]], xr[rt.pt_cols[t][1]])));
-      rlo[tr.track_rows[t]] = offer;
-      rhi[tr.track_rows[t]] = offer;
-      const double avail = __dmul_rn(tr.wind_kw, win(s.cf_series, t));
-      ub[tr.wind_cols[t]] = avail;
-      avail_sum = t ? __dadd_rn(avail_sum, avail) : avail;
-    }
-    if (tr.c0) tr.c0[b] = __dadd_rn(tr.c0_base, loop_opaque(__dmul_rn(tr.waste_per_kw, avail_sum)));
-    lb[tr.soc_init] = s.soc[b]; ub[tr.soc_init] = s.soc[b];
-    lb[tr.thr_init] = s.thr[b]; ub[tr.thr_init] = s.thr[b];
-  } else {
-    loop_check(s, tr, b);
-    const double *x = tr.x + (size_t)b * tr.n;
-    const double delivered = loop_opaque(__dmul_rn(1e-3, loop_opaque(__dadd_rn(x[tr.pt_cols[0][0]], x[tr.pt_cols[0][1]]))));
-    const double rt0 = win(s.rt_series, 0);
-    s.delivered[b] = delivered;
-    s.soc[b] = __ddiv_rn(rint(loop_opaque(__dmul_rn(x[tr.soc0], 100.0))), 100.0);
-    s.thr[b] = __ddiv_rn(rint(loop_opaque(__dmul_rn(x[tr.thr0], 100.0))), 100.0);
-    const double dao = s.da_offer[(size_t)b * 24 + k], dap = s.da_prices[(size_t)b * 24 + k];
-    const double t1 = loop_opaque(__dmul_rn(delivered, rt0)), t2 = loop_opaque(__dmul_rn(dao, loop_opaque(__dsub_rn(dap, rt0))));
-    s.revenue[b] = __dadd_rn(s.revenue[b], loop_opaque(__dadd_rn(t1, t2)));
-    s.energy_mwh[b] = __dadd_rn(s.energy_mwh[b], delivered);
-  }
-}
-
-__global__ void wb_clock_kernel(long long *hour) { *hour += 1; }
+__global__ void wb_clock_kernel(long long *hour, int hours) { *hour += hours; }
 
 __device__ __forceinline__ double loop_power(const dsp_loop_model &m, const double *x, int t) {
   double p = m.pt_const[t];
@@ -190,17 +134,18 @@
   return hipGetLastError();
 }
 
-template <class K, class S, class M>
-static hipError_t launch_hand_off(K kernel, const S &st, const M &rt, const M &tr, int phase, int k, hipStream_t stream) {
-  hipLaunchKernelGGL(kernel, dim3((st.B + 255) / 256), dim3(256), 0, stream, st, rt, tr, phase, k);
-  if (phase == 2) hipLaunchKernelGGL(wb_clock_kernel, dim3(1), dim3(1), 0, stream, (long long *)st.hour);
+template <class K, class S, class M, class... Extra>
+static hipError_t launch_hand_off(K kernel, const S &st, const M &rt, const M &tr, int phase, int k, int advance, hipStream_t stream, Extra... extra) {
+  hipLaunchKernelGGL(kernel, dim3((st.B + 255) / 256), dim3(256), 0, stream, st, rt, tr, phase, k, extra...);
+  if (advance > 0) hipLaunchKernelGGL(wb_clock_kernel, dim3(1), dim3(1), 0, stream, (long long *)st.hour, advance);
   return hipGetLastError();
 }
-hipError_t launch_wb_rolling(const dsp_wb_state &st, const dsp_wb_model &rt, const dsp_wb_model &tr, int phase, int k, hipStream_t stream) {
-  return launch_hand_off(wb_rolling_kernel, st, rt, tr, phase, k, stream);
+hipError_t launch_wb_rolling(const dsp_wb_state &st, const dsp_wb_model &rt, const dsp_wb_model &tr, int phase, int k, int off, int advance,
+                             hipStream_t stream) {
+  return launch_hand_off(wb_rolling_kernel, st, rt, tr, phase, k, advance, stream, off);
 }
 hipError_t launch_loop_update(const dsp_loop_state &st, const dsp_loop_model &rt, const dsp_loop_model &tr, int phase, int k, hipStream_t stream) {
-  return launch_hand_off(loop_update_kernel, st, rt, tr, phase, k, stream);
+  return launch_hand_off(loop_update_kernel, st, rt, tr, phase, k, phase == 2 ? 1 : 0, stream);
 }
 
 }
diff --git a/dispatches_amd/csrc/dsp_loop_device.hpp b/dispatches_amd/csrc/dsp_loop_device.hpp
--- a/dispatches_amd/csrc/dsp_loop_device.hpp
+++ b/dispatches_amd/csrc/dsp_loop_device.hpp
@@ -49,6 +49,97 @@
   tr.c0[b] = c0;
 }
 
+template <class M, class S>
+__device__ __forceinline__ void loop_check(const S &s, const M &m, int b) {
+  if (m.status && s.bad && m.status[b] != 0) *s.bad = 1;
+  if (m.flags && s.uncertified && (m.flags[b] & DSP_FLAG_OBJ_WAIVED)) atomicAdd(reinterpret_cast<unsigned long long *>(s.uncertified), 1ull);
+}
+
+__device__ __forceinline__ double loop_lane_value(double v, int q) {
+  return __hiloint2double(__builtin_amdgcn_readlane(__double2hiint(v), q), __builtin_amdgcn_readlane(__double2loint(v), q));
+}
+template <int LANES>
+__device__ __forceinline__ double wb_sum_in_order(double acc, int T) {
+  if constexpr (LANES == 1) {
+    return acc;
+  } else {
+    const int periods = __builtin_amdgcn_readfirstlane(T);
+    double sum = loop_lane_value(acc, 0);
+    for (int q = 1; q < periods; ++q) sum = __dadd_rn(sum, loop_lane_value(acc, q));
+    return sum;
+  }
+}
+
+template <int LANES>
+__device__ __forceinline__ void wb_phase0(const dsp_wb_state &s, const dsp_wb_model &m, int k, long long h, int b, int lane) {
+  const long long st0 = s.start[b];
+  const unsigned first = (unsigned)((st0 + h) % s.N);
+  auto win = [&](const double *series, int t) { return series[(first + (unsigned)t) % (unsigned)s.N]; };
+  const int known = min(m.T, 24 - k);
+  double *c = m.c + (size_t)b * m.n, *lb = m.lb + (size_t)b * m.n, *ub = m.ub + (size_t)b * m.n;
+  double avail_sum = 0.0;
+  for (int t = lane; t < m.T; t += LANES) {
+    const double rtp = win(s.rt_series, t);
+    const double dap = t < known ? s.da_prices[(size_t)b * 24 + k + t] : win(s.da_series, t);
+    const double r3 = loop_opaque(__dmul_rn(1e-3, rtp));
+    c[m.pt_cols[t][0]] = __dsub_rn(m.base_c[m.pt_cols[t][0]], r3);
+    c[m.pt_cols[t][1]] = __dsub_rn(m.base_c[m.pt_cols[t][1]], r3);
+    c[m.pda_cols[t]] = __dsub_rn(m.base_c[m.pda_cols[t]], loop_opaque(__dsub_rn(dap, rtp)));
+    const double avail = __dmul_rn(m.wind_kw, win(s.cf_series, t));
+    ub[m.wind_cols[t]] = avail;
+    avail_sum = (LANES == 1 && t) ? __dadd_rn(avail_sum, avail) : avail;
+    const double fix = t < known ? s.da_offer[(size_t)b * 24 + k + t] : 0.0;
+    lb[m.pda_cols[t]] = fix;
+    ub[m.pda_cols[t]] = t < known ? fix : INFINITY;
+  }
+  avail_sum = wb_sum_in_order<LANES>(avail_sum, m.T);
+  if (lane == 0) {
+    if (m.c0) m.c0[b] = __dadd_rn(m.c0_base, loop_opaque(__dmul_rn(m.waste_per_kw, avail_sum)));
+    lb[m.soc_init] = s.soc[b]; ub[m.soc_init] = s.soc[b];
+    lb[m.thr_init] = s.thr[b]; ub[m.thr_init] = s.thr[b];
+  }
+}
+
+template <int LANES>
+__device__ __forceinline__ void wb_phase1(const dsp_wb_state &s, const dsp_wb_model &rt, const dsp_wb_model &tr, long long h, int b, int lane) {
+  const long long st0 = s.start[b];
+  const unsigned first = (unsigned)((st0 + h) % s.N);
+  auto win = [&](const double *series, int t) { return series[(first + (unsigned)t) % (unsigned)s.N]; };
+  if (lane == 0) loop_check(s, rt, b);
+  const double *xr = rt.x + (size_t)b * rt.n;
+  double *lb = tr.lb + (size_t)b * tr.n, *ub = tr.ub + (size_t)b * tr.n;
+  double *rlo = tr.rlo + (size_t)b * tr.m, *rhi = tr.rhi + (size_t)b * tr.m;
+  double avail_sum = 0.0;
+  for (int t = lane; t < tr.T; t += LANES) {
+    const double offer = __dmul_rn(1e-3, loop_opaque(__dadd_rn(xr[rt.pt_cols[t][0]], xr[rt.pt_cols[t][1]])));
+    rlo[tr.track_rows[t]] = offer;
+    rhi[tr.track_rows[t]] = offer;
+    const double avail = __dmul_rn(tr.wind_kw, win(s.cf_series, t));
+    ub[tr.wind_cols[t]] = avail;
+    avail_sum = (LANES == 1 && t) ? __dadd_rn(avail_sum, avail) : avail;
+  }
+  avail_sum = wb_sum_in_order<LANES>(avail_sum, tr.T);
+  if (lane == 0) {
+    if (tr.c0) tr.c0[b] = __dadd_rn(tr.c0_base, loop_opaque(__dmul_rn(tr.waste_per_kw, avail_sum)));
+    lb[tr.soc_init] = s.soc[b]; ub[tr.soc_init] = s.soc[b];
+    lb[tr.thr_init] = s.thr[b]; ub[tr.thr_init] = s.thr[b];
+  }
+}
+
+__device__ __forceinline__ void wb_phase2(const dsp_wb_state &s, const dsp_wb_model &tr, int k, long long h, int b) {
+  loop_check(s, tr, b);
+  const double *x = tr.x + (size_t)b * tr.n;
+  const double delivered = loop_opaque(__dmul_rn(1e-3, loop_opaque(__dadd_rn(x[tr.pt_cols[0][0]], x[tr.pt_cols[0][1]]))));
+  const double rt0 = s.rt_series[(s.start[b] + h) % s.N];
+  s.delivered[b] = delivered;
+  s.soc[b] = __ddiv_rn(rint(loop_opaque(__dmul_rn(x[tr.soc0], 100.0))), 100.0);
+  s.thr[b] = __ddiv_rn(rint(loop_opaque(__dmul_rn(x[tr.thr0], 100.0))), 100.0);
+  const double dao = s.da_offer[(size_t)b * 24 + k], dap = s.da_prices[(size_t)b * 24 + k];
+  const double t1 = loop_opaque(__dmul_rn(delivered, rt0)), t2 = loop_opaque(__dmul_rn(dao, loop_opaque(__dsub_rn(dap, rt0))));
+  s.revenue[b] = __dadd_rn(s.revenue[b], loop_opaque(__dadd_rn(t1, t2)));
+  s.energy_mwh[b] = __dadd_rn(s.energy_mwh[b], delivered);
+}
+
 __device__ __forceinline__ double loop_ledger_form(const double *x, const int32_t *cols, const double *coef, int E, double constant,
                                                    double per_avail, double avail0) {
   double v = constant;
diff --git a/dispatches_amd/csrc/dsp_simplex.hip b/dispatches_amd/csrc/dsp_simplex.hip
--- a/dispatches_amd/csrc/dsp_simplex.hip
+++ b/dispatches_amd/csrc/dsp_simplex.hip
@@ -5,6 +5,7 @@
 #include <cstdlib>
 
 #include "dsp_device.hpp"
+#include "dsp_loop_device.hpp"
 #include "dsp_wave.hpp"
 
 namespace dsp {
@@ -12,6 +13,20 @@
 namespace {
 
 constexpr double kBig = 1e300;
+
+__device__ __forceinline__ const WbHandOff &simplex_hand_off_args() {
+  const char *p = (const char *)__builtin_amdgcn_kernarg_segment_ptr() + __builtin_offsetof(SimplexArgs, wb);
+  asm volatile("" : "+v"(p));
+  return *reinterpret_cast<const WbHandOff *>(p);
+}
+__device__ __forceinline__ void simplex_hand_off(const WbHandOff &w, int b, int lane) {
+  const long long h = *w.s.hour + w.off;
+  if ((w.phases & DSP_WB_HAND_PHASE2_PREV) && lane == 0) wb_phase2(w.s, w.tr, w.k - 1, h - 1, b);
+  if (w.phases & DSP_WB_HAND_PHASE0) wb_phase0<64>(w.s, w.rt, w.k, h, b, lane);
+  if (w.phases & DSP_WB_HAND_PHASE1) wb_phase1<64>(w.s, w.rt, w.tr, h, b, lane);
+  __builtin_amdgcn_fence(__ATOMIC_RELEASE, "workgroup");
+  __builtin_amdgcn_fence(__ATOMIC_ACQUIRE, "workgroup");
+}
 
 __device__ __forceinline__ double lds_d(const double *base, int idx) { return base[idx]; }
 
@@ -33,6 +48,7 @@
   int *iscal = reinterpret_cast<int *>(scal + 8);
 
   for (int s = blockIdx.x; s < b.B; s += gridDim.x) {
+    if (a.wb.phases) simplex_hand_off(simplex_hand_off_args(), s, lane);
     bool use_warm = a.warm == 1 && a.warm_valid[s] != 0;
     int pivots_before = 0;
   restart:
@@ -888,7 +904,9 @@
   SimplexArgs args = a;
   void *params[] = {&args};
   static const int force_lds = getenv("DSP_SX_LDS") ? atoi(getenv("DSP_SX_LDS")) : 0;
-  if (!force_lds && !a.warm && a.m <= 24 && cq <= 1 && a.b.B <= 2048) {
+  const bool in_registers = simplex_in_registers(a.warm, a.n, a.m, a.b.B);
+  if (a.wb.phases && in_registers) return hipErrorInvalidValue;
+  if (!force_lds && in_registers) {
     const void *fr = reinterpret_cast<const void *>(&simplex_reg_kernel<1, 24>);
     return hipLaunchKernel(fr, dim3(a.b.B < grid ? a.b.B : grid), dim3(64), params, 0, st);
   }
diff --git a/dispatches_amd/hip_solver.py b/dispatches_amd/hip_solver.py
--- a/dispatches_amd/hip_solver.py
+++ b/dispatches_amd/hip_solver.py
@@ -95,10 +95,13 @@
                     "dsp_get_scaling", "dsp_destroy", "dsp_strerror", "dsp_last_hip_error", "dsp_version",
                     "dsp_rtc_compile_check", "dsp_rtc_message", "dsp_wb_rolling_update", "dsp_loop_update", "dsp_bid_points", "dsp_source_hash",
                     "dsp_market_prepare", "dsp_market_clear", "dsp_loop_market_prepare", "dsp_loop_market_clear", "dsp_loop_param_step", "dsp_loop_project",
-                    "dsp_loop_schedule_prepare", "dsp_loop_monotone_prepare", "dsp_loop_ledger", "dsp_loop_record")
-
-
-ABI_VERSION = 21
+                    "dsp_loop_schedule_prepare", "dsp_loop_monotone_prepare", "dsp_loop_ledger", "dsp_loop_record", "dsp_wb_hour_solve", "dsp_wb_hour_settle")
+
+
+ABI_VERSION = 22
+
+
+WB_HAND_PHASE0, WB_HAND_PHASE1, WB_HAND_PHASE2_PREV = 1, 2, 4
 
 
 BID_MAX_HOURS, BID_MAX_SCENARIOS = 64, 16384
@@ -259,6 +262,11 @@
     lib.dsp_rtc_message.restype = C.c_char_p
     lib.dsp_wb_rolling_update.argtypes = [C.POINTER(DspWbState), C.POINTER(DspWbModel), C.POINTER(DspWbModel), i32, i32, vp]
     lib.dsp_wb_rolling_update.restype = C.c_int
+    lib.dsp_wb_hour_solve.argtypes = [vp, C.POINTER(DspBatch), C.POINTER(DspOptions), C.POINTER(DspWbState), C.POINTER(DspWbModel), C.POINTER(DspWbModel),
+                                      i32, i32, i32, vp]
+    lib.dsp_wb_hour_solve.restype = C.c_int
+    lib.dsp_wb_hour_settle.argtypes = [C.POINTER(DspWbState), C.POINTER(DspWbModel), C.POINTER(DspWbModel), i32, i32, i32, vp]
+    lib.dsp_wb_hour_settle.restype = C.c_int
     lib.dsp_loop_update.argtypes = [C.POINTER(DspLoopState), C.POINTER(DspLoopModel), C.POINTER(DspLoopModel), i32, i32, vp]
     lib.dsp_loop_update.restype = C.c_int
     lib.dsp_bid_points.argtypes = [C.POINTER(DspBidRequest), vp]
@@ -371,7 +379,7 @@
         return t.data_ptr(), width
 
     def solve(self, B, c, lb=None, ub=None, rlo=None, rhi=None, x0=None, y0=None, options=None, out=None,
-              sync_stats=True, obj_offset=None, primal_weight=None, row_compliance=None):
+              sync_stats=True, obj_offset=None, primal_weight=None, row_compliance=None, hand_off=None):
         import torch
 
         n, m = self.lp.n, self.lp.m
@@ -407,9 +415,15 @@
         bt.flags = out["flags"].data_ptr() if "flags" in out else None
         stats = DspStats()
         stream = torch.cuda.current_stream(dev).cuda_stream
-        rc = self.lib.dsp_solve(self.handle, C.byref(bt), C.byref(options) if options is not None else None,
-                                C.byref(stats), 1 if sync_stats else 0, C.c_void_p(stream))
-        _check(self.lib, rc, "dsp_solve")
+        if hand_off is not None:
+            st, rt, tr, phases, k, off = hand_off
+            rc = self.lib.dsp_wb_hour_solve(self.handle, C.byref(bt), C.byref(options) if options is not None else None,
+                                            C.byref(st), C.byref(rt), C.byref(tr), phases, k, off, C.c_void_p(stream))
+            _check(self.lib, rc, "dsp_wb_hour_solve")
+        else:
+            rc = self.lib.dsp_solve(self.handle, C.byref(bt), C.byref(options) if options is not None else None,
+                                    C.byref(stats), 1 if sync_stats else 0, C.c_void_p(stream))
+            _check(self.lib, rc, "dsp_solve")
         self.last_stats = stats
         out["stats"] = stats
         return out
diff --git a/dispatches_amd/rolling.py b/dispatches_amd/rolling.py
--- a/dispatches_amd/rolling.py
+++ b/dispatches_amd/rolling.py
@@ -75,19 +75,24 @@
     def power_output(self, x):
         return 1e-3 * x[:, self.pt_cols].sum(dim=2)
 
-    def solve(self, B, x0=None, y0=None, primal_weight=None, hour=None):
+    def solve(self, B, x0=None, y0=None, primal_weight=None, hour=None, hand_off=None):
         opts = self.opts if (hour is None or self.opts is None) else (self.opts_first if hour == 0 else self.opts_warm)
+        extra = {} if hand_off is None else dict(hand_off=hand_off)
         self.out = self.dlp.solve(B, self.c, self.lb, self.ub, self.rlo if self.lp.m else None,
                                   self.rhi if self.lp.m else None, x0=x0, y0=y0, primal_weight=primal_weight,
-                                  options=opts, out=self.out, sync_stats=False, obj_offset=self.c0)
+                                  options=opts, out=self.out, sync_stats=False, obj_offset=self.c0, **extra)
         return self.out
+
+    def on_warm_simplex(self):
+        return (self.opts is not None and not self.opts.no_simplex and self.opts_warm.simplex_warm == 1 and self.opts_first.simplex_warm == 2
+                and self.lp.n + self.lp.m <= 128 and 1 <= self.lp.m <= 64)
 
 
 class BatchedWindBatteryDoubleLoop(_DeviceLoop):
     def __init__(self, n_scenarios, device=0, first_scenario=0, series="rts_gmlc_309.npz", stride=17,
                  day_ahead_horizon=48, real_time_horizon=4, tracking_horizon=4, wind_mw=200.0, batt_mw=25.0,
                  price_cap=500.0, warm_start=True, lp_backend=None, use_graphs=True, use_fused=True, record=None, simplex_warm=True, warm_patience=10000,
-                 n_price_scenarios=1, forecaster="perfect", max_historical_days=10, market="stub"):
+                 n_price_scenarios=1, forecaster="perfect", max_historical_days=10, market="stub", hand_off_in_solves=True):
         import torch
         from .workflow import Tracker
         self.B = B = int(n_scenarios)
@@ -213,6 +218,10 @@
             self._day_t = torch.zeros((), dtype=torch.int64, device=dev)
             self._limit_h = torch.full((), H, dtype=torch.int64, device=dev)
             self._limit_d = torch.full((), int(days), dtype=torch.int64, device=dev)
+        self._chain = (bool(hand_off_in_solves) and self.use_fused and not self.stochastic and self._rec is None and self.simplex_warm
+                       and self.rt.on_warm_simplex() and self.tr.on_warm_simplex())
+        self._open, self._lag = False, 0
+        self._tr_power0 = [int(v) for v in self.tr.pt_cols[0].cpu().tolist()] if self._chain else None
 
     def _record(self, what, value, daily=False):
         import torch
@@ -241,6 +250,7 @@
         if self.warm_start:
             self.da_x0.zero_(), self.da_y0.zero_()
         self.hour = self.solves = 0
+        self._open, self._lag = False, 0
 
     def _set_prices(self, m, da, rt):
         m.c[:] = m.base_c
@@ -396,6 +406,22 @@
         import ctypes as C
         self._call(self._lib.dsp_wb_rolling_update, C.byref(self._wb_state), C.byref(self._wb_rt), C.byref(self._wb_tr), phase, k)
 
+    def _settle(self):
+        import ctypes as C
+        if self._open:
+            self._call(self._lib.dsp_wb_hour_settle, C.byref(self._wb_state), C.byref(self._wb_rt), C.byref(self._wb_tr),
+                       self.hour - 1 - self.day_start, self._lag - 1, self._lag)
+            self._open, self._lag = False, 0
+
+    def _hour_step_chained(self, k, open_, lag, settle):
+        import ctypes as C
+        from .hip_solver import WB_HAND_PHASE0, WB_HAND_PHASE1, WB_HAND_PHASE2_PREV
+        wb = (self._wb_state, self._wb_rt, self._wb_tr)
+        self.rt.solve(self.B, hour=k, hand_off=wb + (WB_HAND_PHASE0 | (WB_HAND_PHASE2_PREV if open_ else 0), k, lag))
+        self.tr.solve(self.B, hour=k, hand_off=wb + (WB_HAND_PHASE1, k, lag))
+        if settle:
+            self._call(self._lib.dsp_wb_hour_settle, *(C.byref(w) for w in wb), k, lag, lag + 1)
+
     def _hour_step(self, k):
         import torch
         if self.use_fused:
@@ -444,19 +470,41 @@
         self.hour_t += 1
 
     def day_ahead(self):
+        self._settle()
         self.day_start = self.hour
         self._run("da", self._day_ahead_step_stochastic if self.stochastic else self._day_ahead_step)
         self.solves += self.B * self.S
         return self.da_offer.clone()
 
-    def hour_step(self):
+    def hour_step(self, settle=True):
         k = self.hour - self.day_start
+        if self._chain:
+            return self._hour_step_in_solves(k, settle or k == 23)
         self._run(k, (lambda: self._hour_step_stochastic(k)) if self.stochastic else (lambda: self._hour_step(k)))
         self.solves += self.B * self.S + self.B
         self.hour += 1
         return self.delivered.clone()
 
+    def _hour_step_in_solves(self, k, settle):
+        open_, lag = self._open, self._lag
+        key = k if (open_, lag, settle) == (k > 0, k, k == 23) else (k, open_, lag, settle)
+        self._run(key, lambda: self._hour_step_chained(k, open_, lag, settle))
+        self._open, self._lag = (False, 0) if settle else (True, lag + 1)
+        self.solves += 2 * self.B
+        self.hour += 1
+        if settle:
+            return self.delivered.clone()
+        x, (a, b) = self.tr.out["x"], self._tr_power0
+        return (x[:, a] + x[:, b]) * 1e-3
+
+    def run_day(self):
+        self.day_ahead()
+        for _ in range(24):
+            self.hour_step(settle=False)
+        self._warm = True
+
     def results(self):
+        self._settle()
         res = dict(obj=self.revenue, energy_mwh=self.energy_mwh, soc=self.soc, throughput=self.thr)
         if self.stochastic:
             res.update(da_energy_mwh=self.da_energy_mwh, offered_mwh=self.offered_mwh)
diff --git a/include/dsp_hip.h b/include/dsp_hip.h
--- a/include/dsp_hip.h
+++ b/include/dsp_hip.h
@@ -9,7 +9,7 @@
 extern "C" {
 #endif
 
-#define DSP_VERSION 21
+#define DSP_VERSION 22
 
 #define DSP_OK                 0
 #define DSP_ERR_INVALID       -1
@@ -171,6 +171,14 @@
 int dsp_wb_rolling_update(const dsp_wb_state *st, const dsp_wb_model *rt, const dsp_wb_model *tr, int32_t phase, int32_t k,
                           void *hipStream);
 
+#define DSP_WB_HAND_PHASE0       1
+#define DSP_WB_HAND_PHASE1       2
+#define DSP_WB_HAND_PHASE2_PREV  4
+int dsp_wb_hour_solve(dsp_handle *h, const dsp_batch *batch, const dsp_options *opt, const dsp_wb_state *st, const dsp_wb_model *rt,
+                      const dsp_wb_model *tr, int32_t phases, int32_t k, int32_t off, void *hipStream);
+int dsp_wb_hour_settle(const dsp_wb_state *st, const dsp_wb_model *rt, const dsp_wb_model *tr, int32_t k, int32_t off, int32_t advance,
+                       void *hipStream);
+
 #define DSP_LOOP_MAX_T 16
 typedef struct dsp_loop_model {
   double *c, *lb, *ub, *rlo, *rhi;
```

New measurement: 4.672 million (median of 4 runs). Within noise of the previous version (+0.0%).
